# salesforce/LayoutDETR

Hardware: AMD Instinct MI355X
Metric: images/sec G+D fwd-bwd, 256x256 bg x9 elems (higher is better)
Workload: dtype f32

## Files before the change

### include/ldetr_hip.h

```cpp
#ifndef LDETR_HIP_H
#define LDETR_HIP_H

#include <stdint.h>

#ifdef __cplusplus
extern "C" {
#endif

const char* ldetr_last_error(void);
int ldetr_abi_version(void);

int ldetr_debug_trace_tiles(int64_t* buffer);

int ldetr_set_split_bf16(int tiles);

int ldetr_engine_launch_counts(int64_t* f32_pipe, int64_t* bf16_split_pipe);

int ldetr_set_workspace(void* ptr, int64_t bytes);

typedef struct ldetr_tensor4 {
    int N, C, H, W;
    int64_t sn, sc, sh, sw;
} ldetr_tensor4;

typedef struct ldetr_epilogue {
    float alpha;
    const float* col_scale;
    const float* col_bias;
    const float* samp_scale;
    int64_t samp_ld;
    const float* residual;
    int64_t ldr;
    int act;
    float act_alpha;
    float act_gain;
    const float* mask_src;
    int64_t ldm;
    int mask_mode;
    float out_scale;
    float p_drop;
    uint64_t seed;
    const uint64_t* seed_ptr;
    int accumulate;
    float* a_rowsum;
} ldetr_epilogue;

int ldetr_bias_act_f32(const float* x, const float* b, const float* xref, const float* yref, const float* dy, float* y,
                       int64_t sizeX, int sizeB, int64_t stepB, int grad, int act, float alpha, float gain, float clamp,
                       void* stream);

int ldetr_upfirdn2d_f32(const float* x, const float* f, float* y, int N, int C, int inH, int inW,
                        const int64_t* x_strides_nchw, int fh, int fw, int64_t f_stride_h, int64_t f_stride_w,
                        int upx, int upy, int downx, int downy, int padx0, int padx1, int pady0, int pady1, int flip,
                        float gain, int outH, int outW, const int64_t* y_strides_nchw,
                        const float* act_bias, int has_act, float act_alpha, float act_gain, void* stream);

int ldetr_gemm_f32(const float* A, int64_t lda, int ta, const float* B, int64_t ldb, int tb, float* C, int64_t ldc,
                   int M, int N, int K, int splitk, const ldetr_epilogue* ep, int pix_per_sample, void* stream);

typedef struct ldetr_gemm_desc {
    const float* A; int64_t lda; int ta;
    const float* B; int64_t ldb; int tb;
    float* C; int64_t ldc;
    int M, N, K, splitk;
    const ldetr_epilogue* ep;
    int pix_per_sample;
} ldetr_gemm_desc;
int ldetr_gemm_pair_f32(const ldetr_gemm_desc* g0, const ldetr_gemm_desc* g1, void* stream);
int ldetr_gemm_pair_is_single_launch(const ldetr_gemm_desc* g0, const ldetr_gemm_desc* g1);

int ldetr_conv2d_fwd_f32(const float* x, const ldetr_tensor4* xt, const float* w, int Cout, int KH, int KW, int stride,
                         int pad, float* y, int64_t ldy, int OH, int OW, const float* in_scale, int64_t in_scale_ld,
                         const ldetr_epilogue* ep, void* stream);
int ldetr_conv2d_bwd_data_f32(const float* dy, const ldetr_tensor4* dyt, const float* w, int Cin, int KH, int KW,
                              int stride, int pad, float* dx, int64_t lddx, int IH, int IW, const float* dy_scale,
                              int64_t dy_scale_ld, const ldetr_epilogue* ep, void* stream);
int ldetr_conv2d_bwd_weight_f32(const float* x, const ldetr_tensor4* xt, const float* dy, const ldetr_tensor4* dyt,
                                float* dw, int KH, int KW, int stride, int pad, int splitk, const float* x_scale,
                                int64_t x_scale_ld, const float* dy_scale, int64_t dy_scale_ld, int accumulate, void* stream);

int ldetr_conv_transpose2d_fwd_f32(const float* x, const ldetr_tensor4* xt, const float* w, int Cout, int KH, int KW,
                                   int stride, int pad, float* y, int64_t ldy, int OH, int OW, const float* in_scale,
                                   int64_t in_scale_ld, const ldetr_epilogue* ep, void* stream);
int ldetr_conv_transpose2d_bwd_data_f32(const float* dy, const ldetr_tensor4* dyt, const float* w, int Cin, int KH,
                                        int KW, int stride, int pad, float* dx, int64_t lddx, int IH, int IW,
                                        const float* dy_scale, int64_t dy_scale_ld, const ldetr_epilogue* ep,
                                        void* stream);
int ldetr_conv_transpose2d_bwd_weight_f32(const float* x, const ldetr_tensor4* xt, const float* dy,
                                          const ldetr_tensor4* dyt, float* dw, int KH, int KW, int stride, int pad,
                                          int splitk, const float* x_scale, int64_t x_scale_ld, const float* dy_scale,
                                          int64_t dy_scale_ld, int accumulate, void* stream);

int ldetr_attention_fwd_f32(const float* q, int64_t ldq, const float* k, int64_t ldk, const float* v, int64_t ldv,
                            const unsigned char* key_padding_mask, float* out, int64_t ldo, float* lse, int B, int H,
                            int Lq, int Lk, int head_dim, float scale, float p_drop, uint64_t seed, const uint64_t* seed_ptr,
                            int causal, void* stream);
int ldetr_attention_bwd_f32(const float* q, int64_t ldq, const float* k, int64_t ldk, const float* v, int64_t ldv,
                            const unsigned char* key_padding_mask, const float* out, int64_t ldo, const float* lse,
                            const float* dout, int64_t lddo, float* dq, int64_t lddq, float* dk, int64_t lddk,
                            float* dv, int64_t lddv, int B, int H, int Lq, int Lk, int head_dim, float scale,
                            float p_drop, uint64_t seed, const uint64_t* seed_ptr, int causal, void* stream);

int ldetr_torgb_bwd_finish_f32(const float* dws, const float* s, const float* w, int B, int C, float* dw, float* ds, void* stream);

int ldetr_loss_combine_fwd_f32(const float* const* x, const float* w, const int* n, const int* fn, const int* red, int K, int ld,
                               float* vals, float* sums, float* total, void* stream);
int ldetr_loss_combine_bwd_f32(const float* const* x, const float* w, const int* n, const int* fn, const int* red, int K, int ld,
                               const float* g, float* grads, void* stream);
int ldetr_masked_mse_fwd_f32(const float* a, const float* b, const uint8_t* valid, int64_t rows, int D, int bdiv, float* out2, void* stream);
int ldetr_masked_mse_bwd_f32(const float* a, const float* b, const uint8_t* valid, int64_t rows, int D, int bdiv, const float* out2,
                             const float* g, float* da, void* stream);

typedef struct ldetr_ln_args {
    const float* x; const float* r; const float* gamma; const float* beta;
    float* y; float* z; float* mean; float* rstd;
    const float* dy; float* dx; float* dr; float* dgamma; float* dbeta;
    int64_t rows; int D; float eps, p_drop; uint64_t seed; const uint64_t* seed_ptr;
    const float* pos; int64_t pos_rows; float* ypos; const float* dy2;
    int r_parts; int64_t r_part_stride; const float* r_bias;
    const float* dy_parts; int dy_nparts; int64_t dy_part_stride;
} ldetr_ln_args;
int ldetr_layernorm_fwd_group_f32(const ldetr_ln_args* a, int n, void* stream);
int ldetr_layernorm_bwd_group_f32(const ldetr_ln_args* a, int n, void* stream);
int ldetr_sum_parts_f32(const float* base, const float* parts, int n_parts, int64_t part_stride, float* out, int64_t n, void* stream);

typedef struct ldetr_ffn_args {
    const float* x; int64_t ldx;
    const float* w1; const float* b1;
    const float* w2;
    float* h;
    float* ypart;
    int M, F;
    float p_drop; uint64_t seed; const uint64_t* seed_ptr;
    const float* dy;
    float* dxpart;
    float* dh;
} ldetr_ffn_args;
int ldetr_ffn_fwd_group_f32(const ldetr_ffn_args* a, int n, void* stream);
int ldetr_ffn_bwd_group_f32(const ldetr_ffn_args* a, int n, void* stream);

typedef struct ldetr_mha_small_args {
    const float* x; int64_t ldx;
    const float* w_in; const float* b_in; const float* w_out;
    const unsigned char* kpm;
    float* qkv; float* o; float* lse; float* ypart;
    int B, L;
    float scale, p_drop; uint64_t seed; const uint64_t* seed_ptr;
    const float* dr;
    float* dqkv; float* dxpart;
} ldetr_mha_small_args;
int ldetr_mha_small_fwd_group_f32(const ldetr_mha_small_args* a, int n, void* stream);
int ldetr_mha_small_bwd_group_f32(const ldetr_mha_small_args* a, int n, void* stream);

typedef struct ldetr_mha_cross_args {
    const float* x; int64_t ldx;
    const float* w_q; const float* b_q;
    const float* k; int64_t ldk; const float* v; int64_t ldv;
    const float* w_out;
    const unsigned char* kpm;
    float* q; float* o; float* lse; float* ypart;
    int B, Lq, Lk;
    float scale, p_drop; uint64_t seed; const uint64_t* seed_ptr;
    const float* dr;
    float* dq; float* dk; int64_t lddk; float* dv; int64_t lddv; float* dxpart;
} ldetr_mha_cross_args;
int ldetr_mha_cross_fwd_f32(const ldetr_mha_cross_args* a, void* stream);
int ldetr_mha_cross_bwd_f32(const ldetr_mha_cross_args* a, void* stream);

typedef struct ldetr_wgrad_desc {
    const float* A; int64_t lda; const float* B; int64_t ldb;
    float* dW; int64_t ldw; float* db;
    int M, rows, cols;
} ldetr_wgrad_desc;
int ldetr_wgrad_multi_f32(const ldetr_wgrad_desc* d, int n, void* stream);

int ldetr_colsum_f32(const float* a, float* red, int B, int64_t P, int C, void* stream);
int ldetr_act_bwd_reduce_f32(const float* dy, const float* y, float* dv, const float* bias, const float* demod,
                             float* dbias, float* ddemod, int B, int64_t P, int C, int act, float alpha, float gain,
                             void* stream);
int ldetr_mul_reduce_f32(const float* a, const float* x, const float* scale, float* out, float* red, int B, int64_t P,
                         int C, void* stream);
int ldetr_torgb_fwd_f32(const float* x, const float* w, const float* styles, const float* bias, float* y,
                        int B, int64_t P, int C, void* stream);
int ldetr_torgb_bwd_f32(const float* x, const float* dy, const float* w, const float* styles, float* dx, float* dws,
                        float* dbias, int B, int64_t P, int C, void* stream);
int ldetr_sg2_handoff_f32(const float* dxs, const float* x, const float* dy_rgb, float* dv, const float* s_conv, const float* s_rgb,
                          const float* w_rgb, const float* bias, const float* demod, float* ds_conv, float* dws_rgb, float* dbias_rgb,
                          float* dbias, float* ddemod, int B, int64_t P, int C, float alpha, float gain, void* stream);

int ldetr_maxpool3x3s2_fwd_f32(const float* x, float* y, unsigned char* idx, int N, int H, int W, int C, void* stream);
int ldetr_maxpool3x3s2_bwd_f32(const float* dy, const unsigned char* idx, float* dx, int N, int H, int W, int C,
                               void* stream);

int ldetr_grad_sanitize_f32(float* g, int64_t n, float scale, float nan_value, float posinf, float neginf,
                            void* stream);
int ldetr_adam_step_f32(float* p, const float* g, float* m, float* v, int64_t n, int64_t step, float lr, float beta1,
                        float beta2, float eps, int fuse_sanitize, float gscale, float nan_value, float posinf,
                        float neginf, void* stream);
int ldetr_adam_ema_step_f32(float* p, const float* g, float* m, float* v, int64_t n, int64_t step, float lr, float beta1, float beta2,
                            float eps, int fuse_sanitize, float gscale, float nan_value, float posinf, float neginf,
                            float* p_ema, float ema_beta, void* stream);
int ldetr_ema_lerp_f32(float* p_ema, const float* p, int64_t n, float beta, void* stream);

int ldetr_softmax_xent_fwd_f32(const float* logits, int64_t ld, const int64_t* targets, float* row_lse, float* loss_sum, float* count,
                               int64_t rows, int V, int64_t ignore_index, float label_smoothing, void* stream);
int ldetr_softmax_xent_bwd_f32(const float* logits, int64_t ld, const int64_t* targets, const float* row_lse, const float* count,
                               const float* grad_out, float* dlogits, int64_t ldd, int64_t rows, int V, int64_t ignore_index,
                               float label_smoothing, void* stream);

int ldetr_embedding_fwd_f32(const float* weight, const float* pos, const int64_t* ids, float* out, int64_t n, int d, int V, int T,
                            void* stream);
int ldetr_embedding_bwd_f32(const float* dy, const int64_t* ids, float* dweight, int64_t n, int d, int V, int64_t padding_idx,
                            void* stream);

int ldetr_resample_coeffs(int in_size, int out_size, int32_t* bounds, int32_t* weights, int64_t weights_capacity, int* ksize_out);
int ldetr_resize_normalize_u8(const uint8_t* src, int64_t images, int H, int W, int out_h, int out_w, const int32_t* hbounds,
                              const int32_t* hweights, int hksize, const int32_t* vbounds, const int32_t* vweights, int vksize,
                              uint8_t* tmp, uint8_t* out_u8, float* out_chw, float mean0, float mean1, float mean2, float std0,
                              float std1, float std2, void* stream);

#define LDETR_PAGE_FILTER_BLUR 1
#define LDETR_PAGE_FILTER_EDGE 2
int ldetr_page_filter_u8(const uint8_t* src, uint8_t* dst, int64_t images, int H, int W, int kind, float radius, void* stream);

int ldetr_demod_fwd_f32(const float* weight, int64_t so, int64_t si, int64_t sh, int64_t sw, const float* styles, float* dcoefs,
                        float* w2, int B, int O, int I, int KH, int KW, float eps, void* stream);
int ldetr_demod_bwd_f32(const float* weight, int64_t so, int64_t si, int64_t sh, int64_t sw, const float* styles, const float* dcoefs,
                        const float* w2, const float* grad_dcoefs, float* dweight, int accumulate_dweight, float* dstyles, int B, int O,
                        int I, int KH, int KW, void* stream);

int ldetr_layout_losses_f32(const float* bbox, const float* bbox_ref, const uint8_t* valid, int B, int N, float* losses,
                            float* grads, void* stream);
int ldetr_layout_losses_bwd_f32(const float* grads, const float* grad_losses, int B, int N, float* dbbox, void* stream);

int ldetr_layout_finish_f32(const float* bbox_in, const int* num, const float* factors, const unsigned char* jitter, const unsigned char* mode,
                            float* bbox_out, float* overlap, float* alignment, int* order, int C, int K, int N, void* stream);

#define LDETR_FILTER_BILINEAR 0
#define LDETR_FILTER_LANCZOS 1
typedef struct ldetr_layout_raster_args {
    int struct_bytes;
    int B, N, S, nrow, n_colors, n_pages;
    const float* bbox;
    const uint8_t* valid;
    const int32_t* labels;
    const uint8_t* palette;
    const int32_t* page_wh;
    const uint8_t* pages;
    int64_t pages_bytes;
    const int64_t* page_table;
    const int32_t* page_index;
    const int32_t* coeffs;
    int64_t coeffs_len;
    const int64_t* cell_coeffs;
    int32_t* cells_dev;
    uint8_t* out;
} ldetr_layout_raster_args;
int ldetr_resample_coeffs_filter(int filter, int in_size, int out_size, int32_t* bounds, int32_t* weights, int64_t weights_capacity, int* ksize_out);
int ldetr_layout_raster_cell_size(int W, int H, int S, int* wn_out, int* hn_out);
int ldetr_layout_raster_u8(const ldetr_layout_raster_args* a, void* stream);

typedef struct ldetr_patch_resize_args {
    int struct_bytes;
    int n_jobs;
    const uint8_t* src0;
    int64_t src0_bytes;
    const uint8_t* src1;
    int64_t src1_bytes;
    uint8_t* dst;
    int64_t dst_bytes;
    const int64_t* jobs;
    const int32_t* tables;
    const int32_t* tables_host;
    int64_t tables_len;
    int32_t* jobs_dev;
} ldetr_patch_resize_args;
typedef struct ldetr_image_raster_args {
    int struct_bytes;
    int B, N, S, nrow;
    const float* bbox;
    const uint8_t* valid;
    const int32_t* rects;
    const int64_t* patch_off;
    const int64_t* page_off;
    const int32_t* page_wh;
    const uint8_t* pixels;
    int64_t pixels_bytes;
    const int32_t* coeffs;
    int64_t coeffs_len;
    const int64_t* cell_coeffs;
    int32_t* cells_dev;
    uint8_t* out;
} ldetr_image_raster_args;
int ldetr_patch_resize_u8(const ldetr_patch_resize_args* a, void* stream);
int ldetr_image_raster_u8(const ldetr_image_raster_args* a, void* stream);

#define LDETR_PNG_NOT_ELIGIBLE 3
#define LDETR_PNG_MALFORMED 4
typedef struct ldetr_png_decode_args {
    int struct_bytes;
    int n, H, W;
    int phases;
    int reserved;
    const uint8_t* files;
    int64_t files_bytes;
    const int64_t* file_off;
    const int64_t* file_off_dev;
    const int64_t* segments;
    const int64_t* segments_dev;
    int64_t n_segments;
    const int32_t* jobs;
    const int32_t* jobs_dev;
    int64_t n_jobs;
    uint8_t* scratch;
    int64_t scratch_bytes;
    uint8_t* dst;
} ldetr_png_decode_args;
int ldetr_png_scan(const uint8_t* file, int64_t file_bytes, int* width, int* height, int* channels, int64_t* segments, int64_t segments_capacity,
                   int64_t* segments_count, int32_t* row_starts, int64_t row_starts_capacity, int64_t* row_starts_count);
int ldetr_png_decode_u8(const ldetr_png_decode_args* a, void* stream);

typedef struct ldetr_png_encode_args {
    int struct_bytes;
    int H, W;
    int blocks;
    int filter;
    int reserved;
    const uint8_t* src;
    uint8_t* out;
    int64_t out_capacity;
    int64_t* total_bytes;
    uint8_t* workspace;
    int64_t workspace_bytes;
    int64_t* seg_table;
    int64_t seg_table_rows;
} ldetr_png_encode_args;
int ldetr_png_encode_bound(int H, int W, int64_t* out_bytes, int64_t* workspace_bytes);
int ldetr_png_encode_u8(const ldetr_png_encode_args* a, void* stream);

int ldetr_lsap_f64(const double* cost, int batch, int n, int maximize, int* row_ind, int* col_ind, void* stream);

int ldetr_layoutnet_features_f32(const float* bbox, const int64_t* label, const uint8_t* padding_mask, const int* label_map, int map_len,
                                 const float* weights, int64_t weights_len, int num_label, int B, int N, float* out, void* stream);

int ldetr_layoutnet_forward_f32(const float* bbox, const int64_t* label, const uint8_t* padding_mask, const float* enc_weights,
                                int64_t enc_len, const float* dec_weights, int64_t dec_len, int num_label, int B, int N,
                                float* logit_disc, float* logit_cls, float* bbox_pred, float* features, void* stream);

int ldetr_feature_stats_f64(const float* x, int64_t n, int F, double* raw_mean, double* raw_cov, void* stream);

int ldetr_box_giou_pairwise_f32(const float* boxes1, const float* boxes2, int B, int N, int M, int cxcywh, float* iou, float* uni,
                                float* giou, double* cost, double cost_sign, void* stream);

int ldetr_bmm_strided_f32(const float* A, const int64_t* sa, const float* B, const int64_t* sb, float* C, const int64_t* sc,
                          int nb1, int nb2, int M, int N, int K, float alpha, void* stream);

int ldetr_p3_split_f32(const float* src, int64_t ld, void* dst, int64_t rows, int C, void* stream);
int ldetr_p3_merge_f32(const void* src, float* dst, int64_t ld, int64_t rows, int C, void* stream);
int ldetr_p3_weight_bwd(const float* w_ohwi, const float* o_scale, void* dst, int O, int KH, int KW, int I, void* stream);

int ldetr_p3_weight_prep(const int64_t* table_dev, int nconv, int total_blocks, void* stream);

typedef struct ldetr_p3_epilogue {
    float alpha;
    const float* col_scale;
    const float* col_bias;
    const void* residual_p3;
    const float* residual_f32;
    const void* relu_mask_p3;
    int relu;
} ldetr_p3_epilogue;

int ldetr_p3_conv2d_fwd(const void* x, int N, int H, int W, int Cin, const void* w, int Cout, int KH, int KW, int stride, int pad,
// ... 23 lines not shown
```

### layoutdetr_amd/_lib.py

```python
import ctypes
import os
from ctypes import (POINTER, Structure, c_char_p, c_double, c_float, c_int, c_int64, c_ubyte, c_uint64, c_void_p)

_HERE = os.path.dirname(os.path.abspath(__file__))
ABI_VERSION = 25
LIB_PATH = os.environ.get('LDETR_LIB') or os.path.join(_HERE, 'lib', 'libldetr_hip.so')


class Tensor4(Structure):
    _fields_ = [('N', c_int), ('C', c_int), ('H', c_int), ('W', c_int),
                ('sn', c_int64), ('sc', c_int64), ('sh', c_int64), ('sw', c_int64)]


class GemmDesc(Structure):
    _fields_ = [('A', c_void_p), ('lda', c_int64), ('ta', c_int), ('B', c_void_p), ('ldb', c_int64), ('tb', c_int),
                ('C', c_void_p), ('ldc', c_int64), ('M', c_int), ('N', c_int), ('K', c_int), ('splitk', c_int),
                ('ep', c_void_p), ('pix_per_sample', c_int)]


class P3Epilogue(Structure):
    _fields_ = [('alpha', c_float), ('col_scale', c_void_p), ('col_bias', c_void_p), ('residual_p3', c_void_p),
                ('residual_f32', c_void_p), ('relu_mask_p3', c_void_p), ('relu', c_int)]


class Epilogue(Structure):
    _fields_ = [('alpha', c_float), ('col_scale', c_void_p), ('col_bias', c_void_p), ('samp_scale', c_void_p),
                ('samp_ld', c_int64), ('residual', c_void_p), ('ldr', c_int64), ('act', c_int),
                ('act_alpha', c_float), ('act_gain', c_float), ('mask_src', c_void_p), ('ldm', c_int64),
                ('mask_mode', c_int), ('out_scale', c_float), ('p_drop', c_float), ('seed', c_uint64),
                ('seed_ptr', c_void_p), ('accumulate', c_int), ('a_rowsum', c_void_p)]


class LnArgs(Structure):
    _fields_ = [('x', c_void_p), ('r', c_void_p), ('gamma', c_void_p), ('beta', c_void_p),
                ('y', c_void_p), ('z', c_void_p), ('mean', c_void_p), ('rstd', c_void_p),
                ('dy', c_void_p), ('dx', c_void_p), ('dr', c_void_p), ('dgamma', c_void_p), ('dbeta', c_void_p),
                ('rows', c_int64), ('D', c_int), ('eps', c_float), ('p_drop', c_float), ('seed', c_uint64), ('seed_ptr', c_void_p),
                ('pos', c_void_p), ('pos_rows', c_int64), ('ypos', c_void_p), ('dy2', c_void_p),
                ('r_parts', c_int), ('r_part_stride', c_int64), ('r_bias', c_void_p),
                ('dy_parts', c_void_p), ('dy_nparts', c_int), ('dy_part_stride', c_int64)]


class FfnArgs(Structure):
    _fields_ = [('x', c_void_p), ('ldx', c_int64), ('w1', c_void_p), ('b1', c_void_p), ('w2', c_void_p), ('h', c_void_p), ('ypart', c_void_p),
                ('M', c_int), ('F', c_int), ('p_drop', c_float), ('seed', c_uint64), ('seed_ptr', c_void_p),
                ('dy', c_void_p), ('dxpart', c_void_p), ('dh', c_void_p)]


class MhaSmallArgs(Structure):
    _fields_ = [('x', c_void_p), ('ldx', c_int64), ('w_in', c_void_p), ('b_in', c_void_p), ('w_out', c_void_p), ('kpm', c_void_p),
                ('qkv', c_void_p), ('o', c_void_p), ('lse', c_void_p), ('ypart', c_void_p), ('B', c_int), ('L', c_int),
                ('scale', c_float), ('p_drop', c_float), ('seed', c_uint64), ('seed_ptr', c_void_p),
                ('dr', c_void_p), ('dqkv', c_void_p), ('dxpart', c_void_p)]


class MhaCrossArgs(Structure):
    _fields_ = [('x', c_void_p), ('ldx', c_int64), ('w_q', c_void_p), ('b_q', c_void_p), ('k', c_void_p), ('ldk', c_int64), ('v', c_void_p), ('ldv', c_int64),
                ('w_out', c_void_p), ('kpm', c_void_p), ('q', c_void_p), ('o', c_void_p), ('lse', c_void_p), ('ypart', c_void_p),
                ('B', c_int), ('Lq', c_int), ('Lk', c_int), ('scale', c_float), ('p_drop', c_float), ('seed', c_uint64), ('seed_ptr', c_void_p),
                ('dr', c_void_p), ('dq', c_void_p), ('dk', c_void_p), ('lddk', c_int64), ('dv', c_void_p), ('lddv', c_int64), ('dxpart', c_void_p)]


class WgradDesc(Structure):
    _fields_ = [('A', c_void_p), ('lda', c_int64), ('B', c_void_p), ('ldb', c_int64), ('dW', c_void_p), ('ldw', c_int64), ('db', c_void_p),
                ('M', c_int), ('rows', c_int), ('cols', c_int)]


class LayoutRasterArgs(Structure):
    _fields_ = [('struct_bytes', c_int), ('B', c_int), ('N', c_int), ('S', c_int), ('nrow', c_int), ('n_colors', c_int), ('n_pages', c_int),
                ('bbox', c_void_p), ('valid', c_void_p), ('labels', c_void_p), ('palette', c_void_p), ('page_wh', c_void_p),
                ('pages', c_void_p), ('pages_bytes', c_int64), ('page_table', c_void_p), ('page_index', c_void_p),
                ('coeffs', c_void_p), ('coeffs_len', c_int64), ('cell_coeffs', c_void_p), ('cells_dev', c_void_p), ('out', c_void_p)]


class PatchResizeArgs(Structure):
    _fields_ = [('struct_bytes', c_int), ('n_jobs', c_int), ('src0', c_void_p), ('src0_bytes', c_int64), ('src1', c_void_p), ('src1_bytes', c_int64),
                ('dst', c_void_p), ('dst_bytes', c_int64), ('jobs', c_void_p), ('tables', c_void_p), ('tables_host', c_void_p), ('tables_len', c_int64),
                ('jobs_dev', c_void_p)]


class ImageRasterArgs(Structure):
    _fields_ = [('struct_bytes', c_int), ('B', c_int), ('N', c_int), ('S', c_int), ('nrow', c_int),
                ('bbox', c_void_p), ('valid', c_void_p), ('rects', c_void_p), ('patch_off', c_void_p), ('page_off', c_void_p), ('page_wh', c_void_p),
                ('pixels', c_void_p), ('pixels_bytes', c_int64), ('coeffs', c_void_p), ('coeffs_len', c_int64), ('cell_coeffs', c_void_p),
                ('cells_dev', c_void_p), ('out', c_void_p)]


class PngDecodeArgs(Structure):
    _fields_ = [('struct_bytes', c_int), ('n', c_int), ('H', c_int), ('W', c_int), ('phases', c_int), ('reserved', c_int),
                ('files', c_void_p), ('files_bytes', c_int64), ('file_off', c_void_p), ('file_off_dev', c_void_p),
                ('segments', c_void_p), ('segments_dev', c_void_p), ('n_segments', c_int64),
                ('jobs', c_void_p), ('jobs_dev', c_void_p), ('n_jobs', c_int64),
                ('scratch', c_void_p), ('scratch_bytes', c_int64), ('dst', c_void_p)]


class PngEncodeArgs(Structure):
    _fields_ = [('struct_bytes', c_int), ('H', c_int), ('W', c_int), ('blocks', c_int), ('filter', c_int), ('reserved', c_int),
                ('src', c_void_p), ('out', c_void_p), ('out_capacity', c_int64), ('total_bytes', c_void_p),
                ('workspace', c_void_p), ('workspace_bytes', c_int64), ('seg_table', c_void_p), ('seg_table_rows', c_int64)]


_P = c_void_p
_I = c_int
_L = c_int64
_F = c_float
_T4 = POINTER(Tensor4)
_EP = POINTER(Epilogue)

SIGNATURES = {
    'ldetr_set_workspace': [_P, _L],
    'ldetr_bias_act_f32': [_P, _P, _P, _P, _P, _P, _L, _I, _L, _I, _I, _F, _F, _F, _P],
    'ldetr_upfirdn2d_f32': [_P, _P, _P, _I, _I, _I, _I, POINTER(c_int64), _I, _I, _L, _L, _I, _I, _I, _I, _I, _I, _I, _I,
                            _I, _F, _I, _I, POINTER(c_int64), _P, _I, _F, _F, _P],
    'ldetr_gemm_f32': [_P, _L, _I, _P, _L, _I, _P, _L, _I, _I, _I, _I, _EP, _I, _P],
    'ldetr_conv2d_fwd_f32': [_P, _T4, _P, _I, _I, _I, _I, _I, _P, _L, _I, _I, _P, _L, _EP, _P],
    'ldetr_conv2d_bwd_data_f32': [_P, _T4, _P, _I, _I, _I, _I, _I, _P, _L, _I, _I, _P, _L, _EP, _P],
    'ldetr_conv2d_bwd_weight_f32': [_P, _T4, _P, _T4, _P, _I, _I, _I, _I, _I, _P, _L, _P, _L, _I, _P],
    'ldetr_conv_transpose2d_fwd_f32': [_P, _T4, _P, _I, _I, _I, _I, _I, _P, _L, _I, _I, _P, _L, _EP, _P],
    'ldetr_conv_transpose2d_bwd_data_f32': [_P, _T4, _P, _I, _I, _I, _I, _I, _P, _L, _I, _I, _P, _L, _EP, _P],
    'ldetr_conv_transpose2d_bwd_weight_f32': [_P, _T4, _P, _T4, _P, _I, _I, _I, _I, _I, _P, _L, _P, _L, _I, _P],
    'ldetr_attention_fwd_f32': [_P, _L, _P, _L, _P, _L, _P, _P, _L, _P, _I, _I, _I, _I, _I, _F, _F, c_uint64, _P, _I, _P],
    'ldetr_attention_bwd_f32': [_P, _L, _P, _L, _P, _L, _P, _P, _L, _P, _P, _L, _P, _L, _P, _L, _P, _L,
                                _I, _I, _I, _I, _I, _F, _F, c_uint64, _P, _I, _P],
    'ldetr_colsum_f32': [_P, _P, _I, _L, _I, _P],
    'ldetr_act_bwd_reduce_f32': [_P, _P, _P, _P, _P, _P, _P, _I, _L, _I, _I, _F, _F, _P],
    'ldetr_mul_reduce_f32': [_P, _P, _P, _P, _P, _I, _L, _I, _P],
    'ldetr_torgb_fwd_f32': [_P, _P, _P, _P, _P, _I, _L, _I, _P],
    'ldetr_torgb_bwd_f32': [_P, _P, _P, _P, _P, _P, _P, _I, _L, _I, _P],
    'ldetr_maxpool3x3s2_fwd_f32': [_P, _P, _P, _I, _I, _I, _I, _P],
    'ldetr_maxpool3x3s2_bwd_f32': [_P, _P, _P, _I, _I, _I, _I, _P],
    'ldetr_grad_sanitize_f32': [_P, _L, _F, _F, _F, _F, _P],
    'ldetr_adam_step_f32': [_P, _P, _P, _P, _L, _L, _F, _F, _F, _F, _I, _F, _F, _F, _F, _P],
    'ldetr_adam_ema_step_f32': [_P, _P, _P, _P, _L, _L, _F, _F, _F, _F, _I, _F, _F, _F, _F, _P, _F, _P],
    'ldetr_ema_lerp_f32': [_P, _P, _L, _F, _P],
    'ldetr_lsap_f64': [_P, _I, _I, _I, _P, _P, _P],
    'ldetr_layoutnet_features_f32': [_P, _P, _P, POINTER(c_int), _I, _P, _L, _I, _I, _I, _P, _P],
    'ldetr_layoutnet_forward_f32': [_P, _P, _P, _P, _L, _P, _L, _I, _I, _I, _P, _P, _P, _P, _P],
    'ldetr_feature_stats_f64': [_P, _L, _I, _P, _P, _P],
    'ldetr_box_giou_pairwise_f32': [_P, _P, _I, _I, _I, _I, _P, _P, _P, _P, c_double, _P],
    'ldetr_bmm_strided_f32': [_P, _P, _P, _P, _P, _P, _I, _I, _I, _I, _I, _F, _P],
    'ldetr_softmax_xent_fwd_f32': [_P, _L, _P, _P, _P, _P, _L, _I, _L, _F, _P],
    'ldetr_softmax_xent_bwd_f32': [_P, _L, _P, _P, _P, _P, _P, _L, _L, _I, _L, _F, _P],
    'ldetr_embedding_fwd_f32': [_P, _P, _P, _P, _L, _I, _I, _I, _P],
    'ldetr_embedding_bwd_f32': [_P, _P, _P, _L, _I, _I, _L, _P],
    'ldetr_debug_trace_tiles': [_P],
    'ldetr_set_split_bf16': [c_int],
    'ldetr_engine_launch_counts': [POINTER(c_int64), POINTER(c_int64)],
    'ldetr_layernorm_fwd_group_f32': [_P, _I, _P],
    'ldetr_layernorm_bwd_group_f32': [_P, _I, _P],
    'ldetr_sum_parts_f32': [_P, _P, _I, _L, _P, _L, _P],
    'ldetr_ffn_fwd_group_f32': [_P, _I, _P],
    'ldetr_ffn_bwd_group_f32': [_P, _I, _P],
    'ldetr_mha_small_fwd_group_f32': [_P, _I, _P],
    'ldetr_mha_small_bwd_group_f32': [_P, _I, _P],
    'ldetr_mha_cross_fwd_f32': [_P, _P],
    'ldetr_mha_cross_bwd_f32': [_P, _P],
    'ldetr_wgrad_multi_f32': [_P, _I, _P],
    'ldetr_loss_combine_fwd_f32': [_P, _P, _P, _P, _P, _I, _I, _P, _P, _P, _P],
    'ldetr_loss_combine_bwd_f32': [_P, _P, _P, _P, _P, _I, _I, _P, _P, _P],
    'ldetr_masked_mse_fwd_f32': [_P, _P, _P, _L, _I, _I, _P, _P],
    'ldetr_masked_mse_bwd_f32': [_P, _P, _P, _L, _I, _I, _P, _P, _P, _P],
    'ldetr_torgb_bwd_finish_f32': [_P, _P, _P, _I, _I, _P, _P, _P],
    'ldetr_sg2_handoff_f32': [_P, _P, _P, _P, _P, _P, _P, _P, _P, _P, _P, _P, _P, _P, _I, _L, _I, _F, _F, _P],
    'ldetr_gemm_pair_f32': [_P, _P, _P],
    'ldetr_gemm_pair_is_single_launch': [_P, _P],
    'ldetr_demod_fwd_f32': [_P, _L, _L, _L, _L, _P, _P, _P, _I, _I, _I, _I, _I, _F, _P],
    'ldetr_demod_bwd_f32': [_P, _L, _L, _L, _L, _P, _P, _P, _P, _P, _I, _P, _I, _I, _I, _I, _I, _P],
    'ldetr_layout_losses_f32': [_P, _P, _P, _I, _I, _P, _P, _P],
    'ldetr_layout_losses_bwd_f32': [_P, _P, _I, _I, _P, _P],
    'ldetr_layout_finish_f32': [_P, _P, _P, _P, _P, _P, _P, _P, _P, _I, _I, _I, _P],
    'ldetr_resample_coeffs': [_I, _I, _P, _P, _L, _P],
    'ldetr_resample_coeffs_filter': [_I, _I, _I, _P, _P, _L, _P],
    'ldetr_layout_raster_cell_size': [_I, _I, _I, _P, _P],
    'ldetr_layout_raster_u8': [_P, _P],
    'ldetr_patch_resize_u8': [_P, _P],
    'ldetr_image_raster_u8': [_P, _P],
    'ldetr_p3_split_f32': [_P, _L, _P, _L, _I, _P],
    'ldetr_p3_merge_f32': [_P, _P, _L, _L, _I, _P],
    'ldetr_p3_weight_bwd': [_P, _P, _P, _I, _I, _I, _I, _P],
    'ldetr_p3_conv2d_bwd_data': [_P, _I, _I, _I, _I, _P, _I, _I, _I, _I, _I, _I, _I, _P, _P, _P, _P],
    'ldetr_p3_conv2d_fwd': [_P, _I, _I, _I, _I, _P, _I, _I, _I, _I, _I, _P, _P, _P, _P],
    'ldetr_p3_conv2d_bwd_weight': [_P, _I, _I, _I, _I, _P, _I, _I, _I, _I, _I, _P, _P, _P],
    'ldetr_p3_weight_prep': [_P, _I, _I, _P],
    'ldetr_p3_conv2d_fwd_dual': [_P, _P, _I, _I, _I, _I, _P, _P, _I, _I, _I, _I, _I, _P, _P, _P, _P, _P, _P, _P],
    'ldetr_p3_conv2d_bwd_pair': [_P, _I, _I, _I, _I, _P, _P, _I, _I, _I, _I, _I, _I, _I, _P, _P, _P, _P, _P, _P, _P],
    'ldetr_p3_last_launch': [_P],
    'ldetr_engine_last_launch': [_P],
    'ldetr_struct_sizes': [_P],
    'ldetr_resize_normalize_u8': [_P, _L, _I, _I, _I, _I, _P, _P, _I, _P, _P, _I, _P, _P, _P, _F, _F, _F, _F, _F, _F, _P],
    'ldetr_page_filter_u8': [_P, _P, _L, _I, _I, _I, _F, _P],
    'ldetr_png_scan': [_P, _L, _P, _P, _P, _P, _L, _P, _P, _L, _P],
    'ldetr_png_decode_u8': [_P, _P],
    'ldetr_png_encode_bound': [_I, _I, _P, _P],
    'ldetr_png_encode_u8': [_P, _P],
}

_lib = None


def load():
    global _lib
    if _lib is not None:
        return _lib
    if not os.path.exists(LIB_PATH):
        raise RuntimeError(
            f'{LIB_PATH} not found: build the gfx950 kernels first (python -m layoutdetr_amd.build or '
            f'__graft_entry__.build()).  layoutdetr_amd has no CPU/PyTorch fallback path.')
    import torch
    lib = ctypes.CDLL(LIB_PATH)
    lib.ldetr_last_error.restype = c_char_p
    lib.ldetr_last_error.argtypes = []
    lib.ldetr_abi_version.restype = c_int
    lib.ldetr_abi_version.argtypes = []
    for name, argtypes in SIGNATURES.items():
        fn = getattr(lib, name)
        fn.restype = c_int
        fn.argtypes = argtypes
    if lib.ldetr_abi_version() != ABI_VERSION:
        raise RuntimeError('libldetr_hip.so ABI version mismatch; rebuild it')
    sizes = (ctypes.c_int32 * 6)()
    lib.ldetr_struct_sizes(sizes)
    mirror = [ctypes.sizeof(t) for t in (LnArgs, FfnArgs, MhaSmallArgs, MhaCrossArgs, WgradDesc, P3Epilogue)]
    if list(sizes) != mirror:
        raise RuntimeError(f'libldetr_hip.so argument blocks {list(sizes)} do not match the ctypes mirror {mirror}; rebuild')
    _lib = lib
    return lib


def check(rc, what=''):
    if rc != 0:
        msg = load().ldetr_last_error().decode('utf-8', 'replace')
        raise RuntimeError(f'{what}: {msg}' if what else msg)
```

### layoutdetr_amd/build.py

```python
import hashlib
import os
import shutil
import subprocess
import sys
from concurrent.futures import ThreadPoolExecutor

HERE = os.path.dirname(os.path.abspath(__file__))
CSRC = os.path.join(HERE, 'csrc')
LIBDIR = os.path.join(HERE, 'lib')
OBJDIR = os.path.join(LIBDIR, 'obj')
LIBNAME = 'libldetr_hip.so'
ARCH = 'gfx950'

SOURCES = ['ldetr_core.cpp', 'bias_act.hip', 'upfirdn2d.hip', 'gemm_conv.hip', 'attention.hip', 'layernorm.hip',
           'misc_ops.hip', 'optim.hip', 'lsap.hip', 'xent.hip', 'resample.hip', 'layout_loss.hip', 'demod.hip', 'wgrad_smallc.hip', 'stem_conv.hip', 'box_ops.hip', 'ffn_fused.hip', 'conv_c32.hip', 'mha_small.hip', 'p3_engine.hip', 'bmm_strided.hip', 'layoutnet.hip', 'layoutnet_train.hip', 'layout_finish.hip', 'layout_raster.hip', 'page_filter.hip', 'patch_resize.hip', 'png_decode.hip', 'png_encode.hip']
HEADERS = ['ldetr_common.hpp', 'layoutnet_layers.hpp', os.path.join('..', '..', 'include', 'ldetr_hip.h')]

FLAGS = ([] if os.environ.get('LDETR_TILE_TRACE') else ['-DLDETR_TILE_TRACE=0']) + (['-DP3_TRACE'] if os.environ.get('LDETR_P3_TRACE') else []) + ['-O3', '-std=c++17', '-fPIC', f'--offload-arch={ARCH}', '-munsafe-fp-atomics', '-fno-gpu-rdc',
         '-Wno-unused-result', '-Rpass-analysis=kernel-resource-usage']
NO_SCRATCH = ('wgrad_c32_3x3_kernel', 'gemm_f32_kernel', 'gemm_small_kernel', 'attn_fwd_kernel', 'attn_fwd_wide_kernel', 'attn_bwd_kernel', 'ffn_fwd_kernel', 'ffn_bwd_kernel', 'conv3x3_c32_kernel', 'mha_small_fwd_kernel', 'mha_cross_fwd_kernel', 'mha_small_bwd_kernel', 'mha_cross_bwd_kernel', 'wgrad_multi_kernel', 'ln_fwd_kernel', 'ln_bwd_kernel', 'p3_nt_kernel', 'p3_tn_kernel', 'p3_c3_kernel', 'p3_bwd_pair', 'layoutnet_features_kernel', 'layoutnet_forward_kernel', 'feature_stats_f64_kernel', 'layout_finish_kernel', 'layout_raster_kernel', 'page_blur_kernel', 'page_edge_kernel', 'patch_resize_kernel', 'sg2_handoff_kernel', 'png_gather_kernel', 'png_unfilter_kernel', 'png_enc_filter_kernel', 'png_enc_deflate_kernel', 'png_enc_assemble_kernel')


def _hipcc():
    for cand in (os.environ.get('HIPCC'), shutil.which('hipcc'), '/opt/rocm/bin/hipcc'):
        if cand and os.path.exists(cand):
            return cand
    raise RuntimeError('hipcc not found: the gfx950 kernel library cannot be built')


def _digest(paths):
    h = hashlib.sha256()
    for p in paths:
        with open(p, 'rb') as f:
            h.update(f.read())
    h.update(' '.join(FLAGS).encode())
    return h.hexdigest()


def _kernel_resources(remarks):
    out, cur = {}, None
    for line in remarks.splitlines():
        if 'remark:' not in line:
            continue
        body = line.split('remark:', 1)[1].split('[-Rpass-analysis', 1)[0].strip()
        if body.startswith('Function Name:'):
            cur = body.split(':', 1)[1].strip()
            out[cur] = {}
        elif cur is not None and ':' in body:
            k, v = body.rsplit(':', 1)
            out[cur][k.strip()] = v.strip()
    return out


def source_digest():
    return _digest(sorted(os.path.join(CSRC, f) for f in os.listdir(CSRC) if f.endswith(('.hip', '.cpp', '.hpp')) and not f.startswith('.'))
                   + [os.path.normpath(os.path.join(CSRC, HEADERS[-1]))])


def lib_path():
    return os.path.join(LIBDIR, LIBNAME)


def build(force=False, verbose=True):
    os.makedirs(OBJDIR, exist_ok=True)
    hipcc = _hipcc()
    hdrs = [os.path.normpath(os.path.join(CSRC, h)) for h in HEADERS]
    objs, jobs = [], []
    for src in SOURCES:
        sp = os.path.join(CSRC, src)
        obj = os.path.join(OBJDIR, src + '.o')
        stamp = obj + '.sha'
        dig = _digest([sp] + hdrs)
        objs.append(obj)
        if not force and os.path.exists(obj) and os.path.exists(stamp) and open(stamp).read() == dig:
            continue
        jobs.append((sp, obj, stamp, dig))

    def compile_one(job):
        sp, obj, stamp, dig = job
        cmd = [hipcc] + FLAGS + ['-x', 'hip', '-c', sp, '-o', obj]
        if verbose:
            print('[ldetr build]', os.path.basename(sp), flush=True)
        r = subprocess.run(cmd, capture_output=True, text=True)
        if r.returncode != 0:
            raise RuntimeError(f'hipcc failed for {sp}:\n{r.stdout}\n{r.stderr}')
        res = _kernel_resources(r.stderr)
        with open(obj + '.resources.txt', 'w') as f:
            for name, d in res.items():
                f.write(f"{name} vgprs={d.get('VGPRs', '?')} agprs={d.get('AGPRs', '?')} scratch={d.get('ScratchSize [bytes/lane]', '?')} "
                        f"occupancy={d.get('Occupancy [waves/SIMD]', '?')} lds={d.get('LDS Size [bytes/block]', '?')}\n")
        bad = [n for n, d in res.items() if any(k in n for k in NO_SCRATCH) and d.get('ScratchSize [bytes/lane]', '0') != '0']
        if bad:
            raise RuntimeError(f'{os.path.basename(sp)}: scratch memory in register-budgeted kernels: ' + ', '.join(bad[:4]))
        with open(stamp, 'w') as f:
            f.write(dig)

    if jobs:
        with ThreadPoolExecutor(max_workers=min(8, len(jobs))) as ex:
            list(ex.map(compile_one, jobs))
    out = lib_path()
    if jobs or not os.path.exists(out):
        cmd = [hipcc, '-shared', '-fPIC', f'--offload-arch={ARCH}', '-fno-gpu-rdc', '-o', out] + objs
        r = subprocess.run(cmd, capture_output=True, text=True)
        if r.returncode != 0:
            raise RuntimeError(f'link failed:\n{r.stdout}\n{r.stderr}')
        if verbose:
            print('[ldetr build] linked', out, flush=True)
    return out


if __name__ == '__main__':
    build(force='--force' in sys.argv)
```

### layoutdetr_amd/csrc/gemm_conv.hip

```cpp
#include <cstdlib>
#include <type_traits>
#include <atomic>
#include "ldetr_common.hpp"
#include "../../include/ldetr_hip.h"

namespace ldetr {
static thread_local int64_t t_launches_f32 = 0, t_launches_split = 0;
void count_engine_launch(bool bf16_split_pipe) { (bf16_split_pipe ? t_launches_split : t_launches_f32)++; }

enum {
    OP_KC_DENSE = 0,
    OP_KC_CONV = 1,
    OP_KC_CONVT = 2,
    OP_KC_WTAP = 3,
    OP_RC_DENSE = 4,
    OP_RC_PIX = 5,
    OP_RC_WT = 6,
    OP_RC_CONVK = 7,
};

struct Operand {
    const float* p;
    long ld;
    int vec;
// ... 742 lines not shown
                for (int j = 0; j < TN; j++) b[nx][j] = Bs[buf][(kk + 1) * 2 + kl][wn * WN + j * 32 + cl];
            }
            __builtin_amdgcn_sched_barrier(0);
#pragma unroll
            for (int i = 0; i < TM; i++)
#pragma unroll
                for (int j = 0; j < TN; j++)
                    acc[i][j] = __builtin_amdgcn_mfma_f32_32x32x2f32(a[c][i], b[c][j], acc[i][j], 0, 0, 0);
            __builtin_amdgcn_sched_barrier(0);
        }
    };
    auto compute_split = [&]() {
#pragma unroll
        for (int ks = 0; ks < BKT / 16; ks++) {
            bf16x8_t a[TM][3], b[TN][3];
#pragma unroll
            for (int i = 0; i < TM; i++)
#pragma unroll
                for (int q = 0; q < 3; q++) a[i][q] = *reinterpret_cast<const bf16x8_t*>(adrA(q, 2 * ks + kl, wm * WM + i * 32 + cl, 0));
#pragma unroll
            for (int j = 0; j < TN; j++)
#pragma unroll
                for (int q = 0; q < 3; q++) b[j][q] = *reinterpret_cast<const bf16x8_t*>(adrB(q, 2 * ks + kl, wn * WN + j * 32 + cl, 0));
#pragma unroll
            for (int i = 0; i < TM; i++)
#pragma unroll
                for (int j = 0; j < TN; j++) {
                    acc[i][j] = __builtin_amdgcn_mfma_f32_32x32x16_bf16(a[i][1], b[j][1], acc[i][j], 0, 0, 0);
                    acc[i][j] = __builtin_amdgcn_mfma_f32_32x32x16_bf16(a[i][0], b[j][2], acc[i][j], 0, 0, 0);
                    acc[i][j] = __builtin_amdgcn_mfma_f32_32x32x16_bf16(a[i][2], b[j][0], acc[i][j], 0, 0, 0);
                    acc[i][j] = __builtin_amdgcn_mfma_f32_32x32x16_bf16(a[i][0], b[j][1], acc[i][j], 0, 0, 0);
                    acc[i][j] = __builtin_amdgcn_mfma_f32_32x32x16_bf16(a[i][1], b[j][0], acc[i][j], 0, 0, 0);
                    acc[i][j] = __builtin_amdgcn_mfma_f32_32x32x16_bf16(a[i][0], b[j][0], acc[i][j], 0, 0, 0);
                }
        }
    };
    if (nk > 0) {
        gload(z.kbeg, ra0, rb0, sa0);
        lstore(std::bool_constant<SPLIT>{}, 0, ra0, rb0, sa0);
    }
    long long tr1 = 0, tr2 = 0;
    if constexpr (SPLIT) {
        __syncthreads();
        for (int kt = 0; kt < nk; kt++) {
            if (kt + 1 < nk) gload(z.kbeg + (kt + 1) * BKT, ra0, rb0, sa0);
            compute_split();
            __syncthreads();
            if (kt + 1 < nk) { lstore(std::bool_constant<SPLIT>{}, 0, ra0, rb0, sa0); __syncthreads(); }
        }
        float chk = 0.f;
#pragma unroll
        for (int i = 0; i < TM; i++)
#pragma unroll
            for (int j = 0; j < TN; j++)
#pragma unroll
                for (int r = 0; r < 16; r++) chk = __builtin_fmaf(acc[i][j][r], 0.f, chk);
        if (__builtin_expect(__syncthreads_or(chk != chk), 0)) {
            int t2 = tid;
            asm volatile("" : "+v"(t2));
            float (*A1)[LDA] = reinterpret_cast<float (*)[LDA]>(ldetr_smem);
            float (*B1)[LDB] = reinterpret_cast<float (*)[LDB]>(ldetr_smem + BKT * LDA);
            static_assert((size_t)BKT * (LDA + LDB) * sizeof(float) <= (size_t)3 * (BKT / 8) * (PLA + PLB), "the f32 image of one k-tile must fit inside the bf16 image");
#pragma unroll
            for (int i = 0; i < TM; i++)
#pragma unroll
                for (int j = 0; j < TN; j++)
#pragma unroll
                    for (int r = 0; r < 16; r++) acc[i][j][r] = 0.f;
            reset_kstate();
            const int kl2 = (t2 & 63) >> 5, cl2 = t2 & 31, w2 = t2 >> 6, wm2 = w2 / WGN, wn2 = w2 % WGN;
            for (int kt = 0; kt < nk; kt++) {
                gload(z.kbeg + kt * BKT, ra0, rb0, sa0);
                if constexpr (A_DEFER) {
                    if (a_defer) {
#pragma unroll
                        for (int i = 0; i < NUA; i++) { ra0[i].x *= sa0[i].x; ra0[i].y *= sa0[i].y; ra0[i].z *= sa0[i].z; ra0[i].w *= sa0[i].w; }
                    }
                }
#pragma unroll
                for (int i = 0; i < NUA; i++) {
                    int r, k; unitA(t2, i, r, k);
                    if constexpr (A_KC) { A1[k + 0][r] = ra0[i].x; A1[k + 1][r] = ra0[i].y; A1[k + 2][r] = ra0[i].z; A1[k + 3][r] = ra0[i].w; }
                    else { A1[k][r + 0] = ra0[i].x; A1[k][r + 1] = ra0[i].y; A1[k][r + 2] = ra0[i].z; A1[k][r + 3] = ra0[i].w; }
                }
#pragma unroll
                for (int i = 0; i < NUB; i++) {
                    int r, k; unitB(t2, i, r, k);
                    if constexpr (B_KC) { B1[k + 0][r] = rb0[i].x; B1[k + 1][r] = rb0[i].y; B1[k + 2][r] = rb0[i].z; B1[k + 3][r] = rb0[i].w; }
                    else { B1[k][r + 0] = rb0[i].x; B1[k][r + 1] = rb0[i].y; B1[k][r + 2] = rb0[i].z; B1[k][r + 3] = rb0[i].w; }
                }
                __syncthreads();
#pragma unroll 1
                for (int kk = 0; kk < BKT / 2; kk++) {
#pragma unroll
                    for (int i = 0; i < TM; i++) {
                        const float a = A1[kk * 2 + kl2][wm2 * WM + i * 32 + cl2];
#pragma unroll
                        for (int j = 0; j < TN; j++)
                            acc[i][j] = __builtin_amdgcn_mfma_f32_32x32x2f32(a, B1[kk * 2 + kl2][wn2 * WN + j * 32 + cl2], acc[i][j], 0, 0, 0);
                    }
                }
                __syncthreads();
            }
        }
    } else
    {
        __syncthreads();
        if (LDETR_TILE_TRACE && p.trace) tr1 = wall_clock64();
        if (!LDETR_TILE_TRACE) __builtin_amdgcn_sched_barrier(0);
        for (int kt = 0; kt < nk; kt++) {
            const int buf = kt & 1;
            if (kt + 1 < nk) gload(z.kbeg + (kt + 1) * BKT, ra0, rb0, sa0);
            compute(buf);
            if (kt + 1 < nk) lstore(std::false_type{}, buf ^ 1, ra0, rb0, sa0);
            __syncthreads();
        }
    }

    if (LDETR_TILE_TRACE && p.trace) tr2 = wall_clock64();
    if (!LDETR_TILE_TRACE) __builtin_amdgcn_sched_barrier(0);
    auto trace_out = [&]() {
        if (LDETR_TILE_TRACE && p.trace && threadIdx.x == 0) {
            long long* t = p.trace + 5 * (((long)blockIdx.z * gridDim.y + blockIdx.y) * gridDim.x + blockIdx.x);
            t[0] = tr0; t[1] = tr1; t[2] = tr2; t[3] = wall_clock64();
            t[4] = ((long long)__builtin_amdgcn_s_getreg(20 | (31 << 11)) << 32) | (unsigned)__builtin_amdgcn_s_getreg(4 | (31 << 11));
        }
    };
    bool direct = p.splitk <= 1;
    if (p.splitk > 1 && p.ws) {
        const int zb = p.zmode == 1 ? p.pstep * p.pstep : (p.zmode == 2 ? p.ntaps : 1);
        const int ks = blockIdx.z / zb;
        const long tile = ((long)(blockIdx.z - ks * zb) * gridDim.y + blockIdx.y) * gridDim.x + blockIdx.x;
        float* slot0 = p.ws + tile * p.splitk * (long)(BM * BN);
        float* mine = slot0 + (long)ks * (BM * BN);
#pragma unroll
        for (int i = 0; i < TM; i++)
#pragma unroll
            for (int j = 0; j < TN; j++)
#pragma unroll
                for (int r = 0; r < 16; r++)
                    __hip_atomic_store(mine + ((i * TN + j) * 16 + r) * NT + tid, acc[i][j][r], __ATOMIC_RELAXED, __HIP_MEMORY_SCOPE_AGENT);
        asm volatile("s_waitcnt vmcnt(0)" ::: "memory");
        __shared__ int s_last;
        __syncthreads();
        if (tid == 0) {
            int old = atomicAdd(p.ws_count + tile, 1);
            s_last = (old == p.splitk - 1);
            if (s_last) __hip_atomic_store(p.ws_count + tile, 0, __ATOMIC_RELAXED, __HIP_MEMORY_SCOPE_AGENT);
        }
        __syncthreads();
        if (!s_last) { trace_out(); return; }
#pragma unroll
        for (int i = 0; i < TM; i++)
#pragma unroll
            for (int j = 0; j < TN; j++)
#pragma unroll
                for (int r = 0; r < 16; r++) acc[i][j][r] = 0.f;
        for (int sl = 0; sl < p.splitk; sl++) {
            const float* src = slot0 + (long)sl * (BM * BN);
#pragma unroll
            for (int i = 0; i < TM; i++)
#pragma unroll
                for (int j = 0; j < TN; j++)
#pragma unroll
                    for (int r = 0; r < 16; r++)
                        acc[i][j][r] += __hip_atomic_load(src + ((i * TN + j) * 16 + r) * NT + tid, __ATOMIC_RELAXED, __HIP_MEMORY_SCOPE_AGENT);
        }
        direct = true;
    }

    const GemmEpilogue& ep = p.ep;
    const float inv_keep = ep.p_drop > 0.f ? 1.f / (1.f - ep.p_drop) : 1.f;
    if (direct && p.ep_vec) {
        constexpr int CP = BN + 4;
        constexpr int LDSF = 2 * BKT * (LDA + LDB);
        constexpr int PASSES = (BM * CP + LDSF - 1) / LDSF, RP = BM / PASSES;
        static_assert(BM % PASSES == 0 && RP * CP <= LDSF && (RP % 32) == 0, "epilogue staging does not fit");
        static_assert(!SPLIT || RP * CP * 4 <= 3 * (BKT / 8) * (PLA + PLB), "epilogue staging does not fit the split path's LDS image");
        float* Cs = ldetr_smem;
#pragma unroll
        for (int ps = 0; ps < PASSES; ps++) {
            if (ps > 0) __syncthreads();
#pragma unroll
            for (int i = 0; i < TM; i++) {
                const int rb = wm * WM + i * 32 - ps * RP;
                if (rb < 0 || rb >= RP) continue;
#pragma unroll
                for (int j = 0; j < TN; j++)
#pragma unroll
                    for (int r = 0; r < 16; r++)
                        Cs[(rb + (r & 3) + 8 * (r >> 2) + 4 * kl) * CP + wn * WN + j * 32 + cl] = acc[i][j][r];
            }
            __syncthreads();
            for (int u = tid; u < RP * (BN / 4); u += NT) {
                const int rl = u / (BN / 4), c4 = (u - rl * (BN / 4)) * 4;
                const int m = m0 + ps * RP + rl, n = n0 + c4;
                if (m >= z.M || n >= p.N) continue;
                long orow = m;
                if (p.zmode == 1 && p.pstep > 1) {
                    int per = z.DH2 * z.DW2;
                    int nn = m / per; int rem = m - nn * per;
                    int y2 = rem / z.DW2; int x2 = rem - y2 * z.DW2;
                    orow = ((long)nn * p.A.DH + (y2 * p.pstep + z.py)) * p.A.DW + (x2 * p.pstep + z.px);
                }
                const int samp = (ep.samp_scale && p.pix_per_sample > 0) ? (int)((unsigned)orow / (unsigned)p.pix_per_sample) : 0;
                const float4 a4 = *reinterpret_cast<const float4*>(Cs + rl * CP + c4);
                float4 cs4 = make_float4(1.f, 1.f, 1.f, 1.f), cb4 = make_float4(0.f, 0.f, 0.f, 0.f), rs4 = make_float4(0.f, 0.f, 0.f, 0.f);
                if (ep.col_scale) cs4 = *reinterpret_cast<const float4*>(ep.col_scale + n);
                if (ep.col_bias) cb4 = *reinterpret_cast<const float4*>(ep.col_bias + n);
                if (ep.residual) rs4 = *reinterpret_cast<const float4*>(ep.residual + orow * ep.ldr + n);
                float4 mk4 = make_float4(0.f, 0.f, 0.f, 0.f);
                if (ep.mask_mode) mk4 = *reinterpret_cast<const float4*>(ep.mask_src + orow * ep.ldm + n);
                float* dst = p.C + z.c_off + orow * p.ldc + n;
                float4 o;
                o.x = apply_epilogue(ep, a4.x, orow, n + 0, samp, p.ldc, inv_keep, cs4.x, cb4.x, rs4.x, mk4.x);
                o.y = apply_epilogue(ep, a4.y, orow, n + 1, samp, p.ldc, inv_keep, cs4.y, cb4.y, rs4.y, mk4.y);
                o.z = apply_epilogue(ep, a4.z, orow, n + 2, samp, p.ldc, inv_keep, cs4.z, cb4.z, rs4.z, mk4.z);
                o.w = apply_epilogue(ep, a4.w, orow, n + 3, samp, p.ldc, inv_keep, cs4.w, cb4.w, rs4.w, mk4.w);
                if (ep.accumulate) { const float4 c = *reinterpret_cast<const float4*>(dst); o.x += c.x; o.y += c.y; o.z += c.z; o.w += c.w; }
                *reinterpret_cast<float4*>(dst) = o;
            }
        }
        trace_out(); return;
    }
    float cs[TN], cb[TN], sfc[TN];
#pragma unroll
    for (int j = 0; j < TN; j++) {
        int n = n0 + wn * WN + j * 32 + cl;
        cs[j] = (ep.col_scale && n < p.N) ? ep.col_scale[n] : 1.f;
        cb[j] = (ep.col_bias && n < p.N) ? ep.col_bias[n] : 0.f;
        sfc[j] = (p.scol && n < p.N) ? p.scol[(long)z.samp * p.scol_ld + n] : 1.f;
    }
#pragma unroll
    for (int i = 0; i < TM; i++) {
#pragma unroll
        for (int r = 0; r < 16; r++) {
            int m = m0 + wm * WM + i * 32 + (r & 3) + 8 * (r >> 2) + 4 * kl;
            if (m >= z.M) continue;
            long orow = m;
            if (p.zmode == 1 && p.pstep > 1) {
                int per = z.DH2 * z.DW2;
                int n = m / per; int rem = m - n * per;
                int y2 = rem / z.DW2; int x2 = rem - y2 * z.DW2;
                orow = ((long)n * p.A.DH + (y2 * p.pstep + z.py)) * p.A.DW + (x2 * p.pstep + z.px);
            }
            int samp = (ep.samp_scale && p.pix_per_sample > 0) ? (int)((unsigned)orow / (unsigned)p.pix_per_sample) : 0;
            const float sfr = p.srow ? p.srow[(long)z.samp * p.srow_ld + m] : 1.f;
#pragma unroll
            for (int j = 0; j < TN; j++) {
                int n = n0 + wn * WN + j * 32 + cl;
                if (n >= p.N) continue;
                float* dst = p.C + z.c_off + orow * p.ldc + n;
                const float a = acc[i][j][r] * sfr * sfc[j];
                if (!direct) {
                    atomicAdd(dst, a * (ep.row_scale ? ep.alpha * ep.row_scale[orow] : ep.alpha));
                } else {
                    float v = apply_epilogue(ep, a, orow, n, samp, p.ldc, inv_keep, cs[j], cb[j], ep.residual ? ep.residual[orow * ep.ldr + n] : 0.f,
                                           ep.mask_mode ? ep.mask_src[orow * ep.ldm + n] : 0.f);
                    if (ep.accumulate) *dst += v; else *dst = v;
                }
            }
        }
    }
    trace_out();
}

template <int T>
__device__ __forceinline__ void small_load(const Operand& o, int row, int R, int k0, int kl, int kend, float (&f)[16]) {
    const int kb = k0 + 16 * kl;
    if (T == 0) {
        const float* src = o.p + (long)row * o.ld + kb;
        if (row < R && o.vec) {
#pragma unroll
            for (int j = 0; j < 4; j++) {
                float4 v = make_float4(0.f, 0.f, 0.f, 0.f);
                if (kb + 4 * j < kend) v = *reinterpret_cast<const float4*>(src + 4 * j);
                f[4 * j] = v.x; f[4 * j + 1] = v.y; f[4 * j + 2] = v.z; f[4 * j + 3] = v.w;
            }
        } else {
#pragma unroll
            for (int t = 0; t < 16; t++) f[t] = (row < R && kb + t < kend) ? src[t] : 0.f;
        }
    } else {
        const float* src = o.p + (long)kb * o.ld + row;
#pragma unroll
        for (int t = 0; t < 16; t++) f[t] = (row < R && kb + t < kend) ? src[(long)t * o.ld] : 0.f;
    }
}

template <int T>
__device__ __forceinline__ void small_load_fast(const __amdgpu_buffer_rsrc_t& rs, int voff, int k0, int ld, float (&f)[16]) {
    if (T == 0) {
#pragma unroll
        for (int j = 0; j < 4; j++) {
            const auto v = __builtin_amdgcn_raw_buffer_load_b128(rs, voff + 16 * j, k0 * 4, 0);
            f[4 * j] = __int_as_float(v[0]); f[4 * j + 1] = __int_as_float(v[1]); f[4 * j + 2] = __int_as_float(v[2]); f[4 * j + 3] = __int_as_float(v[3]);
        }
    } else {
#pragma unroll
        for (int t = 0; t < 16; t++) f[t] = __int_as_float(__builtin_amdgcn_raw_buffer_load_b32(rs, voff, (k0 + t) * ld * 4, 0));
    }
}

template <int TA, int TB, int NW, bool FAST = false>
__device__ __forceinline__ void gemm_small_body(const GemmParams& p, const int bx, const int by, const int bz, const int sk, const int gx) {
    using f32x16 = __attribute__((__vector_size__(16 * sizeof(float)))) float;
    __shared__ float red[NW][32][33];
    const int tid = threadIdx.x, lane = tid & 63, wave = tid >> 6;
    const int cl = lane & 31, kl = lane >> 5;
    const int m0 = by * 32, n0 = bx * 32;
    const int chunks_all = (p.K + 31) / 32;
    const int cper = (chunks_all + sk - 1) / sk;
    const int kblk0 = bz * cper * 32, kblk1 = min(p.K, kblk0 + cper * 32);
    const int chunks = kblk1 > kblk0 ? (kblk1 - kblk0 + 31) / 32 : 0, per = (chunks + NW - 1) / NW;
    const int kbeg = kblk0 + wave * per * 32, kend = min(kblk1, kbeg + per * 32);
    __amdgpu_buffer_rsrc_t rsA = __builtin_amdgcn_make_buffer_rsrc(const_cast<float*>(p.A.p), 0, FAST ? 0x7fffffff : 0, 0x00020000);
    __amdgpu_buffer_rsrc_t rsB = __builtin_amdgcn_make_buffer_rsrc(const_cast<float*>(p.B.p), 0, FAST ? 0x7fffffff : 0, 0x00020000);
    const int voffA = (m0 + cl < p.M) ? (TA == 0 ? ((m0 + cl) * (int)p.A.ld + 16 * kl) * 4 : (16 * kl * (int)p.A.ld + m0 + cl) * 4) : (int)0x80000000;
    const int voffB = (n0 + cl < p.N) ? (TB == 0 ? ((n0 + cl) * (int)p.B.ld + 16 * kl) * 4 : (16 * kl * (int)p.B.ld + n0 + cl) * 4) : (int)0x80000000;
    auto loadA = [&](int k0, float (&f)[16]) {
        if constexpr (FAST) small_load_fast<TA>(rsA, voffA, k0, (int)p.A.ld, f); else small_load<TA>(p.A, m0 + cl, p.M, k0, kl, kend, f);
        if constexpr (TA == 0) {
            if (p.A.scale) {
                const int kb = k0 + 16 * kl;
#pragma unroll
                for (int j = 0; j < 4; j++) {
                    if (kb + 4 * j < kend) {
                        const float4 s4 = *reinterpret_cast<const float4*>(p.A.scale + kb + 4 * j);
                        f[4 * j] *= s4.x; f[4 * j + 1] *= s4.y; f[4 * j + 2] *= s4.z; f[4 * j + 3] *= s4.w;
                    }
                }
            }
        }
    };
    auto loadB = [&](int k0, float (&f)[16]) {
        if constexpr (FAST) small_load_fast<TB>(rsB, voffB, k0, (int)p.B.ld, f); else small_load<TB>(p.B, n0 + cl, p.N, k0, kl, kend, f);
    };
    f32x16 acc;
#pragma unroll
    for (int r = 0; r < 16; r++) acc[r] = 0.f;
    float a0[16], b0[16], a1[16], b1[16];
    const bool want_rs = TA == 1 && p.ep.a_rowsum != nullptr && bx == 0;
    float rs = 0.f;
    if (kbeg < kend) {
        loadA(kbeg, a0);
        loadB(kbeg, b0);
    }
    for (int k = kbeg; k < kend; k += 64) {
        if (k + 32 < kend) {
            loadA(k + 32, a1);
            loadB(k + 32, b1);
        }
#pragma unroll
        for (int t = 0; t < 16; t++) acc = __builtin_amdgcn_mfma_f32_32x32x2f32(a0[t], b0[t], acc, 0, 0, 0);
        if (want_rs) {
#pragma unroll
            for (int t = 0; t < 16; t++) rs += a0[t];
        }
        if (k + 32 >= kend) break;
        if (k + 64 < kend) {
            loadA(k + 64, a0);
            loadB(k + 64, b0);
        }
#pragma unroll
        for (int t = 0; t < 16; t++) acc = __builtin_amdgcn_mfma_f32_32x32x2f32(a1[t], b1[t], acc, 0, 0, 0);
        if (want_rs) {
#pragma unroll
            for (int t = 0; t < 16; t++) rs += a1[t];
        }
    }
    __shared__ float rsum[NW][32];
    if (want_rs) {
        rs += __shfl_xor(rs, 32);
        if (kl == 0) rsum[wave][cl] = rs;
    }
#pragma unroll
    for (int r = 0; r < 16; r++) red[wave][(r & 3) + 8 * (r >> 2) + 4 * kl][cl] = acc[r];
    __syncthreads();
    if (want_rs && tid < 32 && m0 + tid < p.M) {
        float tot = 0.f;
#pragma unroll
        for (int w = 0; w < NW; w++) tot += rsum[w][tid];
        if (sk > 1) atomicAdd(p.ep.a_rowsum + m0 + tid, tot);
        else p.ep.a_rowsum[m0 + tid] += tot;
    }
    const GemmEpilogue& ep = p.ep;
    const float inv_keep = ep.p_drop > 0.f ? 1.f / (1.f - ep.p_drop) : 1.f;
    float* slot0 = nullptr;
    if (sk > 1) {
        const long tile = (long)by * gx + bx;
        slot0 = p.ws + tile * sk * 1024;
        float* mine = slot0 + (long)bz * 1024;
        for (int q = tid; q < 256; q += NW * 64) {
            const int row = q >> 3, c4 = (q & 7) * 4;
#pragma unroll
            for (int e = 0; e < 4; e++) {
                float sum = 0.f;
#pragma unroll
                for (int w = 0; w < NW; w++) sum += red[w][row][c4 + e];
                __hip_atomic_store(mine + q * 4 + e, sum, __ATOMIC_RELAXED, __HIP_MEMORY_SCOPE_AGENT);
            }
        }
        asm volatile("s_waitcnt vmcnt(0)" ::: "memory");
        __shared__ int s_last_small;
        __syncthreads();
        if (tid == 0) {
            const int old = atomicAdd(p.ws_count + tile, 1);
            s_last_small = (old == sk - 1);
            if (s_last_small) __hip_atomic_store(p.ws_count + tile, 0, __ATOMIC_RELAXED, __HIP_MEMORY_SCOPE_AGENT);
        }
        __syncthreads();
        if (!s_last_small) return;
    }
    for (int q = tid; q < 256; q += NW * 64) {
        const int row = q >> 3, c4 = (q & 7) * 4;
        const int m = m0 + row;
        if (m >= p.M) continue;
        float v[4];
        if (sk > 1) {
#pragma unroll
            for (int e = 0; e < 4; e++) v[e] = 0.f;
            float part[8][4];
#pragma unroll
            for (int z = 0; z < 8; z++)
#pragma unroll
                for (int e = 0; e < 4; e++)
                    part[z][e] = z < sk ? __hip_atomic_load(slot0 + (long)z * 1024 + q * 4 + e, __ATOMIC_RELAXED, __HIP_MEMORY_SCOPE_AGENT) : 0.f;
#pragma unroll
            for (int z = 0; z < 8; z++)
#pragma unroll
                for (int e = 0; e < 4; e++) v[e] += part[z][e];
        } else {
#pragma unroll
            for (int e = 0; e < 4; e++) {
                float sum = 0.f;
#pragma unroll
                for (int w = 0; w < NW; w++) sum += red[w][row][c4 + e];
                v[e] = sum;
            }
        }
        const int samp = (ep.samp_scale && p.pix_per_sample > 0) ? m / p.pix_per_sample : 0;
        float* dst = p.C + (long)m * p.ldc + n0 + c4;
#pragma unroll
        for (int e = 0; e < 4; e++)
            if (n0 + c4 + e < p.N) v[e] = apply_epilogue(ep, v[e], m, n0 + c4 + e, samp, p.ldc, inv_keep, ep.col_scale ? ep.col_scale[n0 + c4 + e] : 1.f, ep.col_bias ? ep.col_bias[n0 + c4 + e] : 0.f,
                                                             ep.residual ? ep.residual[(long)m * ep.ldr + n0 + c4 + e] : 0.f,
                                                             ep.mask_mode ? ep.mask_src[(long)m * ep.ldm + n0 + c4 + e] : 0.f);
        if (n0 + c4 + 3 < p.N && (p.ldc & 3) == 0 && ((((uintptr_t)p.C) & 15) == 0)) {
            float4 o = make_float4(v[0], v[1], v[2], v[3]);
            if (ep.accumulate) { float4 c = *reinterpret_cast<float4*>(dst); o.x += c.x; o.y += c.y; o.z += c.z; o.w += c.w; }
            *reinterpret_cast<float4*>(dst) = o;
        } else {
#pragma unroll
            for (int e = 0; e < 4; e++)
                if (n0 + c4 + e < p.N) { if (ep.accumulate) dst[e] += v[e]; else dst[e] = v[e]; }
        }
    }
}

template <int TA, int TB, int NW, bool FAST = false>
__global__ __launch_bounds__(NW * 64) void gemm_small_kernel(GemmParams p) {
    gemm_small_body<TA, TB, NW, FAST>(p, blockIdx.x, blockIdx.y, blockIdx.z, gridDim.z, gridDim.x);
}

template <int TA0, int TB0, int TA1, int TB1, int NW, bool FAST = false>
__global__ __launch_bounds__(NW * 64) void gemm_small_pair_kernel(GemmParams p0, GemmParams p1, int gx0, int nt0, int sk0, int gx1, int nt1, int sk1) {
    const int b = blockIdx.x;
    if (b < nt0 * sk0) { const int t = b % nt0; gemm_small_body<TA0, TB0, NW, FAST>(p0, t % gx0, t / gx0, b / nt0, sk0, gx0); }
    else { const int c = b - nt0 * sk0, t = c % nt1; gemm_small_body<TA1, TB1, NW, FAST>(p1, t % gx1, t / gx1, c / nt1, sk1, gx1); }
}

static inline bool al16(const void* p) { return (((uintptr_t)p) & 15) == 0; }


constexpr long WS_COUNTERS = 262144;
struct Workspace { void* ptr; size_t bytes; size_t counter_cursor; size_t partial_cursor; };
static Workspace g_workspace[64];
static Workspace& workspace_for_current_device() {
    static Workspace none = {nullptr, 0, 0, 0};
    int dev = 0;
    if (hipGetDevice(&dev) != hipSuccess || dev < 0 || dev >= 64) return none;
    return g_workspace[dev];
}

static bool ring_alloc(long tiles, size_t bytes, int** counters, float** partials) {
    Workspace& w = workspace_for_current_device();
    const size_t need = (bytes + 255) & ~(size_t)255;
    const size_t pbytes = w.bytes > WS_COUNTERS * sizeof(int) ? w.bytes - WS_COUNTERS * sizeof(int) : 0;
    if (!w.ptr || need > pbytes || tiles > WS_COUNTERS) return false;
    if (w.counter_cursor + tiles > (size_t)WS_COUNTERS) w.counter_cursor = 0;
    if (w.partial_cursor + need > pbytes) w.partial_cursor = 0;
    *counters = reinterpret_cast<int*>(w.ptr) + w.counter_cursor;
    *partials = reinterpret_cast<float*>(reinterpret_cast<char*>(w.ptr) + WS_COUNTERS * sizeof(int) + w.partial_cursor);
    w.counter_cursor += tiles; w.partial_cursor += need;
    return true;
}

bool splitk_ws_alloc(long tiles, size_t partial_bytes, float** ws, int** counters) { return ring_alloc(tiles, partial_bytes, counters, ws); }

float* scratch_alloc(size_t bytes) {
    int* counters; float* r;
    return ring_alloc(0, bytes, &counters, &r) ? r : nullptr;
}

static int plan_small_split(GemmParams& p, long blocks) {
    int sk = 1;
    if (blocks <= 128 && p.K >= 1024) {
        sk = p.K / 256; if (sk > 8) sk = 8;
        while (sk > 1 && blocks * sk > 640) sk--;
        if (sk > 1 && !ring_alloc(blocks, (size_t)blocks * sk * 1024 * sizeof(float), &p.ws_count, &p.ws)) sk = 1;
    }
    return sk;
}

static bool small_fast_ok(const GemmParams& p, int ta, int tb) {
    static const int on = (int)knob("SMALL_FAST", 1);
    const long a_bytes = (ta ? (long)p.K * p.A.ld : (long)p.M * p.A.ld) * 4, b_bytes = (tb ? (long)p.K * p.B.ld : (long)p.N * p.B.ld) * 4;
    return on && (p.K % 32) == 0 && a_bytes < 0x7fffffffL && b_bytes < 0x7fffffffL && (ta || (p.A.ld % 4) == 0) && (tb || (p.B.ld % 4) == 0) &&
           ((((uintptr_t)p.A.p) | ((uintptr_t)p.B.p)) & 15) == 0;
}

static bool small_wants8(long blocks, int sk, int K) { return blocks * sk <= 256 && (K + sk - 1) / sk >= 512; }

template <int NW, bool FAST, int TA, int TB>
static auto small_kernel() { return gemm_small_kernel<TA, TB, NW, FAST>; }
template <int NW, bool FAST, int TA0, int TB0, int TA1, int TB1>
static auto small_kernel() { return gemm_small_pair_kernel<TA0, TB0, TA1, TB1, NW, FAST>; }

template <int... MODES, typename... Args>
static void launch_small_kernel(bool fast, bool w8, dim3 grid, hipStream_t st, const Args&... args) {
    if (fast) {
        if (w8) hipLaunchKernelGGL((small_kernel<8, true, MODES...>()), grid, 512, 0, st, args...);
        else hipLaunchKernelGGL((small_kernel<4, true, MODES...>()), grid, 256, 0, st, args...);
    } else {
        if (w8) hipLaunchKernelGGL((small_kernel<8, false, MODES...>()), grid, 512, 0, st, args...);
        else hipLaunchKernelGGL((small_kernel<4, false, MODES...>()), grid, 256, 0, st, args...);
    }
    t_launches_f32++;
}

template <int TA, int TB>
static int launch_small(GemmParams& p, hipStream_t st) {
    dim3 grid(cdiv(p.N, 32), cdiv(p.M, 32), 1);
    const long blocks = (long)grid.x * grid.y;
    const int sk = plan_small_split(p, blocks);
    grid.z = sk;
    const bool fast = small_fast_ok(p, TA, TB);
    const bool w8 = small_wants8(blocks, sk, p.K);
    launch_small_kernel<TA, TB>(fast, w8, grid, st, p);
    note_engine_launch(2, 32, 32, 0, w8 ? 8 : 4, fast ? 1 : 0, 0, sk, blocks * sk, TA * 2 + TB);
    return check_launch("gemm_small");
}

template <int TA0>
static int launch_small_pair(GemmParams& p0, GemmParams& p1, hipStream_t st) {
    const int gx0 = cdiv(p0.N, 32), nt0 = gx0 * cdiv(p0.M, 32), gx1 = cdiv(p1.N, 32), nt1 = gx1 * cdiv(p1.M, 32);
    const int sk0 = plan_small_split(p0, nt0), sk1 = plan_small_split(p1, nt1);
    const bool w8 = small_wants8(nt0, sk0, p0.K) && small_wants8(nt1, sk1, p1.K);
    const bool fast = small_fast_ok(p0, TA0, 1) && small_fast_ok(p1, 1, 1);
    const dim3 grid((unsigned)(nt0 * sk0 + nt1 * sk1));
    launch_small_kernel<TA0, 1, 1, 1>(fast, w8, grid, st, p0, p1, gx0, nt0, sk0, gx1, nt1, sk1);
    note_engine_launch(3, 32, 32, 0, w8 ? 8 : 4, fast ? 1 : 0, 0, sk0 * 256 + sk1, (long)grid.x, (TA0 * 2 + 1) * 4 + 3);
    return check_launch("gemm_small_pair");
}

struct EpiParams { GemmEpilogue ep; float* C; long ldc; long rows; int N; int pix_per_sample; };

__global__ __launch_bounds__(256) void gemm_epilogue_kernel(EpiParams q) {
    const float inv_keep = q.ep.p_drop > 0.f ? 1.f / (1.f - q.ep.p_drop) : 1.f;
    const long total = q.rows * q.N;
    for (long i = (long)blockIdx.x * blockDim.x + threadIdx.x; i < total; i += (long)gridDim.x * blockDim.x) {
        long row = i / q.N; int n = (int)(i - row * q.N);
        int samp = (q.ep.samp_scale && q.pix_per_sample > 0) ? (int)(row / q.pix_per_sample) : 0;
        float* dst = q.C + row * q.ldc + n;
        *dst = apply_epilogue(q.ep, *dst, row, n, samp, q.ldc, inv_keep, q.ep.col_scale ? q.ep.col_scale[n] : 1.f, q.ep.col_bias ? q.ep.col_bias[n] : 0.f,
                              q.ep.residual ? q.ep.residual[row * q.ep.ldr + n] : 0.f,
                              q.ep.mask_mode ? q.ep.mask_src[row * q.ep.ldm + n] : 0.f);
    }
}

static bool epilogue_is_linear(const GemmEpilogue& ep) {
    return !ep.col_scale && !ep.samp_scale && !ep.col_bias && !ep.residual && !ep.act && !ep.mask_mode && ep.p_drop == 0.f &&
           ep.out_scale == 1.f;
}


#ifndef T128_BK
#define T128_BK 32
#endif
#ifndef T128_WAVES
#define T128_WAVES 8
#endif
#ifndef LDETR_EPILOGUE_VEC
#define LDETR_EPILOGUE_VEC 1
#endif
#ifndef T12864_SPLIT_MIN_TILES
#define T12864_SPLIT_MIN_TILES 64
#endif
#ifndef T12864_WAVES
#define T12864_WAVES 8
#define T12864_BK 32
#endif

static const long SMALL_GEMM_TILES = 256;
constexpr long SMALL_GEMM_MNK = 1l << 30;
static bool small_class(long M, long N, long K) { return (long)cdiv(M, 64) * cdiv(N, 64) < SMALL_GEMM_TILES && M * N * K <= SMALL_GEMM_MNK; }
#ifndef WGRAD_MIN_K
#define WGRAD_MIN_K 512
#endif

__global__ void __launch_bounds__(256) zero_fill_kernel(float* __restrict__ dst, long pitch, long width, long rows) {
    const long total = rows * width;
    for (long i = (long)blockIdx.x * 256 + threadIdx.x; i < total; i += (long)gridDim.x * 256) {
        const long r = i / width;
        dst[r * pitch + (i - r * width)] = 0.f;
    }
}
static int zero_fill(float* dst, long pitch, long width, long rows, hipStream_t st) {
    if (rows <= 0 || width <= 0) return LDETR_OK;
    if (pitch == width) { width *= rows; pitch = width; rows = 1; }
    long total = rows * width;
    int g = (int)((total + 255) / 256); if (g > 2048) g = 2048;
    hipLaunchKernelGGL(zero_fill_kernel, g, 256, 0, st, dst, pitch, width, rows);
    return check_launch("zero_fill");
}

static long long* g_trace_buffer = nullptr;
static std::atomic<int> g_split_bf16_override{-1};

static int split_bf16_tiles() {
    static const int env = (int)knob("SPLIT_BF16", 15);
    const int ovr = g_split_bf16_override.load(std::memory_order_relaxed);
    return ovr >= 0 ? ovr : env;
}
bool engine_split_enabled() { return split_bf16_tiles() != 0; }

template <int AMODE>
constexpr bool fast_cap_a = (AMODE == OP_KC_CONV || AMODE == OP_KC_CONVT || AMODE == OP_KC_DENSE || AMODE == OP_RC_DENSE || AMODE == OP_RC_PIX);
template <int BMODE>
constexpr bool fast_cap_b = (BMODE == OP_KC_DENSE || BMODE == OP_RC_WT || BMODE == OP_RC_DENSE || BMODE == OP_RC_PIX || BMODE == OP_KC_WTAP);
template <int AMODE, int BMODE>
constexpr bool fast_cap = fast_cap_a<AMODE> || fast_cap_b<BMODE>;

template <int AMODE, int BMODE>
static bool fast_operands_ok(const GemmParams& p, int Mmax) {
    static const int fast_loads = (int)knob("FAST_LOADS", 63);
    constexpr int BKT = 32;
    constexpr bool a_cap = fast_cap_a<AMODE>;
    if (!fast_cap<AMODE, BMODE>) return false;
    const long lim = 0x7fffffffL;
    auto taps_ok = [&](int C, int KH, int KW) {
        return C > 0 && (C % BKT) == 0 && C >= (p.narrow ? BKT : 2 * BKT) && (long)KH * KW <= 32 && p.samp_pix == 0;
    };
    if (AMODE == OP_KC_CONV) {
        const long padoff = (long)p.A.pad * p.A.sh + (long)p.A.pad * p.A.sw;
        if (!((fast_loads & 1) && p.A.vec && p.zmode == 0 && taps_ok(p.A.C, p.A.KH, p.A.KW) && ((long)p.nsamp * p.A.sn + padoff) * 4 < lim)) return false;
    }
    if (AMODE == OP_KC_CONVT) {
        const long shift = (long)(p.A.KH - 1) * p.A.sh + (long)(p.A.KW - 1) * p.A.sw;
        const int tstep = p.zmode == 1 ? p.pstep : 1;
        if (!((fast_loads & 4) && p.A.vec && taps_ok(p.A.C, p.A.KH, p.A.KW) && tstep == p.A.stride &&
              ((long)p.nsamp * p.A.sn + 2 * shift + p.A.sh + p.A.sw) * 4 < lim)) return false;
    }
    if (AMODE == OP_KC_DENSE) {
        if (!((fast_loads & 8) && p.A.vec && (p.K % BKT) == 0 && (long)Mmax * p.A.ld * 4 < lim && p.samp_pix == 0 && p.zmode == 0)) return false;
    }
    if (BMODE == OP_KC_DENSE) {
        if (!((fast_loads & 2) && p.B.vec && (p.K % BKT) == 0 && (long)p.N * p.B.ld * 4 < lim && p.samp_pix == 0 && (p.zmode == 0 || a_cap))) return false;
    }
    if (AMODE == OP_RC_DENSE) {
        if (!((fast_loads & 16) && p.A.vec && (long)p.K * p.A.ld * 4 < lim)) return false;
    }
    if (BMODE == OP_RC_DENSE) {
        if (!((fast_loads & 16) && p.B.vec && (long)p.K * p.B.ld * 4 < lim)) return false;
    }
    if (BMODE == OP_KC_WTAP) {
        if (!((fast_loads & 4) && p.B.vec && taps_ok(p.B.C, p.B.KH, p.B.KW) && p.B.C == p.A.C && (long)p.N * p.B.ld * 4 < lim)) return false;
    }
    if (AMODE == OP_RC_PIX) {
        const int DH = p.A.DH, DW = p.A.DW, pad = p.A.tapped ? p.A.pad : 0;
        const bool rows_ok = DH > 0 && DW > 0 && ((DW % BKT) == 0 || ((BKT % DW) == 0 && ((long)DH * DW) % BKT == 0));
        if (!((fast_loads & 32) && p.A.vec && rows_ok && (p.K % BKT) == 0 && (BMODE != OP_RC_PIX || (p.B.DH == DH && p.B.DW == DW)) &&
              ((long)p.nsamp * p.A.sn + (long)pad * (p.A.sh + p.A.sw) + (long)BKT * (p.A.sh + p.A.sw)) * 4 < lim)) return false;
    }
    if (BMODE == OP_RC_PIX) {
        const int DH = p.B.DH, DW = p.B.DW, pad = p.B.tapped ? p.B.pad : 0;
        const bool rows_ok = DH > 0 && DW > 0 && ((DW % BKT) == 0 || ((BKT % DW) == 0 && ((long)DH * DW) % BKT == 0));
        if (!((fast_loads & 32) && p.B.vec && rows_ok && (p.K % BKT) == 0 &&
              ((long)p.nsamp * p.B.sn + (long)pad * (p.B.sh + p.B.sw) + (long)BKT * (p.B.sh + p.B.sw)) * 4 < lim)) return false;
    }
    if (BMODE == OP_RC_WT) {
        const int C = (AMODE <= OP_KC_WTAP) ? p.A.C : p.B.C;
        if (!((fast_loads & 4) && p.B.vec && taps_ok(p.B.C, p.B.KH, p.B.KW) && p.B.C == C &&
              ((long)p.B.C * p.B.ld + (long)p.B.KH * p.B.KW * p.B.Cr) * 4 < lim)) return false;
    }
    return true;
}

template <int BM, int BN, int BKT, int AMODE, int BMODE, int NWV, bool FAST, bool SPLIT = false>
static int launch_tile_impl(GemmParams& p, dim3 grid, hipStream_t st) {
    p.trace = g_trace_buffer;
    constexpr bool a_kc = AMODE <= OP_KC_WTAP, b_kc = BMODE <= OP_KC_WTAP;
    constexpr size_t lds = SPLIT ? (size_t)3 * (BKT / 8) * ((BM * 16 + (a_kc ? LDETR_KC_PAD : 0)) + (BN * 16 + (b_kc ? LDETR_KC_PAD : 0)))
                                 : (size_t)2 * BKT * ((BM + 2) + (BN + 2)) * sizeof(float);
    auto kern = gemm_f32_kernel<BM, BN, BKT, AMODE, BMODE, NWV, FAST, SPLIT>;
    if (lds > 64 * 1024) {
        static std::atomic<bool> raised[64];
        int dev = 0;
        if (hipGetDevice(&dev) != hipSuccess || dev < 0 || dev >= 64) dev = -1;
        if (dev < 0 || !raised[dev].load(std::memory_order_acquire)) {
            if (hipFuncSetAttribute(reinterpret_cast<const void*>(kern), hipFuncAttributeMaxDynamicSharedMemorySize, (int)lds) != hipSuccess) {
                set_error("gemm: cannot raise the dynamic LDS limit to %zu bytes", lds);
                return LDETR_ERR_LAUNCH;
            }
            if (dev >= 0) raised[dev].store(true, std::memory_order_release);
        }
    }
    hipLaunchKernelGGL(kern, grid, NWV * 64, lds, st, p);
    (SPLIT ? t_launches_split : t_launches_f32)++;
    note_engine_launch(1, BM, BN, BKT, NWV, FAST ? 1 : 0, SPLIT ? 1 : 0, p.splitk > 1 ? p.splitk : 1, (long)grid.x * grid.y * grid.z, AMODE * 16 + BMODE);
    return check_launch("gemm_f32");
}

template <int BM, int BN, int BKT, int AMODE, int BMODE, int NWV = 4>
static int launch_tile(GemmParams& p, dim3 grid, int Mmax, hipStream_t st) {
    if constexpr (fast_cap<AMODE, BMODE>) {
        if (fast_operands_ok<AMODE, BMODE>(p, Mmax)) return launch_tile_impl<BM, BN, BKT, AMODE, BMODE, NWV, true>(p, grid, st);
    }
    return launch_tile_impl<BM, BN, BKT, AMODE, BMODE, NWV, false>(p, grid, st);
}

template <int AMODE, int BMODE>
static int launch_gemm(GemmParams& p, int Mmax, long out_rows, int zbase, bool auto_split, bool caller_zeroed, hipStream_t st) {
    const int sk0 = p.splitk > 1 ? p.splitk : 1;
    long t128 = (long)cdiv(Mmax, 128) * cdiv(p.N, 128) * zbase * sk0;
    bool use128 = (t128 >= 384 && Mmax >= 128 && p.N >= 128);
    long t64 = (long)cdiv(Mmax, 64) * cdiv(p.N, 64) * zbase;
    long t12864 = (long)cdiv(Mmax, 128) * cdiv(p.N, 64) * zbase * sk0;
    bool use12864 = !use128 && t12864 >= 512 && Mmax >= 128;
    if (!use128 && !use12864 && auto_split && p.splitk <= 1 && zbase == 1 && Mmax >= 128 && t12864 >= T12864_SPLIT_MIN_TILES &&
        !(p.ep.accumulate && !epilogue_is_linear(p.ep))) {
        const int sk = (int)((512 + t12864 - 1) / t12864);
        if (sk >= 2 && sk <= 8 && p.K / sk >= 512) { use12864 = true; p.splitk = sk; }
    }
    if (!use128 && !use12864 && auto_split && p.splitk <= 1 && t64 < 768 && !(p.ep.accumulate && !epilogue_is_linear(p.ep))) {
        int want = (int)(((t64 < 160 ? 384 : 1024) + t64 - 1) / t64);
        int maxs = p.K / (t64 < 160 ? 128 : 256);
        int sk = want < maxs ? want : maxs;
        if (sk >= 2) p.splitk = sk;
    }
    {
        static const int ft = (int)knob("FORCE_TILE", 0);
        static const int fs = (int)knob("FORCE_SK", 0);
        if (ft) {
            use128 = ft == 3 && Mmax >= 128 && p.N >= 128; use12864 = ft == 2 && Mmax >= 128;
            if (fs) { int s2 = fs; while (s2 > 1 && p.K / s2 < 64) s2--; p.splitk = (p.ep.accumulate && !epilogue_is_linear(p.ep)) ? 1 : s2; }
        }
    }
    constexpr bool narrow_cap = (AMODE == OP_KC_CONV || AMODE == OP_KC_CONVT) && (BMODE == OP_KC_DENSE || BMODE == OP_RC_WT || BMODE == OP_KC_WTAP);
    bool use_narrow = false;
    if constexpr (narrow_cap) {
        if (p.N <= 32 && p.N % 4 == 0 && p.splitk <= 1 && (long)cdiv(Mmax, 256) * zbase >= 512) {
            use_narrow = true; use128 = use12864 = false; p.narrow = 1;
        }
    }
    GemmEpilogue full = p.ep;
    const bool split = p.splitk > 1;
    bool fixup = false;
    if (split && !(caller_zeroed && epilogue_is_linear(p.ep)) && !(p.ep.accumulate && epilogue_is_linear(p.ep))) {
        const int bm = (use128 || use12864) ? 128 : 64, bn = use128 ? 128 : 64;
        const long tiles = (long)cdiv(p.N, bn) * cdiv(Mmax, bm) * zbase;
        fixup = ring_alloc(tiles, (size_t)tiles * p.splitk * bm * bn * sizeof(float), &p.ws_count, &p.ws);
    }
    if (split && !fixup) {
        if (!p.ep.accumulate && !caller_zeroed) {
            if (int zrc = zero_fill(p.C, p.ldc, p.N, out_rows, st)) return zrc;
        }
    }
    {
        const GemmEpilogue& e = p.ep;
        auto ok4 = [](const void* q, long ld) { return !q || (al16(q) && (ld % 4) == 0); };
        p.ep_vec = (p.N % 4 == 0) && al16(p.C) && (p.ldc % 4 == 0) && (p.c_tap_stride % 4 == 0) && ok4(e.col_scale, 0) && ok4(e.col_bias, 0) &&
                   ok4(e.residual, e.ldr) && ok4(e.samp_scale, e.samp_ld) && ok4(e.mask_mode ? e.mask_src : nullptr, e.ldm) && !p.srow && !p.scol && !e.row_scale && LDETR_EPILOGUE_VEC;
    }
    dim3 grid(cdiv(p.N, use128 ? 128 : 64), cdiv(Mmax, (use128 || use12864) ? 128 : 64), zbase * (split ? p.splitk : 1));
    constexpr int split_min_kk = 128;
    const int split_tiles = split_bf16_tiles();
    bool sp = false;
    if constexpr (fast_cap<AMODE, BMODE>) sp = split_tiles && (p.K / (split ? p.splitk : 1)) >= split_min_kk && fast_operands_ok<AMODE, BMODE>(p, Mmax);
    if constexpr (narrow_cap) {
        if (use_narrow) {
            if constexpr (fast_cap<AMODE, BMODE>) { if (sp && (split_tiles & 4)) return launch_tile_impl<256, 32, 32, AMODE, BMODE, 4, true, true>(p, dim3(1, cdiv(Mmax, 256), zbase), st); }
            return launch_tile<256, 32, 32, AMODE, BMODE, 4>(p, dim3(1, cdiv(Mmax, 256), zbase), Mmax, st);
        }
    }
    int rc = LDETR_OK;
    if constexpr (fast_cap<AMODE, BMODE>) {
        if (sp && use128 && (split_tiles & 1)) rc = launch_tile_impl<128, 128, 32, AMODE, BMODE, 4, true, true>(p, grid, st);
        else if (sp && use12864 && (split_tiles & 2)) rc = launch_tile_impl<128, 64, 32, AMODE, BMODE, 4, true, true>(p, grid, st);
        else if (sp && !use128 && !use12864 && (split_tiles & 8)) rc = launch_tile_impl<64, 64, 32, AMODE, BMODE, 4, true, true>(p, grid, st);
        else sp = false;
    }
    if (!sp) {
        if (use128) rc = launch_tile<128, 128, T128_BK, AMODE, BMODE, T128_WAVES>(p, grid, Mmax, st);
        else if (use12864) rc = launch_tile<128, 64, T12864_BK, AMODE, BMODE, T12864_WAVES>(p, grid, Mmax, st);
        else rc = launch_tile<64, 64, 32, AMODE, BMODE>(p, grid, Mmax, st);
    }
    if (rc) return rc;
    if (split && !fixup && !epilogue_is_linear(full)) {
        EpiParams q;
        q.ep = full; q.ep.alpha = 1.f; q.ep.row_scale = nullptr; q.ep.accumulate = 0;
        q.C = p.C; q.ldc = p.ldc; q.rows = out_rows; q.N = p.N; q.pix_per_sample = p.pix_per_sample;
        long total = out_rows * p.N;
        int g = (int)((total + 255) / 256); if (g > 4096) g = 4096; if (g < 1) g = 1;
        hipLaunchKernelGGL(gemm_epilogue_kernel, g, 256, 0, st, q);
        rc = check_launch("gemm_epilogue");
    }
    return rc;
}

static int wgrad_auto_split(int M, int N, int K, int zbase) {
    const int WMINK = ((double)M * N * K * zbase < 6e8) ? 128 : WGRAD_MIN_K;
    auto pick = [&](long tiles, long target, int min_k) {
        long s = (target + tiles - 1) / tiles, maxs = K / min_k;
        if (s > maxs) s = maxs;
        return (int)(s < 1 ? 1 : s);
    };
    if (M >= 128 && N >= 128) {
        long t = (long)cdiv(M, 128) * cdiv(N, 128) * zbase; int s = pick(t, 512, WMINK);
        if (t * s >= 384) return s;
    }
    if (M >= 128) {
        long t = (long)cdiv(M, 128) * cdiv(N, 64) * zbase; int s = pick(t, 768, WMINK);
        if (t * s >= 512) return s;
    }
    long t = (long)cdiv(M, 64) * cdiv(N, 64) * zbase;
    return pick(t, 768, WMINK);
}

static void set_sample_slices(GemmParams& p, int nsamp, int pix_per_samp, int want, const float* srow, long srow_ld,
                              const float* scol, long scol_ld) {
    int q = (want + nsamp / 2) / nsamp;
    if (q < 1) q = 1;
    while (q > 1 && pix_per_samp / q < 64) q--;
    p.samp_pix = pix_per_samp; p.samp_q = q;
    p.srow = srow; p.srow_ld = srow_ld; p.scol = scol; p.scol_ld = scol_ld;
    p.splitk = nsamp * q;
    if (p.splitk > 1) p.ep.accumulate = 0;
}

static void fill_epilogue(GemmEpilogue& ep, const ldetr_epilogue* e) {
    memset(&ep, 0, sizeof(ep));
    ep.out_scale = 1.f; ep.act_gain = 1.f; ep.alpha = 1.f;
    if (!e) return;
    ep.alpha = e->alpha;
    ep.col_scale = e->col_scale; ep.col_bias = e->col_bias;
    ep.samp_scale = e->samp_scale; ep.samp_ld = e->samp_ld;
    ep.residual = e->residual; ep.ldr = e->ldr;
    ep.act = e->act; ep.act_alpha = e->act_alpha; ep.act_gain = e->act_gain;
    ep.mask_src = e->mask_src; ep.ldm = e->ldm; ep.mask_mode = e->mask_mode;
    ep.out_scale = e->out_scale; ep.p_drop = e->p_drop; ep.seed = e->seed; ep.seed_ptr = (const unsigned long long*)e->seed_ptr; ep.accumulate = e->accumulate;
    ep.a_rowsum = e->a_rowsum;
}

static void init_operand(Operand& o) { memset(&o, 0, sizeof(o)); o.KW = 1; o.KH = 1; o.stride = 1; o.C = 1; o.Cr = 1; }

static GemmParams new_params() {
    GemmParams p; memset(&p, 0, sizeof(p));
    init_operand(p.A); init_operand(p.B);
    return p;
}

static void set_conv_src(Operand& o, const float* x, const ldetr_tensor4* t) {
    o.p = x; o.SH = t->H; o.SW = t->W; o.sn = t->sn; o.sh = t->sh; o.sw = t->sw; o.sc = t->sc;
}

static void set_conv_operand(Operand& o, const float* x, const ldetr_tensor4* t, const float* scale, long scale_ld, int DH, int DW,
                             int stride, int pad, int KH, int KW) {
    set_conv_src(o, x, t);
    o.DH = DH; o.DW = DW; o.stride = stride; o.pad = pad; o.KH = KH; o.KW = KW;
    o.scale = scale; o.scale_ld = scale_ld;
    o.vec = al16(x) && (t->sn % 4 == 0) && (t->sh % 4 == 0) && (t->sw % 4 == 0) && (!scale || (al16(scale) && scale_ld % 4 == 0));
}

static bool packed_nhwc(const ldetr_tensor4* t) { return t->sw == t->C && t->sh == (long)t->W * t->C && t->sn == (long)t->H * t->W * t->C; }

}

using namespace ldetr;

extern "C" int ldetr_debug_trace_tiles(int64_t* buffer) {
    g_trace_buffer = reinterpret_cast<long long*>(buffer);
    return LDETR_OK;
}

extern "C" int ldetr_engine_launch_counts(int64_t* f32_pipe, int64_t* bf16_split_pipe) {
    if (f32_pipe) *f32_pipe = t_launches_f32;
    if (bf16_split_pipe) *bf16_split_pipe = t_launches_split;
    return LDETR_OK;
}

extern "C" int ldetr_set_split_bf16(int tiles) {
    const int prev = g_split_bf16_override.exchange(tiles);
    return prev;
}

extern "C" int ldetr_set_workspace(void* ptr, int64_t bytes) {
    int dev = 0;
    LDETR_CHECK(hipGetDevice(&dev) == hipSuccess && dev >= 0 && dev < 64, "set_workspace: no current device");
    LDETR_CHECK(bytes >= 0, "set_workspace: negative size");
    LDETR_CHECK(!ptr || (((uintptr_t)ptr) & 15) == 0, "set_workspace: pointer must be 16-byte aligned");
    LDETR_CHECK(!ptr || bytes > (int64_t)(WS_COUNTERS * sizeof(int)), "set_workspace: too small");
    g_workspace[dev].ptr = ptr; g_workspace[dev].bytes = ptr ? (size_t)bytes : 0;
    g_workspace[dev].counter_cursor = 0; g_workspace[dev].partial_cursor = 0;
    return LDETR_OK;
}

static GemmParams fill_dense(const ldetr_gemm_desc& g) {
    GemmParams p = new_params();
    p.A.p = g.A; p.A.ld = g.lda; p.B.p = g.B; p.B.ld = g.ldb;
    p.A.vec = al16(g.A) && (g.lda % 4 == 0) && (g.ta ? (g.M % 4 == 0) : (g.K % 4 == 0));
    p.B.vec = al16(g.B) && (g.ldb % 4 == 0) && (g.tb ? (g.N % 4 == 0) : (g.K % 4 == 0));
    p.M = g.M; p.N = g.N; p.K = g.K; p.C = g.C; p.ldc = g.ldc;
    p.zmode = 0; p.splitk = 1; p.pstep = 1; p.nsamp = 1; p.pix_per_sample = g.pix_per_sample;
    fill_epilogue(p.ep, g.ep);
    return p;
}

static int gemm_dense(const ldetr_gemm_desc& g, void* stream) {
    const int M = g.M, N = g.N, K = g.K, ta = g.ta, tb = g.tb;
    LDETR_CHECK(g.A && g.B && g.C, "gemm: null pointer");
    LDETR_CHECK(M >= 0 && N >= 0 && K >= 0, "gemm: negative dimension");
    if (M == 0 || N == 0) return LDETR_OK;
    GemmParams p = fill_dense(g);
    p.splitk = g.splitk < 1 ? 1 : g.splitk;
    LDETR_CHECK(!(p.splitk > 1 && p.ep.accumulate && !epilogue_is_linear(p.ep)), "gemm: split-K + accumulate needs a linear epilogue");
    hipStream_t st = (hipStream_t)stream;
    const bool auto_split = (g.splitk == 0);
    const bool small = auto_split && small_class(M, N, K);
    if (p.ep.a_rowsum) {
        LDETR_CHECK(ta == 1 && g.lda == M, "gemm: a_rowsum needs ta == 1 and a packed A (lda == M)");
        if (!(small && tb)) {
            int rc = ldetr_colsum_f32(g.A, p.ep.a_rowsum, 1, K, M, stream);
            if (rc) return rc;
            p.ep.a_rowsum = nullptr;
        }
    }
    if (small) {
        if (!ta && !tb) return launch_small<0, 0>(p, st);
        if (!ta && tb) return launch_small<0, 1>(p, st);
        if (ta && tb) return launch_small<1, 1>(p, st);
    }
    if (!ta && !tb) return launch_gemm<OP_KC_DENSE, OP_KC_DENSE>(p, M, M, 1, auto_split, false, st);
    if (!ta && tb) return launch_gemm<OP_KC_DENSE, OP_RC_DENSE>(p, M, M, 1, auto_split, false, st);
    if (ta && tb) return launch_gemm<OP_RC_DENSE, OP_RC_DENSE>(p, M, M, 1, auto_split, false, st);
    set_error("gemm: (ta=1, tb=0) is not instantiated");
    return LDETR_ERR_UNSUPPORTED;
}

extern "C" int ldetr_gemm_f32(const float* A, int64_t lda, int ta, const float* B, int64_t ldb, int tb,
                              float* C, int64_t ldc, int M, int N, int K, int splitk,
                              const ldetr_epilogue* ep, int pix_per_sample, void* stream) {
    const ldetr_gemm_desc g = {A, lda, ta, B, ldb, tb, C, ldc, M, N, K, splitk, ep, pix_per_sample};
    return gemm_dense(g, stream);
}

static bool small_class(const ldetr_gemm_desc& g) {
    return g.splitk == 0 && g.M > 0 && g.N > 0 && g.K > 0 && small_class(g.M, g.N, g.K);
}

static bool pair_single_launch(const ldetr_gemm_desc* g0, const ldetr_gemm_desc* g1) {
    static const int pair_on = (int)knob("GEMM_PAIR", 1);
    const bool nn_tn = g0->ta == 0 && g0->tb == 1 && g1->ta == 1 && g1->tb == 1, tn_tn = g0->ta == 1 && g0->tb == 1 && g1->ta == 1 && g1->tb == 1;
    return pair_on && (nn_tn || tn_tn) && g0->A && g0->B && g0->C && g1->A && g1->B && g1->C && small_class(*g0) && small_class(*g1) &&
           (!g1->ep || !g1->ep->a_rowsum || g1->lda == g1->M) && (!(g0->ep && g0->ep->a_rowsum) || (tn_tn && g0->lda == g0->M));
}

extern "C" int ldetr_gemm_pair_is_single_launch(const ldetr_gemm_desc* g0, const ldetr_gemm_desc* g1) {
    return (g0 && g1 && pair_single_launch(g0, g1)) ? 1 : 0;
}

extern "C" int ldetr_gemm_pair_f32(const ldetr_gemm_desc* g0, const ldetr_gemm_desc* g1, void* stream) {
    LDETR_CHECK(g0 && g1, "gemm_pair: null descriptor");
    if (pair_single_launch(g0, g1)) {
        GemmParams p0 = fill_dense(*g0), p1 = fill_dense(*g1);
        return g0->ta == 1 ? launch_small_pair<1>(p0, p1, (hipStream_t)stream) : launch_small_pair<0>(p0, p1, (hipStream_t)stream);
    }
    int rc = gemm_dense(*g0, stream);
    if (rc) return rc;
    return gemm_dense(*g1, stream);
}

extern "C" int ldetr_conv2d_fwd_f32(const float* x, const ldetr_tensor4* xt, const float* w, int Cout, int KH, int KW,
                                    int stride, int pad, float* y, int64_t ldy, int OH, int OW,
                                    const float* in_scale, int64_t in_scale_ld,
                                    const ldetr_epilogue* ep, void* stream) {
    LDETR_CHECK(x && w && y && xt, "conv2d_fwd: null pointer");
    int eOH = (xt->H + 2 * pad - KH) / stride + 1, eOW = (xt->W + 2 * pad - KW) / stride + 1;
    LDETR_CHECK(eOH == OH && eOW == OW, "conv2d_fwd: output size mismatch (expected %dx%d)", eOH, eOW);
    {
        const int took = try_launch_stem_conv(x, xt, w, Cout, KH, KW, stride, pad, y, ldy, OH, OW, in_scale, ep, (hipStream_t)stream);
        if (took >= 0) return took;
    }
    {
        const int took = try_launch_conv_c32(x, xt, w, Cout, KH, KW, stride, pad, y, ldy, OH, OW, in_scale, in_scale_ld, ep, 0, (hipStream_t)stream);
        if (took > 0) t_launches_f32++;
        if (took != 0) return took > 0 ? LDETR_OK : LDETR_ERR_LAUNCH;
    }
    GemmParams p = new_params();
    set_conv_operand(p.A, x, xt, in_scale, in_scale_ld, OH, OW, stride, pad, KH, KW);
    p.A.C = xt->C;
    p.A.vec = p.A.vec && (xt->sc == 1) && (xt->C % 4 == 0);
    long K = (long)KH * KW * xt->C;
    p.B.p = w; p.B.ld = K; p.B.vec = al16(w) && (K % 4 == 0);
    p.M = xt->N * OH * OW; p.N = Cout; p.K = (int)K; p.C = y; p.ldc = ldy;
    p.zmode = 0; p.splitk = 1; p.pstep = 1; p.nsamp = xt->N; p.pix_per_sample = OH * OW;
    fill_epilogue(p.ep, ep);
    hipStream_t st = (hipStream_t)stream;
    if (KH == 1 && KW == 1 && stride == 1 && pad == 0 && p.A.vec && !in_scale && packed_nhwc(xt)) {
        p.A.ld = xt->C;
        if (!p.ep.samp_scale && small_class(p.M, p.N, p.K)) return launch_small<0, 0>(p, st);
        return launch_gemm<OP_KC_DENSE, OP_KC_DENSE>(p, p.M, p.M, 1, true, false, st);
    }
    return launch_gemm<OP_KC_CONV, OP_KC_DENSE>(p, p.M, p.M, 1, true, false, st);
}

extern "C" int ldetr_conv2d_bwd_data_f32(const float* dy, const ldetr_tensor4* dyt, const float* w, int Cin, int KH, int KW,
                                         int stride, int pad, float* dx, int64_t lddx, int IH, int IW,
                                         const float* dy_scale, int64_t dy_scale_ld,
                                         const ldetr_epilogue* ep, void* stream) {
    LDETR_CHECK(dy && w && dx && dyt, "conv2d_bwd_data: null pointer");
    LDETR_CHECK(dyt->sc == 1 && dyt->C % 4 == 0 && Cin % 4 == 0, "conv2d_bwd_data: channels must be NHWC-contiguous multiples of 4");
    {
        const int took = try_launch_conv_c32(dy, dyt, w, Cin, KH, KW, stride, pad, dx, lddx, IH, IW, dy_scale, dy_scale_ld, ep, 1, (hipStream_t)stream);
        if (took > 0) t_launches_f32++;
        if (took != 0) return took > 0 ? LDETR_OK : LDETR_ERR_LAUNCH;
    }
    GemmParams p = new_params();
    set_conv_operand(p.A, dy, dyt, dy_scale, dy_scale_ld, IH, IW, stride, pad, KH, KW);
    p.A.C = dyt->C;
    LDETR_CHECK(p.A.vec, "conv2d_bwd_data: dy must be 16-byte aligned NHWC");
    p.B.p = w; p.B.ld = (long)KH * KW * Cin; p.B.C = dyt->C; p.B.Cr = Cin; p.B.KH = KH; p.B.KW = KW;
    p.B.vec = al16(w);
    p.N = Cin; p.C = dx; p.ldc = lddx;
    p.zmode = 1; p.splitk = 1; p.pstep = stride; p.nsamp = dyt->N; p.pix_per_sample = IH * IW;
    p.M = dyt->N * IH * IW; p.K = KH * KW * dyt->C;
    fill_epilogue(p.ep, ep);
    if (KH == 1 && KW == 1 && stride == 1 && pad == 0 && packed_nhwc(dyt) && (!dy_scale || dy_scale_ld == 0) && dyt->C % 4 == 0 &&
        !p.ep.samp_scale && small_class(p.M, p.N, p.K)) {
        GemmParams g = p;
        g.zmode = 0; g.pstep = 1; g.A.ld = dyt->C; g.B.ld = Cin; g.B.vec = al16(w) && (Cin % 4 == 0);
        return launch_small<0, 1>(g, (hipStream_t)stream);
    }
    int Mmax = dyt->N * cdiv(IH, stride) * cdiv(IW, stride);
    return launch_gemm<OP_KC_CONVT, OP_RC_WT>(p, Mmax, (long)p.M, stride * stride, true, false, (hipStream_t)stream);
}

static int wgrad_begin(GemmParams& p, int splitk, int nsamp, float* dw, long wsz, int accumulate, hipStream_t st) {
    p = new_params();
    fill_epilogue(p.ep, nullptr);
    p.splitk = splitk; p.pstep = 1; p.nsamp = nsamp; p.pix_per_sample = 0;
    if (!accumulate) { if (int zrc = zero_fill(dw, wsz, wsz, 1, st)) return zrc; }
    if (splitk == 1 && accumulate) p.ep.accumulate = 1;
    return LDETR_OK;
}

static void wgrad_factor_sample_scales(GemmParams& p, int nsamp, int pix_per_samp, int accumulate, const float*& dy_scale, long dy_scale_ld,
                                       const float*& x_scale, long x_scale_ld) {
    if (!((dy_scale || x_scale) && (!dy_scale || dy_scale_ld != 0) && (!x_scale || x_scale_ld != 0) && pix_per_samp >= 64)) return;
    set_sample_slices(p, nsamp, pix_per_samp, p.splitk, dy_scale, dy_scale_ld, x_scale, x_scale_ld);
    if (p.splitk == 1 && accumulate) p.ep.accumulate = 1;
    dy_scale = nullptr; x_scale = nullptr;
}

extern "C" int ldetr_conv2d_bwd_weight_f32(const float* x, const ldetr_tensor4* xt, const float* dy, const ldetr_tensor4* dyt,
                                           float* dw, int KH, int KW, int stride, int pad, int splitk,
                                           const float* x_scale, int64_t x_scale_ld,
                                           const float* dy_scale, int64_t dy_scale_ld, int accumulate, void* stream) {
    LDETR_CHECK(x && dy && dw && xt && dyt, "conv2d_bwd_weight: null pointer");
    LDETR_CHECK(dyt->sc == 1, "conv2d_bwd_weight: dy must be NHWC");
    int Cin = xt->C, Cout = dyt->C, OH = dyt->H, OW = dyt->W;
    hipStream_t st = (hipStream_t)stream;
    int Kpix = dyt->N * OH * OW;
    const bool gather = (xt->sc != 1 || Cin % 4 != 0);
    if (splitk < 1)
        splitk = gather ? wgrad_auto_split(Cout, KH * KW * Cin, Kpix, 1) : wgrad_auto_split(Cout, Cin, Kpix, KH * KW);
    GemmParams p;
    if (int rc = wgrad_begin(p, splitk, xt->N, dw, (long)Cout * KH * KW * Cin, accumulate, st)) return rc;
    if (!gather) {
        const int took = try_launch_wgrad_smallc(x, xt, dy, dyt, dw, KH, KW, stride, pad, x_scale, x_scale_ld, dy_scale, dy_scale_ld, st);
        if (took > 0) t_launches_f32++;
        if (took != 0) return took > 0 ? LDETR_OK : LDETR_ERR_LAUNCH;
    }
    p.M = Cout; p.K = Kpix; p.C = dw; p.ldc = (long)KH * KW * Cin;
    if (gather) {
        LDETR_CHECK(packed_nhwc(dyt), "conv2d_bwd_weight: dy must be packed NHWC");
        LDETR_CHECK(!x_scale && !dy_scale, "conv2d_bwd_weight: scales unsupported on the scalar-gather path");
        p.A.p = dy; p.A.ld = Cout; p.A.vec = al16(dy) && (Cout % 4 == 0);
        set_conv_src(p.B, x, xt);
        p.B.DH = OH; p.B.DW = OW; p.B.C = Cin; p.B.stride = stride; p.B.pad = pad; p.B.KH = KH; p.B.KW = KW;
        p.N = KH * KW * Cin; p.zmode = 0;
        return launch_gemm<OP_RC_DENSE, OP_RC_CONVK>(p, p.M, p.M, 1, false, true, st);
    }
    if (dy_scale && dy_scale_ld == 0) { p.ep.row_scale = dy_scale; dy_scale = nullptr; }
    p.N = Cin; p.zmode = 2; p.ntaps = KH * KW; p.c_tap_stride = Cin;
    wgrad_factor_sample_scales(p, dyt->N, OH * OW, accumulate, dy_scale, dy_scale_ld, x_scale, x_scale_ld);
    if (!dy_scale && packed_nhwc(dyt)) {
        p.A.p = dy; p.A.ld = Cout; p.A.vec = al16(dy) && (Cout % 4 == 0);
        if (!x_scale && KH == 1 && KW == 1 && stride == 1 && pad == 0 && packed_nhwc(xt)) {
            p.B.p = x; p.B.ld = Cin; p.B.vec = al16(x);
            if (small_class(p.M, p.N, p.K) && Kpix <= 8192) {
                p.zmode = 0; p.ntaps = 1; p.c_tap_stride = 0; p.splitk = 1; p.ep.accumulate = 1;
                return launch_small<1, 1>(p, st);
            }
            return launch_gemm<OP_RC_DENSE, OP_RC_DENSE>(p, p.M, p.M, 1, false, true, st);
        }
        set_conv_operand(p.B, x, xt, x_scale, x_scale_ld, OH, OW, stride, pad, KH, KW);
        p.B.tapped = 1;
        return launch_gemm<OP_RC_DENSE, OP_RC_PIX>(p, p.M, p.M, p.ntaps, false, true, st);
    }
    set_conv_operand(p.A, dy, dyt, dy_scale, dy_scale_ld, OH, OW, 1, 0, 1, 1);
    p.A.vec = p.A.vec && (Cout % 4 == 0);
    set_conv_operand(p.B, x, xt, x_scale, x_scale_ld, OH, OW, stride, pad, KH, KW);
    p.B.tapped = 1;
    return launch_gemm<OP_RC_PIX, OP_RC_PIX>(p, p.M, p.M, p.ntaps, false, true, st);
}

extern "C" int ldetr_conv_transpose2d_fwd_f32(const float* x, const ldetr_tensor4* xt, const float* w, int Cout, int KH, int KW,
                                              int stride, int pad, float* y, int64_t ldy, int OH, int OW,
                                              const float* in_scale, int64_t in_scale_ld,
                                              const ldetr_epilogue* ep, void* stream) {
    LDETR_CHECK(x && w && y && xt, "conv_transpose2d_fwd: null pointer");
    LDETR_CHECK(xt->sc == 1 && xt->C % 4 == 0, "conv_transpose2d_fwd: x must be NHWC with C % 4 == 0");
    int eOH = (xt->H - 1) * stride - 2 * pad + KH, eOW = (xt->W - 1) * stride - 2 * pad + KW;
    LDETR_CHECK(eOH == OH && eOW == OW, "conv_transpose2d_fwd: output size mismatch (expected %dx%d)", eOH, eOW);
    GemmParams p = new_params();
    set_conv_operand(p.A, x, xt, in_scale, in_scale_ld, OH, OW, stride, pad, KH, KW);
    p.A.C = xt->C;
    LDETR_CHECK(p.A.vec, "conv_transpose2d_fwd: x must be 16-byte aligned NHWC");
    p.B.p = w; p.B.ld = (long)KH * KW * xt->C; p.B.C = xt->C; p.B.KH = KH; p.B.KW = KW; p.B.vec = al16(w);
    LDETR_CHECK(p.B.vec, "conv_transpose2d_fwd: w must be 16-byte aligned");
    p.N = Cout; p.C = y; p.ldc = ldy;
    p.zmode = 1; p.splitk = 1; p.pstep = stride; p.nsamp = xt->N; p.pix_per_sample = OH * OW;
    p.M = xt->N * OH * OW; p.K = KH * KW * xt->C;
    fill_epilogue(p.ep, ep);
    int Mmax = xt->N * cdiv(OH, stride) * cdiv(OW, stride);
    return launch_gemm<OP_KC_CONVT, OP_KC_WTAP>(p, Mmax, (long)p.M, stride * stride, false, false, (hipStream_t)stream);
}

extern "C" int ldetr_conv_transpose2d_bwd_data_f32(const float* dy, const ldetr_tensor4* dyt, const float* w, int Cin, int KH, int KW,
                                                   int stride, int pad, float* dx, int64_t lddx, int IH, int IW,
                                                   const float* dy_scale, int64_t dy_scale_ld,
                                                   const ldetr_epilogue* ep, void* stream) {
    LDETR_CHECK(dy && w && dx && dyt, "conv_transpose2d_bwd_data: null pointer");
    LDETR_CHECK(dyt->sc == 1 && dyt->C % 4 == 0 && Cin % 4 == 0, "conv_transpose2d_bwd_data: channels must be NHWC multiples of 4");
    GemmParams p = new_params();
    set_conv_operand(p.A, dy, dyt, dy_scale, dy_scale_ld, IH, IW, stride, pad, KH, KW);
    p.A.C = dyt->C;
    LDETR_CHECK(p.A.vec, "conv_transpose2d_bwd_data: dy must be 16-byte aligned NHWC");
    p.B.p = w; p.B.ld = (long)KH * KW * Cin; p.B.C = dyt->C; p.B.Cr = Cin; p.B.KH = KH; p.B.KW = KW; p.B.vec = al16(w);
    p.M = dyt->N * IH * IW; p.N = Cin; p.K = KH * KW * dyt->C; p.C = dx; p.ldc = lddx;
    p.zmode = 0; p.splitk = 1; p.pstep = 1; p.nsamp = dyt->N; p.pix_per_sample = IH * IW;
    fill_epilogue(p.ep, ep);
    return launch_gemm<OP_KC_CONV, OP_RC_WT>(p, p.M, p.M, 1, true, false, (hipStream_t)stream);
}

extern "C" int ldetr_conv_transpose2d_bwd_weight_f32(const float* x, const ldetr_tensor4* xt, const float* dy, const ldetr_tensor4* dyt,
                                                     float* dw, int KH, int KW, int stride, int pad, int splitk,
                                                     const float* x_scale, int64_t x_scale_ld,
                                                     const float* dy_scale, int64_t dy_scale_ld, int accumulate, void* stream) {
    LDETR_CHECK(x && dy && dw && xt && dyt, "conv_transpose2d_bwd_weight: null pointer");
    LDETR_CHECK(dyt->sc == 1 && xt->sc == 1 && xt->C % 4 == 0 && dyt->C % 4 == 0, "conv_transpose2d_bwd_weight: NHWC, C % 4 == 0 required");
    int Cin = xt->C, Cout = dyt->C;
    hipStream_t st = (hipStream_t)stream;
    if (splitk < 1) splitk = wgrad_auto_split(Cout, Cin, xt->N * xt->H * xt->W, KH * KW);
    GemmParams p;
    if (int rc = wgrad_begin(p, splitk, xt->N, dw, (long)Cout * KH * KW * Cin, accumulate, st)) return rc;
    wgrad_factor_sample_scales(p, xt->N, xt->H * xt->W, accumulate, dy_scale, dy_scale_ld, x_scale, x_scale_ld);
    set_conv_operand(p.A, dy, dyt, dy_scale, dy_scale_ld, xt->H, xt->W, stride, pad, KH, KW);
    p.A.tapped = 1;
    p.M = Cout; p.N = Cin; p.K = xt->N * xt->H * xt->W; p.C = dw; p.ldc = (long)KH * KW * Cin;
    p.zmode = 2; p.ntaps = KH * KW; p.c_tap_stride = Cin;
    set_conv_operand(p.B, x, xt, x_scale, x_scale_ld, xt->H, xt->W, 1, 0, 1, 1);
    if (!x_scale && packed_nhwc(xt)) {
        p.B.p = x; p.B.ld = Cin; p.B.vec = al16(x);
        return launch_gemm<OP_RC_PIX, OP_RC_DENSE>(p, p.M, p.M, p.ntaps, false, true, st);
    }
    return launch_gemm<OP_RC_PIX, OP_RC_PIX>(p, p.M, p.M, p.ntaps, false, true, st);
}
```

### layoutdetr_amd/hip/attention.py

```python
import math

import torch

from . import core
from .linear import linear


class _AttnFn(torch.autograd.Function):

    @staticmethod
    def forward(ctx, q, k, v, kpm, B, H, Lq, Lk, p_drop, kv_grad_dst=None):
        core.require_gpu(q, k, v, kpm)
        ctx.kv_grad_dst = kv_grad_dst
        dh = q.shape[1] // H
        assert q.stride(1) == 1 and k.stride(1) == 1 and v.stride(1) == 1
        d = H * dh
        out = torch.empty((B * Lq, d), device=q.device, dtype=torch.float32)
        lse = torch.empty((B * H * Lq,), device=q.device, dtype=torch.float32)
        seed = core.next_seed() if p_drop > 0 else 0
        scale = 1.0 / math.sqrt(dh)
        core.check(core.lib().ldetr_attention_fwd_f32(
            core.ptr(q), q.stride(0), core.ptr(k), k.stride(0), core.ptr(v), v.stride(0), core.ptr(kpm),
            core.ptr(out), d, core.ptr(lse), B, H, Lq, Lk, dh, scale, p_drop, seed, core.seed_ptr() if p_drop > 0 else None,
            0, core.stream()), 'attention_fwd')
        ctx.save_for_backward(q, k, v, kpm, out, lse)
        ctx.cfg = (B, H, Lq, Lk, dh, scale, p_drop, seed)
        return out

    @staticmethod
    def backward(ctx, dout):
        q, k, v, kpm, out, lse = ctx.saved_tensors
        B, H, Lq, Lk, dh, scale, p_drop, seed = ctx.cfg
        d = H * dh
        dout = core.f32c(dout)
        dq = torch.empty((B * Lq, d), device=q.device, dtype=torch.float32)
        if ctx.kv_grad_dst is not None:
            dk, dv = ctx.kv_grad_dst()
        else:
            dk = torch.empty((B * Lk, d), device=q.device, dtype=torch.float32)
            dv = torch.empty((B * Lk, d), device=q.device, dtype=torch.float32)
        core.check(core.lib().ldetr_attention_bwd_f32(
            core.ptr(q), q.stride(0), core.ptr(k), k.stride(0), core.ptr(v), v.stride(0), core.ptr(kpm),
            core.ptr(out), d, core.ptr(lse), core.ptr(dout), d, core.ptr(dq), d, core.ptr(dk), dk.stride(0), core.ptr(dv), dv.stride(0),
            B, H, Lq, Lk, dh, scale, p_drop, seed, core.seed_ptr() if p_drop > 0 else None, 0, core.stream()), 'attention_bwd')
        return dq, dk, dv, None, None, None, None, None, None, None


class _AttnPackedFn(torch.autograd.Function):

    @staticmethod
    def forward(ctx, qkv, v_sep, kpm, B, H, L, p_drop, causal=False):
        core.require_gpu(qkv, v_sep, kpm)
        assert qkv.stride(1) == 1
        d = qkv.shape[1] // (3 if v_sep is None else 2)
        dh = d // H
        q, k = qkv[:, :d], qkv[:, d:2 * d]
        v = qkv[:, 2 * d:] if v_sep is None else v_sep
        assert v.stride(1) == 1
        out = torch.empty((B * L, d), device=qkv.device, dtype=torch.float32)
        lse = torch.empty((B * H * L,), device=qkv.device, dtype=torch.float32)
        seed = core.next_seed() if p_drop > 0 else 0
        scale = 1.0 / math.sqrt(dh)
        core.check(core.lib().ldetr_attention_fwd_f32(
            core.ptr(q), q.stride(0), core.ptr(k), k.stride(0), core.ptr(v), v.stride(0), core.ptr(kpm),
            core.ptr(out), d, core.ptr(lse), B, H, L, L, dh, scale, p_drop, seed, core.seed_ptr() if p_drop > 0 else None,
            1 if causal else 0, core.stream()), 'attention_fwd')
        ctx.save_for_backward(qkv, v_sep, kpm, out, lse)
        ctx.cfg = (B, H, L, dh, scale, p_drop, seed, 1 if causal else 0)
        return out

    @staticmethod
    def backward(ctx, dout):
        qkv, v_sep, kpm, out, lse = ctx.saved_tensors
        B, H, L, dh, scale, p_drop, seed, causal = ctx.cfg
        d = H * dh
        q, k = qkv[:, :d], qkv[:, d:2 * d]
        v = qkv[:, 2 * d:] if v_sep is None else v_sep
        dout = core.f32c(dout)
        dqkv = torch.empty_like(qkv)
        dq, dk = dqkv[:, :d], dqkv[:, d:2 * d]
        dv = dqkv[:, 2 * d:] if v_sep is None else torch.empty((B * L, d), device=qkv.device, dtype=torch.float32)
        core.check(core.lib().ldetr_attention_bwd_f32(
            core.ptr(q), q.stride(0), core.ptr(k), k.stride(0), core.ptr(v), v.stride(0), core.ptr(kpm),
            core.ptr(out), d, core.ptr(lse), core.ptr(dout), d, core.ptr(dq), dq.stride(0), core.ptr(dk), dk.stride(0),
            core.ptr(dv), dv.stride(0), B, H, L, L, dh, scale, p_drop, seed, core.seed_ptr() if p_drop > 0 else None,
            causal, core.stream()), 'attention_bwd')
        return dqkv, (None if v_sep is None else dv), None, None, None, None, None, None


def kpm_u8(key_padding_mask):
    m = key_padding_mask
    if m is None:
        return None
    if m.dtype == torch.bool:
        return (m if m.is_contiguous() else m.contiguous()).view(torch.uint8)
    return m.to(torch.uint8).contiguous()


def attention(q, k, v, key_padding_mask, B, H, Lq, Lk, p_drop=0.0, kv_grad_dst=None):
    return _AttnFn.apply(q, k, v, kpm_u8(key_padding_mask), B, H, Lq, Lk, p_drop, kv_grad_dst)


class _GroupedKVFn(torch.autograd.Function):

    @staticmethod
    def forward(ctx, mem_pos, mem, holder, *params):
        core.require_gpu(mem_pos, mem)
        ctx.set_materialize_grads(False)
        Ws, bs = params[0::2], params[1::2]
        n, d = len(Ws), mem.shape[1]
        M = mem.shape[0]
        mp, mm = core.f32c(mem_pos), core.f32c(mem)
        with torch.no_grad():
            Wk = torch.cat([w.detach()[d:2 * d] for w in Ws] + [w.detach()[2 * d:] for w in Ws])
            bk = torch.cat([b.detach()[d:2 * d] for b in bs] + [b.detach()[2 * d:] for b in bs])
        nd = n * d
        KV = torch.empty((M, 2 * nd), device=mem.device, dtype=torch.float32)
        core.gemm(mp, Wk[:nd], 0, 0, M, nd, d, out=KV[:, :nd], ep=core.epilogue(col_bias=bk[:nd]))
        core.gemm(mm, Wk[nd:], 0, 0, M, nd, d, out=KV[:, nd:], ep=core.epilogue(col_bias=bk[nd:]))
        ctx.save_for_backward(mp, mm, Wk)
        ctx.params = (Ws, bs)
        ctx.cfg = (n, d, M)
        ctx.holder = holder
        holder.dK = holder.dV = None
        return tuple(KV[:, i * d:(i + 1) * d] for i in range(2 * n))

    @staticmethod
    def backward(ctx, *grads):
        mp, mm, Wk = ctx.saved_tensors
        n, d, M = ctx.cfg
        Ws, bs = ctx.params
        nd = n * d
        dK, dV = ctx.holder.dK, ctx.holder.dV
        fresh = dK is None
        if fresh:
            dK = core.zeros((M, nd), mp.device); dV = core.zeros((M, nd), mp.device)
        for i, g in enumerate(grads):
            dst = (dK if i < n else dV)[:, (i % n) * d:(i % n + 1) * d]
            if g is None:
                if not fresh:
                    dst.zero_()
            elif g.data_ptr() != dst.data_ptr() or g.stride() != dst.stride():
                dst.copy_(g)
        ctx.holder.dK = ctx.holder.dV = None
        dmp = core.gemm(dK, Wk[:nd], 0, 1, M, d, nd) if ctx.needs_input_grad[0] else None
        dmm = core.gemm(dV, Wk[nd:], 0, 1, M, d, nd) if ctx.needs_input_grad[1] else None
        need_w = any(ctx.needs_input_grad[3 + 2 * i] for i in range(n)) and not core.WEIGHT_GRADIENTS_DISABLED[0]
        out = [None] * (2 * n)
        if need_w:
            T = torch.empty((2, nd, d), device=mp.device, dtype=torch.float32)
            tb = core.zeros((2, nd), mp.device)
            core.gemm(dK, mp, 1, 1, nd, d, M, out=T[0], ep=core.epilogue(a_rowsum=tb[0]))
            core.gemm(dV, mm, 1, 1, nd, d, M, out=T[1], ep=core.epilogue(a_rowsum=tb[1]))
            gws, gbs = [core.flat_grad(w) for w in Ws], [core.flat_grad(b) for b in bs]
            strided = all(g is not None for g in gws + gbs) and n > 1
            if strided:
                sw = gws[1].storage_offset() - gws[0].storage_offset(); sb = gbs[1].storage_offset() - gbs[0].storage_offset()
                strided = (all(g.is_contiguous() and g.untyped_storage().data_ptr() == gws[0].untyped_storage().data_ptr() for g in gws + gbs)
                           and all(gws[i].storage_offset() - gws[0].storage_offset() == i * sw and gbs[i].storage_offset() - gbs[0].storage_offset() == i * sb for i in range(n)))
            if strided:
                gw = torch.as_strided(gws[0], (n, 2, d, d), (sw, d * d, d, 1), gws[0].storage_offset() + d * d)
                gw += T.view(2, n, d, d).permute(1, 0, 2, 3)
                gb = torch.as_strided(gbs[0], (n, 2, d), (sb, d, 1), gbs[0].storage_offset() + d)
                gb += tb.view(2, n, d).permute(1, 0, 2)
            else:
                for i in range(n):
                    if gws[i] is not None:
                        gws[i][d:2 * d] += T[0, i * d:(i + 1) * d]; gws[i][2 * d:] += T[1, i * d:(i + 1) * d]
                    else:
                        g = torch.zeros_like(Ws[i]); g[d:2 * d] = T[0, i * d:(i + 1) * d]; g[2 * d:] = T[1, i * d:(i + 1) * d]
                        out[2 * i] = g
                    if gbs[i] is not None:
                        gbs[i][d:2 * d] += tb[0, i * d:(i + 1) * d]; gbs[i][2 * d:] += tb[1, i * d:(i + 1) * d]
                    else:
                        g = torch.zeros_like(bs[i]); g[d:2 * d] = tb[0, i * d:(i + 1) * d]; g[2 * d:] = tb[1, i * d:(i + 1) * d]
                        out[2 * i + 1] = g
        return (dmp, dmm, None) + tuple(out)


class _KVHolder(object):
    dK = dV = None


def grouped_kv(mem_pos, mem, mhas):
    n, d, M = len(mhas), mem.shape[1], mem.shape[0]
    holder = _KVHolder()
    outs = _GroupedKVFn.apply(mem_pos, mem, holder, *[t for m in mhas for t in (m.in_proj_weight, m.in_proj_bias)])

    def dst(i):
        def views():
            if holder.dK is None:
                holder.dK = core.zeros((M, n * d), mem.device)
                holder.dV = core.zeros((M, n * d), mem.device)
            return holder.dK[:, i * d:(i + 1) * d], holder.dV[:, i * d:(i + 1) * d]
        return views
    return [(outs[i], outs[n + i], dst(i)) for i in range(n)]


def mha_forward(query, key, value, in_proj_weight, in_proj_bias, out_w, out_b, nhead, B, Lq, Lk,
                key_padding_mask=None, p_drop=0.0, same_qk=False, same_qkv=False, qk_pos=None, passthru=False, qk_in=None, kv_alias=False):
    d = query.shape[1]
    W, bvec = in_proj_weight, in_proj_bias
    alias = query
    if same_qkv:
        r = linear(query, W, bvec, passthru=passthru)
        qkv, alias = r if passthru else (r, query)
        o = _AttnPackedFn.apply(qkv, None, kpm_u8(key_padding_mask), B, nhead, Lq, p_drop)
    elif same_qk and qk_in is not None:
        qk = linear(qk_in, W, bvec, rows=(0, 2 * d))
        r = linear(query, W, bvec, rows=(2 * d, 3 * d), passthru=passthru)
        v, alias = r if passthru else (r, query)
        o = _AttnPackedFn.apply(qk, v, kpm_u8(key_padding_mask), B, nhead, Lq, p_drop)
    elif same_qk:
        r = linear(query, W, bvec, rows=(0, 2 * d), add_input=qk_pos, passthru=passthru)
        qk, alias = r if passthru else (r, query)
        vin = alias if value is query else value
        r = linear(vin, W, bvec, rows=(2 * d, 3 * d), passthru=passthru and value is query)
        v, alias = r if (passthru and value is query) else (r, alias)
        o = _AttnPackedFn.apply(qk, v, kpm_u8(key_padding_mask), B, nhead, Lq, p_drop)
    else:
        r = linear(query, W, bvec, rows=(0, d), passthru=passthru)
        q, alias = r if passthru else (r, query)
        if kv_alias:
            k, key = linear(key, W, bvec, rows=(d, 2 * d), passthru=True)
            v, value = linear(value, W, bvec, rows=(2 * d, 3 * d), passthru=True)
        else:
            k = linear(key, W, bvec, rows=(d, 2 * d))
            v = linear(value, W, bvec, rows=(2 * d, 3 * d))
        o = attention(q, k, v, key_padding_mask, B, nhead, Lq, Lk, p_drop)
    out = linear(o, out_w, out_b)
    if kv_alias:
        return out, alias, key, value
    return (out, alias) if passthru else out


def mha_cross_kv(query, K, V, grad_dst, in_proj_weight, in_proj_bias, out_w, out_b, nhead, B, Lq, Lk, key_padding_mask=None, p_drop=0.0):
    d = query.shape[1]
    q, alias = linear(query, in_proj_weight, in_proj_bias, rows=(0, d), passthru=True)
    o = attention(q, K, V, key_padding_mask, B, nhead, Lq, Lk, p_drop, kv_grad_dst=grad_dst)
    return linear(o, out_w, out_b), alias
```

### layoutdetr_amd/hip/core.py

```python
import ctypes
import os

import torch

from .. import _lib
from .._lib import Epilogue, Tensor4

ACT_NONE, ACT_RELU, ACT_LRELU = 0, 1, 2

_seed_counter = [0x5EED]

WEIGHT_GRADIENTS_DISABLED = [False]


class _EngineProfile(object):

    def __init__(self):
        self.enabled = False
        self.records = []

    def reset(self):
        self.records = []

    def summary(self):
        fl = sum(r[1] for r in self.records)
        ms = sum(r[2].elapsed_time(r[3]) for r in self.records)
        return fl, ms * 1e-3, len(self.records)


PROF = _EngineProfile()


_LEGACY_ENV = ('LDETR_PAIR_D', 'LDETR_DUAL_TRUNK', 'LDETR_FUSED_LAYOUT_LOSSES', 'LDETR_FFN_FUSED', 'LDETR_FFN_FUSED_LARGE', 'LDETR_GROUP_KV', 'LDETR_NO_WORKSPACE',
               'LDETR_TOKEN_STACKS', 'LDETR_SPLIT_BF16', 'LDETR_GEMM_PAIR', 'LDETR_P3_PAIR')
_legacy_warned = [False]


def _warn_legacy_env():
    if _legacy_warned[0]:
        return
    _legacy_warned[0] = True
    old = [k for k in _LEGACY_ENV if k in os.environ]
    if old:
        import warnings
        warnings.warn(f'{", ".join(old)}: these switch variables are IGNORED; the switches that remain are keys of LDETR_DEBUG="KEY=value,..."; see DESIGN.md, '
                      '"Diagnostic switches"')


def knob(key, default):
    _warn_legacy_env()
    for kv in os.environ.get('LDETR_DEBUG', '').split(','):
        k, _, v = kv.partition('=')
        if k.strip() == key and v.strip():
            try:
                return int(v)
            except ValueError:
                return int(float(v))
    return default


def engine_call(tag, flops, thunk, operands=(), nbytes=None):
    if not PROF.enabled:
        return thunk()
    s = torch.cuda.Event(enable_timing=True)
    e = torch.cuda.Event(enable_timing=True)
    c0 = engine_launch_counts()
    s.record()
    r = thunk()
    e.record()
    c1 = engine_launch_counts()
    if nbytes is None:
        nbytes = 4.0 * sum(t.numel() for t in operands if t is not None)
    PROF.records.append((tag, float(flops), s, e, nbytes, (c1[0] - c0[0], c1[1] - c0[1]), launched_kernel(tag)))
    return r


_P3_KINDS = {1: 'p3_nt_kernel', 2: 'p3_c3_kernel', 3: 'p3_tn_kernel', 4: 'p3_bwd_pair_nt_kernel', 5: 'p3_bwd_pair_c3_kernel'}
_ENGINE_KINDS = {1: 'gemm_f32_kernel', 2: 'gemm_small_kernel', 3: 'gemm_small_pair_kernel', 4: 'conv3x3_c32_kernel', 5: 'wgrad_c32_3x3_kernel', 6: 'stem_conv7x7_kernel'}


def launched_kernel(tag):
    info = (ctypes.c_int32 * 10)()
    if tag.startswith('ldetr_p3'):
        check(lib().ldetr_p3_last_launch(info), 'p3_last_launch')
        kind, bm, bn, nw, sk = info[0], info[1], info[2], info[3], info[4]
        name = _P3_KINDS.get(kind, 'p3_?')
        if kind in (2, 5):
            return name
        return f'{name}<{bm},{bn},{nw}w>' + (f' splitK={sk}' if sk > 1 else '')
    if tag == 'ldetr_token_stack':
        return 'token-stack kernels (mha_small / mha_cross / ffn / wgrad_multi)'
    check(lib().ldetr_engine_last_launch(info), 'engine_last_launch')
    kind, bm, bn, bk, nw, fast, split, sk = [info[i] for i in range(8)]
    name = _ENGINE_KINDS.get(kind, 'engine_?')
    if kind == 1:
        return f'{name}<{bm},{bn},{bk},{nw}w' + (',FAST' if fast else '') + (',SPLIT' if split else '') + '>' + (f' splitK={sk}' if sk > 1 else '')
    if kind in (2, 3):
        return f'{name}<{nw}w' + (',FAST' if fast else '') + '>'
    if kind == 4:
        return 'conv3x3_c32_split_kernel' if split else name
    return name


def engine_launch_counts():
    a, b = ctypes.c_int64(0), ctypes.c_int64(0)
    lib().ldetr_engine_launch_counts(ctypes.byref(a), ctypes.byref(b))
    return a.value, b.value



_workspace = {}
WORKSPACE_BYTES = int(os.environ.get('LDETR_WORKSPACE_MIB', '256')) << 20


def disable_splitk_workspace():
    l = _lib.load()
    dev = torch.cuda.current_device()
    _workspace[dev] = None
    check(l.ldetr_set_workspace(None, 0), 'set_workspace')


def enable_splitk_workspace():
    _workspace.pop(torch.cuda.current_device(), None)
    lib()


def lib():
    l = _lib.load()
    if torch.cuda.is_available():
        dev = torch.cuda.current_device()
        if dev not in _workspace:
            ws = torch.zeros(WORKSPACE_BYTES // 4, dtype=torch.float32, device=torch.device('cuda', dev))
            _workspace[dev] = ws
            check_rc = l.ldetr_set_workspace(ctypes.c_void_p(ws.data_ptr()), ws.numel() * 4)
            if check_rc != 0:
                raise RuntimeError('ldetr_set_workspace failed: ' + l.ldetr_last_error().decode())
    return l


def check(rc, what=''):
    _lib.check(rc, what)


def require_gpu(*tensors):
    for t in tensors:
        if t is not None and t.device.type != 'cuda':
            raise RuntimeError('layoutdetr_amd ops require tensors in GPU memory (no CPU fallback); got device '
                               f'{t.device}')


def stream():
    return ctypes.c_void_p(torch.cuda.current_stream().cuda_stream)


def ptr(t):
    if t is None:
        return None
    return ctypes.c_void_p(t.data_ptr())


def f32c(t):
    if t is None:
        return None
    if t.dtype != torch.float32:
        t = t.float()
    return t.contiguous()


def next_seed():
    _seed_counter[0] += 1
    base = int(torch.initial_seed()) & 0xFFFFFFFF
    return ((base << 32) ^ (_seed_counter[0] * 0x9E3779B1)) & 0xFFFFFFFFFFFFFFFF


_iter_seed = {}


def iter_seed(device=None):
    device = torch.device('cuda', torch.cuda.current_device()) if device is None else torch.device(device)
    key = (device.type, device.index)
    if key not in _iter_seed:
        _iter_seed[key] = torch.zeros(1, dtype=torch.int64, device=device)
    return _iter_seed[key]


def reseed(device=None):
    iter_seed(device).random_()


def seed_ptr():
    return ctypes.c_void_p(iter_seed().data_ptr())


def tensor4_nhwc(x):
    N, H, W, C = x.shape
    sn, sh, sw, sc = x.stride()
    return Tensor4(N, C, H, W, sn, sc, sh, sw)


def tensor4_nchw(x):
    N, C, H, W = x.shape
    sn, sc, sh, sw = x.stride()
    return Tensor4(N, C, H, W, sn, sc, sh, sw)


def epilogue(alpha=1.0, col_scale=None, col_bias=None, samp_scale=None, residual=None, act=ACT_NONE, act_alpha=0.0,
             act_gain=1.0, mask_src=None, mask_mode=0, out_scale=1.0, p_drop=0.0, seed=0, accumulate=False, a_rowsum=None):
    ep = Epilogue()
    ep.alpha = alpha
    ep.col_scale = col_scale.data_ptr() if col_scale is not None else None
    ep.col_bias = col_bias.data_ptr() if col_bias is not None else None
    if samp_scale is not None:
        ep.samp_scale = samp_scale.data_ptr()
        ep.samp_ld = samp_scale.stride(0)
    if residual is not None:
        ep.residual = residual.data_ptr()
        ep.ldr = residual.shape[-1]
    ep.act = act
    ep.act_alpha = act_alpha
    ep.act_gain = act_gain
    if mask_src is not None:
        ep.mask_src = mask_src.data_ptr()
        ep.ldm = mask_src.shape[-1]
    ep.mask_mode = mask_mode
    ep.out_scale = out_scale
    ep.p_drop = p_drop
    ep.seed = seed
    ep.seed_ptr = iter_seed().data_ptr() if p_drop > 0 else None
    ep.accumulate = 1 if accumulate else 0
    ep.a_rowsum = a_rowsum.data_ptr() if a_rowsum is not None else None
    return ep


def gemm(A, B, ta, tb, M, N, K, out=None, ep=None, splitk=0, pix_per_sample=0, lda=None, ldb=None):
    require_gpu(A, B)
    if out is None:
        out = torch.empty((M, N), device=A.device, dtype=torch.float32)
    lda = A.stride(0) if lda is None else lda
    ldb = B.stride(0) if ldb is None else ldb
    engine_call('gemm', 2.0 * M * N * K, lambda: check(lib().ldetr_gemm_f32(
        ptr(A), lda, int(ta), ptr(B), ldb, int(tb), ptr(out), out.stride(0), M, N, K, splitk,
        ctypes.byref(ep) if ep is not None else None, pix_per_sample, stream()), 'gemm'), nbytes=4.0 * (M * K + N * K + M * N))
    return out


def _pair_descs(g0, g1):
    descs = []
    flops = 0.0
    for g in (g0, g1):
        require_gpu(g['A'], g['B'], g['out'])
        d = _lib.GemmDesc()
        d.A = g['A'].data_ptr(); d.lda = g['A'].stride(0); d.ta = int(g['ta'])
        d.B = g['B'].data_ptr(); d.ldb = g['B'].stride(0); d.tb = int(g['tb'])
        d.C = g['out'].data_ptr(); d.ldc = g['out'].stride(0)
        d.M, d.N, d.K, d.splitk = int(g['M']), int(g['N']), int(g['K']), 0
        d.ep = ctypes.addressof(g['ep']) if g.get('ep') is not None else None
        d.pix_per_sample = 0
        descs.append(d)
        flops += 2.0 * d.M * d.N * d.K
    return descs, flops


def gemm_pair_is_single_launch(g0, g1):
    descs, _ = _pair_descs(g0, g1)
    return lib().ldetr_gemm_pair_is_single_launch(ctypes.byref(descs[0]), ctypes.byref(descs[1])) == 1


def gemm_pair(g0, g1):
    descs, flops = _pair_descs(g0, g1)
    engine_call('gemm', flops, lambda: check(lib().ldetr_gemm_pair_f32(ctypes.byref(descs[0]), ctypes.byref(descs[1]), stream()), 'gemm_pair'),
                nbytes=4.0 * sum(d.M * d.K + d.N * d.K + d.M * d.N for d in descs))


def colsum(a2d, B=1):
    require_gpu(a2d)
    R, C = a2d.shape
    if C % 4 != 0:
        return a2d.reshape(B, R // B, C).sum(1)
    red = torch.zeros((B, C), device=a2d.device, dtype=torch.float32)
    check(lib().ldetr_colsum_f32(ptr(a2d), ptr(red), B, R // B, C, stream()), 'colsum')
    return red


def flat_grad(p):
    if isinstance(p, torch.nn.Parameter) and getattr(p, '_ldetr_flat', False) and p.grad is not None and not torch.is_grad_enabled():
        return p.grad
    return None


class _ZeroArena(object):

    def __init__(self):
        self.buf = {}
        self.cursor = 0
        self.high = {}
        self.open = None

    def begin(self, device):
        dev = device.index if device.index is not None else torch.cuda.current_device()
        self.open = None
        if dev not in self.buf:
            if torch.cuda.is_current_stream_capturing():
                return
            cap = 1 << 22
            self.buf[dev] = (torch.zeros(cap, device=torch.device('cuda', dev), dtype=torch.float32), cap)
            self.high[dev] = 0
        buf, cap = self.buf[dev]
        n = min(cap, max(self.high[dev] * 2, 1 << 16))
        buf[:n].zero_()
        self.limit, self.cursor, self.open = n, 0, dev

    def take(self, shape, device):
        dev = device.index if device.index is not None else torch.cuda.current_device()
        if self.open != dev:
            return None
        n = 1
        for d in shape:
            n *= int(d)
        pad = (n + 3) // 4 * 4
        if self.cursor + pad > self.limit:
            self.high[dev] = max(self.high[dev], self.cursor + pad)
            return None
        out = self.buf[dev][0][self.cursor:self.cursor + n].view(shape)
        self.cursor += pad
        self.high[dev] = max(self.high[dev], self.cursor)
        return out

    def end(self):
        if self.open is not None and self.cursor and knob('ARENA_GUARD', 0) and not torch.cuda.is_current_stream_capturing():
            self.buf[self.open][0][:self.cursor].fill_(float('nan'))
        self.open = None


ZERO_ARENA = _ZeroArena()
_ZERO_ARENA_ON = True


def zero_arena_begin(device):
    if _ZERO_ARENA_ON:
        ZERO_ARENA.begin(torch.device(device))


def zero_arena_end():
    ZERO_ARENA.end()


def zeros(shape, device):
    device = torch.device(device)
    t = ZERO_ARENA.take(tuple(shape), device) if device.type == 'cuda' else None
    return t if t is not None else torch.zeros(shape, device=device, dtype=torch.float32)


def pick_splitk(tiles, K, target=512, min_k=256):
    s = 1
    while tiles * s < target and K // (s * 2) >= min_k and s < 256:
        s *= 2
    return s
```

### layoutdetr_amd/hip/linear.py

```python
import ctypes
import os

import torch

from . import core
from .core import ACT_LRELU, ACT_NONE, ACT_RELU


def act_backward(dy2, y2, act, act_alpha, act_gain, want_dbias, bias=None, demod=None, want_ddemod=False, B=1, dbias_out=None):
    R, C = dy2.shape
    if C % 4 != 0:
        if act == ACT_NONE:
            dv = dy2 * act_gain if act_gain != 1.0 else dy2
        else:
            neg = 0.0 if act == ACT_RELU else act_alpha
            dv = dy2 * torch.where(y2 > 0, act_gain, act_gain * neg)
        if want_dbias and dbias_out is not None:
            dbias_out += dv.sum(0)
            return dv, None, None
        return dv, (dv.sum(0) if want_dbias else None), None
    dv = torch.empty_like(dy2)
    if want_dbias and dbias_out is not None:
        dbias = dbias_out
    else:
        dbias = torch.zeros(C, device=dy2.device, dtype=torch.float32) if want_dbias else None
    ddemod = core.zeros((B, C), dy2.device) if want_ddemod else None
    core.check(core.lib().ldetr_act_bwd_reduce_f32(
        core.ptr(dy2), core.ptr(y2), core.ptr(dv), core.ptr(bias), core.ptr(demod), core.ptr(dbias), core.ptr(ddemod),
        B, R // B, C, act, act_alpha, act_gain, core.stream()), 'act_bwd_reduce')
    return dv, (None if dbias_out is not None else dbias), ddemod


class _LinearFn(torch.autograd.Function):
    @staticmethod
    def forward(ctx, x, weight, bias, act, act_alpha, act_gain, p_drop, wscale, rows, add_input, passthru):
        core.require_gpu(x, weight, bias)
        ctx.set_materialize_grads(False)
        r0, r1 = rows if rows is not None else (0, weight.shape[0])
        N, K = r1 - r0, weight.shape[1]
        x2 = x.reshape(-1, K)
        if not (x2.dtype == torch.float32 and x2.stride(1) == 1 and x2.stride(0) >= K and x2.stride(0) % 4 == 0 and x2.data_ptr() % 16 == 0):
            x2 = core.f32c(x2)
        if add_input is not None:
            if add_input.requires_grad:
                raise RuntimeError('linear: add_input is a constant (the sine position embedding); a learned embedding must be added by the caller')
            x2 = x2 + add_input.reshape(-1, K)
        w = core.f32c(weight.detach()[r0:r1])
        b = core.f32c(bias.detach()[r0:r1]) if bias is not None else None
        M = x2.shape[0]
        seed = core.next_seed() if p_drop > 0 else 0
        ep = core.epilogue(alpha=wscale, col_bias=b, act=act, act_alpha=act_alpha, act_gain=act_gain, p_drop=p_drop,
                           seed=seed)
        y = core.gemm(x2, w, 0, 0, M, N, K, ep=ep)
        ctx.save_for_backward(x2, w, y if act != ACT_NONE else None)
        ctx.cfg = (act, act_alpha, act_gain, p_drop, wscale, bias is not None, x.shape)
        ctx.params = (weight, bias, r0, r1)
        if p_drop > 0 and act != ACT_RELU:
            raise RuntimeError('linear: fused dropout is only defined after relu (FFN hidden layer)')
        if passthru:
            return y.reshape(*x.shape[:-1], N), x
        return y.reshape(*x.shape[:-1], N)

    @staticmethod
    def backward(ctx, dy, dx_pass=None):
        x2, w, y = ctx.saved_tensors
        act, act_alpha, act_gain, p_drop, wscale, has_bias, xshape = ctx.cfg
        N, K = w.shape
        M = x2.shape[0]
        if dy is None:
            return (dx_pass,) + (None,) * 10
        dy2 = core.f32c(dy.reshape(-1, N))
        need_x, need_w, need_b = ctx.needs_input_grad[0], ctx.needs_input_grad[1], has_bias and ctx.needs_input_grad[2]
        wparam, bparam, r0, r1 = ctx.params
        gw = core.flat_grad(wparam) if need_w else None
        gb = core.flat_grad(bparam) if need_b else None
        if gw is not None:
            gw = gw[r0:r1]
        if gb is not None:
            gb = gb[r0:r1] if (N % 4 == 0 and r0 % 4 == 0) else None
        pairable = need_x and need_w and gw is not None and gw.is_contiguous()
        dx = dw = db = None
        if act != ACT_NONE:
            gain = act_gain / (1.0 - p_drop) if p_drop > 0 else act_gain
            dpre, db, _ = act_backward(dy2, y, act, act_alpha, gain, need_b, dbias_out=gb)
        else:
            dpre = dy2
            db = None
            fold_db = need_b and gb is not None and need_w and gw is not None and gw.is_contiguous() and dpre.is_contiguous()
            if need_b and not fold_db:
                if gb is not None:
                    core.check(core.lib().ldetr_colsum_f32(core.ptr(dpre), core.ptr(gb), 1, M, N, core.stream()), 'colsum')
                else:
                    db = core.colsum(dpre).reshape(-1)
        if need_x and need_w and pairable:
            res = core.f32c(dx_pass.reshape(-1, K)) if dx_pass is not None else None
            dx2 = torch.empty((M, K), device=dpre.device, dtype=torch.float32)
            rsum = gb if (act == ACT_NONE and fold_db) else None
            core.gemm_pair(dict(A=dpre, B=w, ta=0, tb=1, M=M, N=K, K=N, out=dx2, ep=core.epilogue(alpha=wscale, residual=res)),
                           dict(A=dpre, B=x2, ta=1, tb=1, M=N, N=K, K=M, out=gw, ep=core.epilogue(alpha=wscale, accumulate=True, a_rowsum=rsum)))
            dx = dx2.reshape(xshape)
            need_x = need_w = False
        if need_x:
            res = core.f32c(dx_pass.reshape(-1, K)) if dx_pass is not None else None
            dx = core.gemm(dpre, w, 0, 1, M, K, N, ep=core.epilogue(alpha=wscale, residual=res)).reshape(xshape)
        if need_w:
            if gw is not None and gw.is_contiguous():
                rsum = gb if (act == ACT_NONE and fold_db) else None
                core.gemm(dpre, x2, 1, 1, N, K, M, out=gw, ep=core.epilogue(alpha=wscale, accumulate=True, a_rowsum=rsum))
            else:
                dw = core.gemm(dpre, x2, 1, 1, N, K, M, ep=core.epilogue(alpha=wscale))
        full = wparam.shape[0]
        if dw is not None and (r1 - r0) != full:
            dwf = torch.zeros((full, K), device=dw.device, dtype=torch.float32); dwf[r0:r1] = dw; dw = dwf
        if db is not None and (r1 - r0) != full:
            dbf = torch.zeros(full, device=db.device, dtype=torch.float32); dbf[r0:r1] = db; db = dbf
        return dx, dw, db, None, None, None, None, None, None, None, None


def linear(x, weight, bias=None, act=ACT_NONE, act_alpha=0.0, act_gain=1.0, p_drop=0.0, wscale=1.0, rows=None, add_input=None,
           passthru=False):
    return _LinearFn.apply(x, weight, bias, act, act_alpha, act_gain, p_drop, wscale, rows, add_input, passthru)
```

### layoutdetr_amd/training/networks_detr.py

```python
import numpy as np
import torch
import torch.nn as nn
import torch.nn.functional as F

from ..detr_util.misc import NestedTensor, nested_tensor_from_tensor_list
from ..hip import composite
from ..hip import conv as hconv
from ..hip import core
from ..hip.linear import linear
from .detr_backbone import Backbone, Joiner
from .detr_position_encoding import PositionEmbeddingSine
from .detr_transformer import Transformer, TransformerEncoder, TransformerEncoderLayer, TransformerWithToken
from .networks_stylegan2 import Decoder
from .util import TransformerWithToken_layoutganpp, encode_seq_first, encode_seq_first_pair


def merge_lists(lists):
    ret = []
    for l in lists:
        ret += l
    return ret


def split_list(list_a, chunk_size):
    return [list_a[i:i + chunk_size] for i in range(0, len(list_a), chunk_size)]


def normalize_2nd_moment(x, eps=1e-8):
    return x * (x.square().mean(dim=1, keepdim=True) + eps).rsqrt()


REFERENCE_DEFAULTS = False


def _resolve_text_mode(text_mode, tokenizer):
    if text_mode is not None:
        return text_mode
    if not REFERENCE_DEFAULTS:
        return 'features'
    if tokenizer is None:
        raise RuntimeError("Generator / Discriminator built through the reference's module names (layoutdetr_amd.dropin) take strings as bbox_text "
                           "and therefore need the BERT vocabulary: set LDETR_BERT_VOCAB=<path to bert-base-uncased vocab.txt> (or pass "
                           "tokenizer_vocab=...), or pass text_mode='features' and feed TextFeatures")
    return 'encoder+lm'


def build_backbone():
    backbone = Backbone(name='resnet50', train_backbone=True, return_interm_layers=None, dilation=False)
    position_embedding = PositionEmbeddingSine(num_pos_feats=128, normalize=True)
    model = Joiner(backbone, position_embedding)
    model.num_channels = backbone.num_channels
    return model


class TextFeatures(object):

    def __init__(self, text_feat, text_len, input_ids=None, attention_mask=None):
        self.text_feat = text_feat
        self.text_len = text_len
        self.input_ids = input_ids
        self.attention_mask = attention_mask

    def __len__(self):
        return self.text_feat.shape[0]

    def __getitem__(self, idx):
        return TextFeatures(self.text_feat[idx], self.text_len[idx],
                            None if self.input_ids is None else self.input_ids[idx],
                            None if self.attention_mask is None else self.attention_mask[idx])


class TextTokens(object):

    def __init__(self, input_ids, attention_mask, text_len, bos_token_id=30522, pad_token_id=0):
        self.input_ids, self.attention_mask, self.text_len = input_ids, attention_mask, text_len
        self.bos_token_id, self.pad_token_id = bos_token_id, pad_token_id

    def __len__(self):
        return self.input_ids.shape[0]

    def __getitem__(self, idx):
        return TextTokens(self.input_ids[idx], self.attention_mask[idx], self.text_len[idx], self.bos_token_id, self.pad_token_id)


def _build_text_encoder(text_mode, med_config, num_layers, num_heads):
    if text_mode == 'features':
        return _NoTextEncoder()
    if text_mode not in ('encoder', 'encoder+lm'):
        raise ValueError("text_mode must be 'features' (TextFeatures in), 'encoder' or 'encoder+lm' (TextTokens in)")
    import os
    from . import med
    cfg = med.BertConfig.from_json_file(med_config) if (med_config and os.path.exists(med_config)) else med.BertConfig()
    cfg.num_hidden_layers, cfg.num_attention_heads = num_layers, num_heads
    return med.BertModel(cfg, add_pooling_layer=False)


def _build_text_decoder(text_mode, med_config, num_layers, num_heads, encoder_width, vocab_size=30524):
    if text_mode != 'encoder+lm':
        return None
    import os
    from . import med
    cfg = med.BertConfig.from_json_file(med_config) if (med_config and os.path.exists(med_config)) else med.BertConfig()
    cfg.num_hidden_layers, cfg.num_attention_heads, cfg.encoder_width, cfg.vocab_size = num_layers, num_heads, encoder_width, vocab_size
    return med.BertLMHeadModel(cfg)


def _lm_loss(module, bbox_text, padding_mask, B, N, static):
    if module.text_decoder is None or not isinstance(bbox_text, TextTokens):
        return None
    dev = padding_mask.device
    T = bbox_text.input_ids.shape[-1]
    ids = bbox_text.input_ids.reshape(B * N, T).to(dev).clone()
    am = bbox_text.attention_mask.reshape(B * N, T).to(dev)
    ids[:, 0] = bbox_text.bos_token_id
    targets = ids.masked_fill(ids == bbox_text.pad_token_id, -100)
    pm = padding_mask.reshape(B * N)
    if static:
        targets = targets.masked_fill(pm[:, None], -100)
    else:
        keep = ~pm
        ids, am, targets = ids[keep], am[keep], targets[keep]
    return module.text_decoder(ids, attention_mask=am, labels=targets, return_dict=True, mode='text').loss


class _NoTextEncoder(nn.Module):

    def forward(self, *a, **k):
        raise NotImplementedError("text_mode='features': pass TextFeatures instead of strings (BERT text path is SURVEY §8f-1)")


class _EmbeddingFn(torch.autograd.Function):

    @staticmethod
    def forward(ctx, ids, weight):
        core.require_gpu(ids, weight)
        V, d = weight.shape
        i64 = ids.to(torch.int64).contiguous()
        out = torch.empty(tuple(ids.shape) + (d,), device=weight.device, dtype=torch.float32)
        core.check(core.lib().ldetr_embedding_fwd_f32(core.ptr(weight.detach().contiguous()), None, core.ptr(i64), core.ptr(out), i64.numel(), d, V, 1, core.stream()), 'embedding_fwd')
        ctx.save_for_backward(i64)
        ctx.param = weight
        return out

    @staticmethod
    def backward(ctx, dy):
        i64, = ctx.saved_tensors
        w = ctx.param
        V, d = w.shape
        acc = core.flat_grad(w)
        tgt = acc if (acc is not None and acc.is_contiguous()) else torch.zeros((V, d), device=dy.device, dtype=torch.float32)
        core.check(core.lib().ldetr_embedding_bwd_f32(core.ptr(core.f32c(dy)), core.ptr(i64), core.ptr(tgt), i64.numel(), d, V, -1, core.stream()), 'embedding_bwd')
        return None, (None if tgt is acc else tgt)


class Embedding(nn.Embedding):

    def forward(self, ids):
        if ids.is_cuda and self.weight.dtype == torch.float32 and self.weight.shape[1] % 4 == 0 and self.padding_idx is None:
            return _EmbeddingFn.apply(ids, self.weight)
        return super().forward(ids)


class Linear(nn.Linear):

    def forward(self, x, relu=False):
        if composite.active():
            return composite.linear(x, self.weight, self.bias, relu=relu)
        return linear(x, self.weight, self.bias, act=core.ACT_RELU if relu else core.ACT_NONE)


class Conv1x1(nn.Conv2d):

    def forward(self, x_nchw_view):
        x = x_nchw_view.permute(0, 2, 3, 1)
        y = hconv.conv2d_nhwc(x, self.weight, None, self.bias, None, 1, 0, relu=False)
        return y.permute(0, 3, 1, 2)


class MLP(nn.Module):

    def __init__(self, input_dim, hidden_dim, output_dim, num_layers):
        super().__init__()
        self.num_layers = num_layers
        h = [hidden_dim] * (num_layers - 1)
        self.layers = nn.ModuleList(Linear(n, k) for n, k in zip([input_dim] + h, h + [output_dim]))

    def forward(self, x, final_relu=False):
        for i, layer in enumerate(self.layers):
            x = layer(x, relu=(i < self.num_layers - 1) or final_relu)
        return x


def _build_tokenizer(tokenizer_vocab):
    import os
    path = tokenizer_vocab or os.environ.get('LDETR_BERT_VOCAB')
    if not path:
        return None
    from .tokenizer import BertWordPieceTokenizer
    return BertWordPieceTokenizer(path)


def _coerce_text(module, bbox_text, device):
    if isinstance(bbox_text, (list, tuple)) and len(bbox_text) and isinstance(bbox_text[0], (list, tuple)):
        if module.tokenizer is None:
            raise NotImplementedError('bbox_text strings need the BERT vocabulary: construct the module with tokenizer_vocab=<vocab.txt> '
                                      '(or set LDETR_BERT_VOCAB), or pass TextTokens / TextFeatures')
        if module.text_mode == 'features':
            raise NotImplementedError("bbox_text strings need the text encoder: construct the module with text_mode='encoder' (or 'encoder+lm')")
        from .tokenizer import texts_to_tokens
        return texts_to_tokens(module.tokenizer, bbox_text, module.max_text_length, device)
    return bbox_text


def _text_inputs(module, bbox_text, B, N, device):
    if isinstance(bbox_text, TextFeatures):
        return bbox_text.text_feat.to(device=device, dtype=torch.float32), bbox_text.text_len.to(device=device, dtype=torch.int64)
    if isinstance(bbox_text, TextTokens):
        T = bbox_text.input_ids.shape[-1]
        out = module.text_encoder(bbox_text.input_ids.reshape(B * N, T).to(device), attention_mask=bbox_text.attention_mask.reshape(B * N, T).to(device),
                                  return_dict=True, mode='text')
        return out.last_hidden_state[:, 0, :].reshape(B, N, -1), bbox_text.text_len.to(device=device, dtype=torch.int64)
    raise NotImplementedError('pass TextFeatures (precomputed CLS features) or TextTokens (tokenizer output); strings need the host tokenizer')


def _check_background_size(background_size):
    if ((background_size + 31) // 32) ** 2 > 16384:
        raise NotImplementedError(f'background_size={background_size}: at most 4096 (16384 image tokens)')


def _masked_ce_static(logits, target, valid):
    from .med import softmax_cross_entropy
    return softmax_cross_entropy(logits.flatten(0, 1), target.flatten().masked_fill(~valid.flatten(), -100))


def _zero_like_loss(ref):
    return ref.new_full((), 0.0)


class Generator(nn.Module):
    def __init__(self, z_dim, num_bbox_labels, img_channels, img_height, img_width, c_dim,
                 f_dim=256, num_heads=4, num_layers=8, hidden_dim=256,
                 med_config='configs/med_config.json', bert_f_dim=768, bert_num_encoder_layers=12, bert_num_decoder_layers=12,
                 bert_num_heads=12, background_size=1024, im_f_dim=512, max_text_length=256, text_mode=None, tokenizer_vocab=None):
        super().__init__()
        self.z_dim = z_dim
        self.tokenizer = _build_tokenizer(tokenizer_vocab)
        self.num_bbox_labels = num_bbox_labels
        self.c_dim = c_dim
        self.max_text_length = max_text_length
        self.text_mode = text_mode = _resolve_text_mode(text_mode, self.tokenizer)
        self.static_shapes = False
        _check_background_size(background_size)

        self.backbone = build_backbone()
        self.input_proj = Conv1x1(self.backbone.num_channels, hidden_dim, kernel_size=1)
        self.fc_z = Linear(z_dim * 9, bert_f_dim)
        self.emb_label = Embedding(num_bbox_labels, bert_f_dim)
        self.text_encoder = _build_text_encoder(text_mode, med_config, bert_num_encoder_layers, bert_num_heads)
        self.text_decoder = _build_text_decoder(text_mode, med_config, bert_num_decoder_layers, bert_num_heads, im_f_dim)
        self.enc_text_len = Embedding(max_text_length, bert_f_dim)
        self.fc_in = MLP(input_dim=4 * bert_f_dim, hidden_dim=bert_f_dim, output_dim=hidden_dim, num_layers=3)
        self.transformer = Transformer(d_model=hidden_dim, dropout=0.1, nhead=8, dim_feedforward=2048, num_encoder_layers=6,
                                       num_decoder_layers=6, normalize_before=False, return_intermediate_dec=False)
        self.bbox_embed = MLP(input_dim=hidden_dim, hidden_dim=hidden_dim, output_dim=4, num_layers=3)
        self.fc_z_rec = Linear(hidden_dim, z_dim * 9)
        self.fc_out_cls = Linear(hidden_dim, num_bbox_labels)
        self.fc_text_len_rec = Linear(hidden_dim, max_text_length)

    def trunk(self, background, body_out=None):
        if isinstance(background, (list, torch.Tensor)):
            background = nested_tensor_from_tensor_list(background)
        return self.backbone(background, body_out)

    def encode_condition(self, background, bbox_class, bbox_text, padding_mask):
        from . import shared_decode
        return shared_decode.encode_condition(self, background, bbox_class, bbox_text, padding_mask)

    def decode_candidates(self, cond, z):
        from . import shared_decode
        return shared_decode.decode_candidates(self, cond, z)

    def forward(self, z, bbox_class, bbox_real, bbox_text, bbox_patch, padding_mask, background, c, reconst=False, trunk_out=None):
        bg_feat, pos = self.trunk(background) if trunk_out is None else trunk_out
        bg_feat, mask = bg_feat[-1].decompose()
        assert mask is not None

        B, N = bbox_patch.shape[0], bbox_patch.shape[1]
        bbox_text = _coerce_text(self, bbox_text, bbox_class.device)
        z0 = normalize_2nd_moment(z.view(B, -1))
        zf = self.fc_z(z0).unsqueeze(1).expand(-1, N, -1)
        l = self.emb_label(bbox_class)
        text_feat, text_len = _text_inputs(self, bbox_text, B, N, bbox_class.device)
        text_len_feat = self.enc_text_len(text_len)
        x = torch.cat([zf, l, text_feat, text_len_feat], dim=-1)
        x = self.fc_in(x, final_relu=True).permute(1, 0, 2)

        x = self.transformer(src=self.input_proj(bg_feat), mask=mask, pos_embed=pos[-1], tgt=x, tgt_key_padding_mask=padding_mask)[0]
        bbox_fake = self.bbox_embed(x).sigmoid()
        if not reconst:
            return bbox_fake

        valid = ~padding_mask
        if self.static_shapes:
            z_rec = self.fc_z_rec(x)
            if z_rec.is_cuda and not z0.requires_grad:
                from ..hip.losses import masked_mse
                loss_z = masked_mse(z_rec, z0, valid.contiguous().view(torch.uint8), bdiv=N)
            else:
                vf = valid.to(torch.float32)
                cnt = vf.sum().clamp_min(1.0)
                loss_z = ((z_rec - z0.unsqueeze(1)).square().sum(-1) * vf).sum() / (cnt * z_rec.shape[-1])
            logit_cls = self.fc_out_cls(x)
            loss_text_len = _masked_ce_static(self.fc_text_len_rec(x), text_len, valid)
            loss_lm = _lm_loss(self, bbox_text, padding_mask, B, N, True)
            return bbox_fake, loss_z, logit_cls, (loss_lm if loss_lm is not None else _zero_like_loss(loss_z)), loss_text_len
        xv = x[valid]
        z_rec = self.fc_z_rec(xv)
        loss_z = F.mse_loss(z_rec, z0.unsqueeze(1).expand(-1, N, -1)[valid])
        logit_cls = self.fc_out_cls(xv)
        loss_lm = _lm_loss(self, bbox_text, padding_mask, B, N, False)
        loss_lm = loss_lm if loss_lm is not None else _zero_like_loss(loss_z)
        text_len_rec = self.fc_text_len_rec(xv)
        loss_text_len = F.cross_entropy(text_len_rec, text_len[valid])
        return bbox_fake, loss_z, logit_cls, loss_lm, loss_text_len


class Discriminator(nn.Module):
    def __init__(self, num_bbox_labels, img_channels, img_height, img_width, c_dim,
                 f_dim=256, num_heads=4, num_layers=8, max_bbox=50, hidden_dim=256,
                 med_config='configs/med_config.json', bert_f_dim=768, bert_num_encoder_layers=12, bert_num_decoder_layers=12,
                 bert_num_heads=12, background_size=1024, im_f_dim=512, max_text_length=256, text_mode=None, tokenizer_vocab=None):
        super().__init__()
        self.tokenizer = _build_tokenizer(tokenizer_vocab)
        self.num_bbox_labels = num_bbox_labels
        self.c_dim = c_dim
        self.max_text_length = max_text_length
        self.text_mode = text_mode = _resolve_text_mode(text_mode, self.tokenizer)
        self.static_shapes = False
        _check_background_size(background_size)

        self.backbone = build_backbone()
        self.input_proj = Conv1x1(self.backbone.num_channels, hidden_dim, kernel_size=1)
        self.fc_bbox = Linear(4, bert_f_dim)
        self.emb_label = Embedding(num_bbox_labels, bert_f_dim)
        self.text_encoder = _build_text_encoder(text_mode, med_config, bert_num_encoder_layers, bert_num_heads)
        self.text_decoder = _build_text_decoder(text_mode, med_config, bert_num_decoder_layers, bert_num_heads, im_f_dim)
        self.enc_text_len = Embedding(max_text_length, bert_f_dim)
        self.enc_fc_in = MLP(input_dim=4 * bert_f_dim, hidden_dim=bert_f_dim, output_dim=hidden_dim, num_layers=3)
        self.enc_transformer = TransformerWithToken(d_model=hidden_dim, dropout=0.1, nhead=8, dim_feedforward=2048,
                                                    num_encoder_layers=6, num_decoder_layers=6, normalize_before=False,
                                                    return_intermediate_dec=False)
        self.fc_out_disc = Linear(hidden_dim, 1)

        self.pos_token = nn.Parameter(torch.rand(max_bbox, 1, hidden_dim))
        self.dec_fc_in = Linear(hidden_dim + hidden_dim, hidden_dim)
        self.dec_transformer = TransformerEncoder(TransformerEncoderLayer(d_model=hidden_dim, nhead=8, dim_feedforward=2048), num_layers=6)
        self.bbox_embed = Linear(hidden_dim, 4)
        self.fc_out_cls = Linear(hidden_dim, num_bbox_labels)
        self.fc_text_len_rec = Linear(hidden_dim, max_text_length)
        self.bg_decoder = Decoder(z_dim=hidden_dim, w_dim=im_f_dim, channel_max=im_f_dim, channel_base=8192, img_channels=img_channels,
                                  img_resolution=background_size, use_noise=False, num_fp16_res=0, conv_clamp=None,
                                  fused_modconv_default=False)

        self.fc_bbox_uncond = Linear(4, bert_f_dim)
        self.emb_label_uncond = Embedding(num_bbox_labels, bert_f_dim)
        self.enc_fc_in_uncond = MLP(input_dim=2 * bert_f_dim, hidden_dim=bert_f_dim, output_dim=hidden_dim, num_layers=3)
        self.enc_transformer_uncond = TransformerWithToken_layoutganpp(d_model=hidden_dim, dim_feedforward=2048, nhead=8, num_layers=6)
        self.fc_out_disc_uncond = Linear(hidden_dim, 1)
        self.pos_token_uncond = nn.Parameter(torch.rand(max_bbox, 1, hidden_dim))
        self.dec_fc_in_uncond = Linear(hidden_dim + hidden_dim, hidden_dim)
        self.dec_transformer_uncond = TransformerEncoder(TransformerEncoderLayer(d_model=hidden_dim, nhead=8, dim_feedforward=2048), num_layers=6)
        self.bbox_embed_uncond = Linear(hidden_dim, 4)
        self.fc_out_cls_uncond = Linear(hidden_dim, num_bbox_labels)

    def trunk(self, background, body_out=None):
        if isinstance(background, (list, torch.Tensor)):
            background = nested_tensor_from_tensor_list(background)
        return self.backbone(background, body_out)

    def _logits(self, bbox, l, text_feat, text_len_feat, l_uncond, padding_mask, src, mask, pos):
        b = self.fc_bbox(bbox)
        x = torch.cat([b, l, text_feat, text_len_feat], dim=-1)
        x = self.enc_fc_in(x, final_relu=True).permute(1, 0, 2)
        x_uncond = torch.cat([self.fc_bbox_uncond(bbox), l_uncond], dim=-1)
        x_uncond = self.enc_fc_in_uncond(x_uncond, final_relu=True).permute(1, 0, 2)
        partner = None if composite.active() else self.enc_transformer_uncond.as_prog(x_uncond, padding_mask)
        if partner is not None:
            x, _, y_uncond = self.enc_transformer(src=src, mask=mask, pos_embed=pos, tgt=x, tgt_key_padding_mask=padding_mask, partner=partner[0])
            x_uncond = partner[1](y_uncond)
        else:
            x = self.enc_transformer(src=src, mask=mask, pos_embed=pos, tgt=x, tgt_key_padding_mask=padding_mask)[0]
            x_uncond = self.enc_transformer_uncond(x_uncond, src_key_padding_mask=padding_mask)
        x0 = x.transpose(0, 1)[0]
        logit_disc = self.fc_out_disc(x0).squeeze(-1)
        x0_uncond = x_uncond[0]
        return x0, logit_disc, x0_uncond, self.fc_out_disc_uncond(x0_uncond).squeeze(-1)

    def _reconstruct(self, x0, x0_uncond, bbox_text, text_len, padding_mask, B, N):
        valid = ~padding_mask
        x = x0.unsqueeze(0).expand(N, -1, -1)
        t = self.pos_token[:N].expand(-1, B, -1)
        x = self.dec_fc_in(torch.cat([x, t], dim=-1), relu=True)
        x_uncond = x0_uncond.unsqueeze(0).expand(N, -1, -1)
        t_uncond = self.pos_token_uncond[:N].expand(-1, B, -1)
        x_uncond = self.dec_fc_in_uncond(torch.cat([x_uncond, t_uncond], dim=-1), relu=True)
        x, x_uncond = encode_seq_first_pair(self.dec_transformer, x, self.dec_transformer_uncond, x_uncond, padding_mask)
        static = self.static_shapes
        x = x.permute(1, 0, 2) if static else x.permute(1, 0, 2)[valid]
        bbox_pred = self.bbox_embed(x).sigmoid()
        logit_cls = self.fc_out_cls(x)
        text_len_rec = self.fc_text_len_rec(x)
        if static:
            loss_text_len = _masked_ce_static(text_len_rec, text_len, valid)
        else:
            loss_text_len = F.cross_entropy(text_len_rec, text_len[valid])
        loss_lm = _lm_loss(self, bbox_text, padding_mask, B, N, static)
        loss_lm = loss_lm if loss_lm is not None else _zero_like_loss(loss_text_len)
        bg_rec = self.bg_decoder(x0)

        x_uncond = x_uncond.permute(1, 0, 2) if static else x_uncond.permute(1, 0, 2)[valid]
        bbox_pred_uncond = self.bbox_embed_uncond(x_uncond).sigmoid()
        logit_cls_uncond = self.fc_out_cls_uncond(x_uncond)
        return bbox_pred, logit_cls, loss_lm, loss_text_len, bg_rec, bbox_pred_uncond, logit_cls_uncond

    def forward(self, bbox, bbox_class, bbox_text, bbox_patch, padding_mask, background, c, reconst=False, trunk_out=None):
        bg_feat, pos = self.trunk(background) if trunk_out is None else trunk_out
        bg_feat, mask = bg_feat[-1].decompose()
        assert mask is not None

        B, N = bbox_patch.shape[0], bbox_patch.shape[1]
        bbox_text = _coerce_text(self, bbox_text, bbox_class.device)
        l = self.emb_label(bbox_class)
        text_feat, text_len = _text_inputs(self, bbox_text, B, N, bbox_class.device)
        text_len_feat = self.enc_text_len(text_len)
        x0, logit_disc, x0_uncond, logit_disc_uncond = self._logits(bbox, l, text_feat, text_len_feat, self.emb_label_uncond(bbox_class), padding_mask,
                                                                    self.input_proj(bg_feat), mask, pos[-1])
        if not reconst:
            return logit_disc, logit_disc_uncond
        return (logit_disc, logit_disc_uncond) + self._reconstruct(x0, x0_uncond, bbox_text, text_len, padding_mask, B, N)

    def forward_pair(self, bbox_fake, bbox_real, bbox_class, bbox_text, bbox_patch, padding_mask, background, c, trunk_out=None):
        bg_feat, pos = self.trunk(background) if trunk_out is None else trunk_out
        bg_feat, mask = bg_feat[-1].decompose()
        B, N = bbox_patch.shape[0], bbox_patch.shape[1]
        bbox_text = _coerce_text(self, bbox_text, bbox_class.device)
        l = self.emb_label(bbox_class)
        text_feat, text_len = _text_inputs(self, bbox_text, B, N, bbox_class.device)
        text_len_feat = self.enc_text_len(text_len)
        l_uncond = self.emb_label_uncond(bbox_class)
        two = lambda t: torch.cat([t, t], dim=0)
        x0, logit, x0_uncond, logit_uncond = self._logits(torch.cat([bbox_fake, bbox_real], dim=0), two(l), two(text_feat), two(text_len_feat), two(l_uncond),
                                                            two(padding_mask), two(self.input_proj(bg_feat)), two(mask), two(pos[-1]))
        rec = self._reconstruct(x0[B:], x0_uncond[B:], bbox_text, text_len, padding_mask, B, N)
        return (logit[:B], logit_uncond[:B]), (logit[B:], logit_uncond[B:]) + rec
```

Measured before the change: 504.4.

## Batch sibling small linears into one grouped small-GEMM launch

Adds a grouped small-GEMM kernel that runs up to four independent small GEMMs of mixed transpose modes in a single launch, with blocks ordered by per-split K. A new autograd function batches the forward and backward GEMMs of sibling linear layers through it. The generator and discriminator heads, the conditional/unconditional input MLPs and the QK/V attention projections are routed through it. The aim is to cut kernel-launch and host overhead for many tiny GEMMs, at the cost of more complex argument marshalling, extra Python descriptor building, and zero-filled full-size gradient buffers when a layer uses only a slice of its weight rows.

```diff
diff --git a/include/ldetr_hip.h b/include/ldetr_hip.h
--- a/include/ldetr_hip.h
+++ b/include/ldetr_hip.h
@@ -69,6 +69,9 @@
 int ldetr_gemm_pair_f32(const ldetr_gemm_desc* g0, const ldetr_gemm_desc* g1, void* stream);
 int ldetr_gemm_pair_is_single_launch(const ldetr_gemm_desc* g0, const ldetr_gemm_desc* g1);
 
+int ldetr_gemm_group_f32(const ldetr_gemm_desc* g, int n, void* stream);
+int ldetr_gemm_group_is_single_launch(const ldetr_gemm_desc* g, int n);
+
 int ldetr_conv2d_fwd_f32(const float* x, const ldetr_tensor4* xt, const float* w, int Cout, int KH, int KW, int stride,
                          int pad, float* y, int64_t ldy, int OH, int OW, const float* in_scale, int64_t in_scale_ld,
                          const ldetr_epilogue* ep, void* stream);
diff --git a/layoutdetr_amd/_lib.py b/layoutdetr_amd/_lib.py
--- a/layoutdetr_amd/_lib.py
+++ b/layoutdetr_amd/_lib.py
@@ -164,6 +164,8 @@
     'ldetr_sg2_handoff_f32': [_P, _P, _P, _P, _P, _P, _P, _P, _P, _P, _P, _P, _P, _P, _I, _L, _I, _F, _F, _P],
     'ldetr_gemm_pair_f32': [_P, _P, _P],
     'ldetr_gemm_pair_is_single_launch': [_P, _P],
+    'ldetr_gemm_group_f32': [_P, _I, _P],
+    'ldetr_gemm_group_is_single_launch': [_P, _I],
     'ldetr_demod_fwd_f32': [_P, _L, _L, _L, _L, _P, _P, _P, _I, _I, _I, _I, _I, _F, _P],
     'ldetr_demod_bwd_f32': [_P, _L, _L, _L, _L, _P, _P, _P, _P, _P, _I, _P, _I, _I, _I, _I, _I, _P],
     'ldetr_layout_losses_f32': [_P, _P, _P, _I, _I, _P, _P, _P],
diff --git a/layoutdetr_amd/build.py b/layoutdetr_amd/build.py
--- a/layoutdetr_amd/build.py
+++ b/layoutdetr_amd/build.py
@@ -18,7 +18,7 @@
 
 FLAGS = ([] if os.environ.get('LDETR_TILE_TRACE') else ['-DLDETR_TILE_TRACE=0']) + (['-DP3_TRACE'] if os.environ.get('LDETR_P3_TRACE') else []) + ['-O3', '-std=c++17', '-fPIC', f'--offload-arch={ARCH}', '-munsafe-fp-atomics', '-fno-gpu-rdc',
          '-Wno-unused-result', '-Rpass-analysis=kernel-resource-usage']
-NO_SCRATCH = ('wgrad_c32_3x3_kernel', 'gemm_f32_kernel', 'gemm_small_kernel', 'attn_fwd_kernel', 'attn_fwd_wide_kernel', 'attn_bwd_kernel', 'ffn_fwd_kernel', 'ffn_bwd_kernel', 'conv3x3_c32_kernel', 'mha_small_fwd_kernel', 'mha_cross_fwd_kernel', 'mha_small_bwd_kernel', 'mha_cross_bwd_kernel', 'wgrad_multi_kernel', 'ln_fwd_kernel', 'ln_bwd_kernel', 'p3_nt_kernel', 'p3_tn_kernel', 'p3_c3_kernel', 'p3_bwd_pair', 'layoutnet_features_kernel', 'layoutnet_forward_kernel', 'feature_stats_f64_kernel', 'layout_finish_kernel', 'layout_raster_kernel', 'page_blur_kernel', 'page_edge_kernel', 'patch_resize_kernel', 'sg2_handoff_kernel', 'png_gather_kernel', 'png_unfilter_kernel', 'png_enc_filter_kernel', 'png_enc_deflate_kernel', 'png_enc_assemble_kernel')
+NO_SCRATCH = ('wgrad_c32_3x3_kernel', 'gemm_f32_kernel', 'gemm_small_kernel', 'gemm_small_group_kernel', 'attn_fwd_kernel', 'attn_fwd_wide_kernel', 'attn_bwd_kernel', 'ffn_fwd_kernel', 'ffn_bwd_kernel', 'conv3x3_c32_kernel', 'mha_small_fwd_kernel', 'mha_cross_fwd_kernel', 'mha_small_bwd_kernel', 'mha_cross_bwd_kernel', 'wgrad_multi_kernel', 'ln_fwd_kernel', 'ln_bwd_kernel', 'p3_nt_kernel', 'p3_tn_kernel', 'p3_c3_kernel', 'p3_bwd_pair', 'layoutnet_features_kernel', 'layoutnet_forward_kernel', 'feature_stats_f64_kernel', 'layout_finish_kernel', 'layout_raster_kernel', 'page_blur_kernel', 'page_edge_kernel', 'patch_resize_kernel', 'sg2_handoff_kernel', 'png_gather_kernel', 'png_unfilter_kernel', 'png_enc_filter_kernel', 'png_enc_deflate_kernel', 'png_enc_assemble_kernel')
 
 
 def _hipcc():
diff --git a/layoutdetr_amd/csrc/gemm_conv.hip b/layoutdetr_amd/csrc/gemm_conv.hip
--- a/layoutdetr_amd/csrc/gemm_conv.hip
+++ b/layoutdetr_amd/csrc/gemm_conv.hip
@@ -1068,10 +1068,14 @@
     }
 }
 
+template <int NW> struct SmallLds { float red[NW][32][33]; float rsum[NW][32]; int last; };
+template <int NW> __device__ __forceinline__ SmallLds<NW>& small_lds() { __shared__ SmallLds<NW> s; return s; }
+
 template <int TA, int TB, int NW, bool FAST = false>
 __device__ __forceinline__ void gemm_small_body(const GemmParams& p, const int bx, const int by, const int bz, const int sk, const int gx) {
     using f32x16 = __attribute__((__vector_size__(16 * sizeof(float)))) float;
-    __shared__ float red[NW][32][33];
+    SmallLds<NW>& lds = small_lds<NW>();
+    float (&red)[NW][32][33] = lds.red;
     const int tid = threadIdx.x, lane = tid & 63, wave = tid >> 6;
     const int cl = lane & 31, kl = lane >> 5;
     const int m0 = by * 32, n0 = bx * 32;
@@ -1135,7 +1139,7 @@
             for (int t = 0; t < 16; t++) rs += a1[t];
         }
     }
-    __shared__ float rsum[NW][32];
+    float (&rsum)[NW][32] = lds.rsum;
     if (want_rs) {
         rs += __shfl_xor(rs, 32);
         if (kl == 0) rsum[wave][cl] = rs;
@@ -1168,7 +1172,7 @@
             }
         }
         asm volatile("s_waitcnt vmcnt(0)" ::: "memory");
-        __shared__ int s_last_small;
+        int& s_last_small = lds.last;
         __syncthreads();
         if (tid == 0) {
             const int old = atomicAdd(p.ws_count + tile, 1);
@@ -1236,6 +1240,27 @@
     else { const int c = b - nt0 * sk0, t = c % nt1; gemm_small_body<TA1, TB1, NW, FAST>(p1, t % gx1, t / gx1, c / nt1, sk1, gx1); }
 }
 
+constexpr int GROUP_MAX = 4;
+struct GroupArgs {
+    GemmParams p[GROUP_MAX];
+    int end[GROUP_MAX], gx[GROUP_MAX], nt[GROUP_MAX], sk[GROUP_MAX], mode[GROUP_MAX];
+};
+static_assert(sizeof(GroupArgs) <= 4096, "gemm_small_group_kernel: the argument block must fit the 4 KiB kernel-argument segment");
+
+template <int NW, bool FAST = false>
+__global__ __launch_bounds__(NW * 64) void gemm_small_group_kernel(GroupArgs a) {
+    const int b = blockIdx.x;
+    const int i = (b >= a.end[0]) + (b >= a.end[1]) + (b >= a.end[2]);
+    const int c = b - (i ? a.end[i - 1] : 0);
+    const int nt = a.nt[i], gx = a.gx[i], sk = a.sk[i], t = c % nt, bz = c / nt;
+    const GemmParams& p = a.p[i];
+    switch (a.mode[i]) {
+        case 0: gemm_small_body<0, 0, NW, FAST>(p, t % gx, t / gx, bz, sk, gx); break;
+        case 1: gemm_small_body<0, 1, NW, FAST>(p, t % gx, t / gx, bz, sk, gx); break;
+        default: gemm_small_body<1, 1, NW, FAST>(p, t % gx, t / gx, bz, sk, gx); break;
+    }
+}
+
 static inline bool al16(const void* p) { return (((uintptr_t)p) & 15) == 0; }
 
 
@@ -1249,11 +1274,17 @@
     return g_workspace[dev];
 }
 
+static bool ring_fits(long tiles, size_t bytes) {
+    const Workspace& w = workspace_for_current_device();
+    const size_t need = (bytes + 255) & ~(size_t)255;
+    const size_t pbytes = w.bytes > WS_COUNTERS * sizeof(int) ? w.bytes - WS_COUNTERS * sizeof(int) : 0;
+    return w.ptr && need <= pbytes && tiles <= WS_COUNTERS;
+}
 static bool ring_alloc(long tiles, size_t bytes, int** counters, float** partials) {
     Workspace& w = workspace_for_current_device();
     const size_t need = (bytes + 255) & ~(size_t)255;
     const size_t pbytes = w.bytes > WS_COUNTERS * sizeof(int) ? w.bytes - WS_COUNTERS * sizeof(int) : 0;
-    if (!w.ptr || need > pbytes || tiles > WS_COUNTERS) return false;
+    if (!ring_fits(tiles, bytes)) return false;
     if (w.counter_cursor + tiles > (size_t)WS_COUNTERS) w.counter_cursor = 0;
     if (w.partial_cursor + need > pbytes) w.partial_cursor = 0;
     *counters = reinterpret_cast<int*>(w.ptr) + w.counter_cursor;
@@ -1269,13 +1300,18 @@
     return ring_alloc(0, bytes, &counters, &r) ? r : nullptr;
 }
 
+static int small_split_factor(int K, long blocks) {
+    int sk = 1;
+    if (blocks <= 128 && K >= 1024) {
+        sk = K / 256; if (sk > 8) sk = 8;
+        while (sk > 1 && blocks * sk > 640) sk--;
+        if (sk > 1 && !ring_fits(blocks, (size_t)blocks * sk * 1024 * sizeof(float))) sk = 1;
+    }
+    return sk;
+}
 static int plan_small_split(GemmParams& p, long blocks) {
-    int sk = 1;
-    if (blocks <= 128 && p.K >= 1024) {
-        sk = p.K / 256; if (sk > 8) sk = 8;
-        while (sk > 1 && blocks * sk > 640) sk--;
-        if (sk > 1 && !ring_alloc(blocks, (size_t)blocks * sk * 1024 * sizeof(float), &p.ws_count, &p.ws)) sk = 1;
-    }
+    int sk = small_split_factor(p.K, blocks);
+    if (sk > 1 && !ring_alloc(blocks, (size_t)blocks * sk * 1024 * sizeof(float), &p.ws_count, &p.ws)) sk = 1;
     return sk;
 }
 
@@ -1292,6 +1328,8 @@
 static auto small_kernel() { return gemm_small_kernel<TA, TB, NW, FAST>; }
 template <int NW, bool FAST, int TA0, int TB0, int TA1, int TB1>
 static auto small_kernel() { return gemm_small_pair_kernel<TA0, TB0, TA1, TB1, NW, FAST>; }
+template <int NW, bool FAST>
+static auto small_kernel() { return gemm_small_group_kernel<NW, FAST>; }
 
 template <int... MODES, typename... Args>
 static void launch_small_kernel(bool fast, bool w8, dim3 grid, hipStream_t st, const Args&... args) {
@@ -1328,6 +1366,31 @@
     launch_small_kernel<TA0, 1, 1, 1>(fast, w8, grid, st, p0, p1, gx0, nt0, sk0, gx1, nt1, sk1);
     note_engine_launch(3, 32, 32, 0, w8 ? 8 : 4, fast ? 1 : 0, 0, sk0 * 256 + sk1, (long)grid.x, (TA0 * 2 + 1) * 4 + 3);
     return check_launch("gemm_small_pair");
+}
+
+static int launch_small_group(GemmParams* p, const int* mode, int n, hipStream_t st) {
+    int order[GROUP_MAX], gx[GROUP_MAX], nt[GROUP_MAX], sk[GROUP_MAX];
+    bool fast = true, w8 = true;
+    for (int i = 0; i < n; i++) {
+        gx[i] = cdiv(p[i].N, 32); nt[i] = gx[i] * cdiv(p[i].M, 32);
+        sk[i] = plan_small_split(p[i], nt[i]);
+        fast = fast && small_fast_ok(p[i], mode[i] >> 1, mode[i] & 1);
+        w8 = w8 && small_wants8(nt[i], sk[i], p[i].K);
+        order[i] = i;
+    }
+    for (int i = 1; i < n; i++)
+        for (int j = i; j > 0 && cdiv(p[order[j]].K, sk[order[j]]) > cdiv(p[order[j - 1]].K, sk[order[j - 1]]); j--) { const int o = order[j]; order[j] = order[j - 1]; order[j - 1] = o; }
+    GroupArgs a;
+    int total = 0, sks = 0, modes = 0;
+    for (int s = 0; s < GROUP_MAX; s++) {
+        const int i = order[s < n ? s : n - 1];
+        a.p[s] = p[i]; a.gx[s] = gx[i]; a.nt[s] = nt[i]; a.sk[s] = sk[i]; a.mode[s] = mode[i];
+        if (s < n) { total += nt[i] * sk[i]; sks |= sk[i] << (8 * s); modes |= (8 | mode[i]) << (4 * s); }
+        a.end[s] = total;
+    }
+    launch_small_kernel<>(fast, w8, dim3((unsigned)total), st, a);
+    note_engine_launch(7, 32, 32, 0, w8 ? 8 : 4, fast ? 1 : 0, 0, sks, (long)total, modes);
+    return check_launch("gemm_small_group");
 }
 
 struct EpiParams { GemmEpilogue ep; float* C; long ldc; long rows; int N; int pix_per_sample; };
@@ -1755,6 +1818,42 @@
     int rc = gemm_dense(*g0, stream);
     if (rc) return rc;
     return gemm_dense(*g1, stream);
+}
+
+static bool group_member_ok(const ldetr_gemm_desc& g) {
+    const bool ta = g.ta != 0, tb = g.tb != 0;
+    return g.A && g.B && g.C && small_class(g) && (!ta || tb) && (!(g.ep && g.ep->a_rowsum) || (ta && tb && g.lda == g.M));
+}
+static bool group_single_launch(const ldetr_gemm_desc* g, int n) {
+    if (!g || n < 1 || n > GROUP_MAX) return false;
+    bool w8 = false;
+    for (int i = 0; i < n; i++) {
+        if (!group_member_ok(g[i])) return false;
+        const long blocks = (long)cdiv(g[i].N, 32) * cdiv(g[i].M, 32);
+        const bool w = small_wants8(blocks, small_split_factor(g[i].K, blocks), g[i].K);
+        if (i && w != w8) return false;
+        w8 = w;
+    }
+    return true;
+}
+
+extern "C" int ldetr_gemm_group_is_single_launch(const ldetr_gemm_desc* g, int n) { return group_single_launch(g, n) ? 1 : 0; }
+
+extern "C" int ldetr_gemm_group_f32(const ldetr_gemm_desc* g, int n, void* stream) {
+    LDETR_CHECK(g, "gemm_group: null descriptor");
+    LDETR_CHECK(n >= 1 && n <= 16, "gemm_group: 1 <= n <= 16 problems");
+    for (int i0 = 0; i0 < n; i0 += GROUP_MAX) {
+        const int m = n - i0 < GROUP_MAX ? n - i0 : GROUP_MAX;
+        if (m > 1 && group_single_launch(g + i0, m)) {
+            GemmParams p[GROUP_MAX]; int mode[GROUP_MAX];
+            for (int i = 0; i < m; i++) { p[i] = fill_dense(g[i0 + i]); mode[i] = (g[i0 + i].ta ? 2 : 0) + (g[i0 + i].tb ? 1 : 0); }
+            const int rc = launch_small_group(p, mode, m, (hipStream_t)stream);
+            if (rc) return rc;
+        } else {
+            for (int i = 0; i < m; i++) { const int rc = gemm_dense(g[i0 + i], stream); if (rc) return rc; }
+        }
+    }
+    return LDETR_OK;
 }
 
 extern "C" int ldetr_conv2d_fwd_f32(const float* x, const ldetr_tensor4* xt, const float* w, int Cout, int KH, int KW,
diff --git a/layoutdetr_amd/hip/attention.py b/layoutdetr_amd/hip/attention.py
--- a/layoutdetr_amd/hip/attention.py
+++ b/layoutdetr_amd/hip/attention.py
@@ -3,7 +3,7 @@
 import torch
 
 from . import core
-from .linear import linear
+from .linear import linear, linear_group
 
 
 class _AttnFn(torch.autograd.Function):
@@ -206,6 +206,10 @@
         r = linear(query, W, bvec, passthru=passthru)
         qkv, alias = r if passthru else (r, query)
         o = _AttnPackedFn.apply(qkv, None, kpm_u8(key_padding_mask), B, nhead, Lq, p_drop)
+    elif same_qk and qk_in is not None and core.knob('GEMM_GROUP', 3) & 1:
+        r = linear_group([(qk_in, W, bvec, (0, 2 * d), core.ACT_NONE, False), (query, W, bvec, (2 * d, 3 * d), core.ACT_NONE, passthru)])
+        qk, v, alias = r[0], r[1], (r[2] if passthru else query)
+        o = _AttnPackedFn.apply(qk, v, kpm_u8(key_padding_mask), B, nhead, Lq, p_drop)
     elif same_qk and qk_in is not None:
         qk = linear(qk_in, W, bvec, rows=(0, 2 * d))
         r = linear(query, W, bvec, rows=(2 * d, 3 * d), passthru=passthru)
diff --git a/layoutdetr_amd/hip/core.py b/layoutdetr_amd/hip/core.py
--- a/layoutdetr_amd/hip/core.py
+++ b/layoutdetr_amd/hip/core.py
@@ -76,7 +76,7 @@
 
 
 _P3_KINDS = {1: 'p3_nt_kernel', 2: 'p3_c3_kernel', 3: 'p3_tn_kernel', 4: 'p3_bwd_pair_nt_kernel', 5: 'p3_bwd_pair_c3_kernel'}
-_ENGINE_KINDS = {1: 'gemm_f32_kernel', 2: 'gemm_small_kernel', 3: 'gemm_small_pair_kernel', 4: 'conv3x3_c32_kernel', 5: 'wgrad_c32_3x3_kernel', 6: 'stem_conv7x7_kernel'}
+_ENGINE_KINDS = {1: 'gemm_f32_kernel', 2: 'gemm_small_kernel', 3: 'gemm_small_pair_kernel', 4: 'conv3x3_c32_kernel', 5: 'wgrad_c32_3x3_kernel', 6: 'stem_conv7x7_kernel', 7: 'gemm_small_group_kernel'}
 
 
 def launched_kernel(tag):
@@ -95,7 +95,7 @@
     name = _ENGINE_KINDS.get(kind, 'engine_?')
     if kind == 1:
         return f'{name}<{bm},{bn},{bk},{nw}w' + (',FAST' if fast else '') + (',SPLIT' if split else '') + '>' + (f' splitK={sk}' if sk > 1 else '')
-    if kind in (2, 3):
+    if kind in (2, 3, 7):
         return f'{name}<{nw}w' + (',FAST' if fast else '') + '>'
     if kind == 4:
         return 'conv3x3_c32_split_kernel' if split else name
@@ -244,10 +244,10 @@
     return out
 
 
-def _pair_descs(g0, g1):
+def _pair_descs(*gs):
     descs = []
     flops = 0.0
-    for g in (g0, g1):
+    for g in gs:
         require_gpu(g['A'], g['B'], g['out'])
         d = _lib.GemmDesc()
         d.A = g['A'].data_ptr(); d.lda = g['A'].stride(0); d.ta = int(g['ta'])
@@ -269,6 +269,22 @@
 def gemm_pair(g0, g1):
     descs, flops = _pair_descs(g0, g1)
     engine_call('gemm', flops, lambda: check(lib().ldetr_gemm_pair_f32(ctypes.byref(descs[0]), ctypes.byref(descs[1]), stream()), 'gemm_pair'),
+                nbytes=4.0 * sum(d.M * d.K + d.N * d.K + d.M * d.N for d in descs))
+
+
+def _group_array(gs):
+    descs, flops = _pair_descs(*gs)
+    return (_lib.GemmDesc * len(descs))(*descs), flops, descs
+
+
+def gemm_group_is_single_launch(gs):
+    arr, _, _ = _group_array(gs)
+    return lib().ldetr_gemm_group_is_single_launch(arr, len(gs)) == 1
+
+
+def gemm_group(gs):
+    arr, flops, descs = _group_array(gs)
+    engine_call('gemm_group', flops, lambda: check(lib().ldetr_gemm_group_f32(arr, len(gs), stream()), 'gemm_group'),
                 nbytes=4.0 * sum(d.M * d.K + d.N * d.K + d.M * d.N for d in descs))
 
 
diff --git a/layoutdetr_amd/hip/linear.py b/layoutdetr_amd/hip/linear.py
--- a/layoutdetr_amd/hip/linear.py
+++ b/layoutdetr_amd/hip/linear.py
@@ -117,6 +117,137 @@
         return dx, dw, db, None, None, None, None, None, None, None, None
 
 
+def _rows2d(x, K):
+    x2 = x.reshape(-1, K)
+    if not (x2.dtype == torch.float32 and x2.stride(1) == 1 and x2.stride(0) >= K and x2.stride(0) % 4 == 0 and x2.data_ptr() % 16 == 0):
+        x2 = core.f32c(x2)
+    return x2
+
+
+def _issue_members(members):
+    chunks, cur = [], []
+    for probs in members:
+        if cur and sum(len(m) for m in cur) + len(probs) > 4:
+            chunks.append(cur); cur = []
+        if probs:
+            cur.append(probs)
+    if cur:
+        chunks.append(cur)
+    for chunk in chunks:
+        flat = [g for m in chunk for g in m]
+        if len(flat) > 1 and len(chunk) > 1 and core.gemm_group_is_single_launch(flat):
+            core.gemm_group(flat)
+            continue
+        for m in chunk:
+            if len(m) == 2 and m[1]['ep'].accumulate:
+                core.gemm_pair(m[0], m[1])
+                continue
+            for g in m:
+                core.gemm(g['A'], g['B'], g['ta'], g['tb'], g['M'], g['N'], g['K'], out=g['out'], ep=g['ep'])
+
+
+class _LinearGroupFn(torch.autograd.Function):
+
+    @staticmethod
+    def forward(ctx, meta, *tensors):
+        ctx.set_materialize_grads(False)
+        n = len(meta)
+        ys, probs, saved, cfg, params, x2s = [], [], [], [], [], {}
+        for i, (rows, act, passthru) in enumerate(meta):
+            x, weight, bias = tensors[3 * i:3 * i + 3]
+            core.require_gpu(x, weight, bias)
+            r0, r1 = rows if rows is not None else (0, weight.shape[0])
+            N, K = r1 - r0, weight.shape[1]
+            if id(x) not in x2s:
+                x2s[id(x)] = _rows2d(x, K)
+            x2 = x2s[id(x)]
+            w = core.f32c(weight.detach()[r0:r1])
+            b = core.f32c(bias.detach()[r0:r1]) if bias is not None else None
+            M = x2.shape[0]
+            y = torch.empty((M, N), device=x2.device, dtype=torch.float32)
+            probs.append(dict(A=x2, B=w, ta=0, tb=0, M=M, N=N, K=K, out=y, ep=core.epilogue(col_bias=b, act=act)))
+            saved += [x2, w, y if act != ACT_NONE else None]
+            cfg.append((act, bias is not None, x.shape, bool(passthru)))
+            params.append((weight, bias, r0, r1))
+            ys.append(y.reshape(*x.shape[:-1], N))
+        core.gemm_group(probs)
+        ctx.save_for_backward(*saved)
+        ctx.cfg, ctx.params = cfg, params
+        return tuple(ys) + tuple(tensors[3 * i] for i in range(n) if meta[i][2])
+
+    @staticmethod
+    def backward(ctx, *grads):
+        saved, cfg, n = ctx.saved_tensors, ctx.cfg, len(ctx.cfg)
+        passes = iter(grads[n:])
+        out, members = [None], []
+        for i in range(n):
+            x2, w, y = saved[3 * i:3 * i + 3]
+            act, has_bias, xshape, passthru = cfg[i]
+            dy, dx_pass = grads[i], (next(passes) if passthru else None)
+            if dy is None:
+                out += [dx_pass, None, None]
+                continue
+            N, K = w.shape
+            M = x2.shape[0]
+            dy2 = core.f32c(dy.reshape(-1, N))
+            need_x, need_w, need_b = ctx.needs_input_grad[1 + 3 * i], ctx.needs_input_grad[2 + 3 * i], has_bias and ctx.needs_input_grad[3 + 3 * i]
+            wparam, bparam, r0, r1 = ctx.params[i]
+            gw = core.flat_grad(wparam) if need_w else None
+            gb = core.flat_grad(bparam) if need_b else None
+            if gw is not None:
+                gw = gw[r0:r1]
+            if gb is not None:
+                gb = gb[r0:r1] if (N % 4 == 0 and r0 % 4 == 0) else None
+            flat_w = gw is not None and gw.is_contiguous()
+            dx = dw = db = rsum = None
+            if act != ACT_NONE:
+                dpre, db, _ = act_backward(dy2, y, act, 0.0, 1.0, need_b, dbias_out=gb)
+            else:
+                dpre = dy2
+                if need_b and gb is not None and need_w and flat_w:
+                    rsum = gb
+                elif need_b and gb is not None:
+                    core.check(core.lib().ldetr_colsum_f32(core.ptr(dpre), core.ptr(gb), 1, M, N, core.stream()), 'colsum')
+                elif need_b:
+                    db = core.colsum(dpre).reshape(-1)
+            probs = []
+            members.append(probs)
+            if need_x:
+                res = core.f32c(dx_pass.reshape(-1, K)) if dx_pass is not None else None
+                dx2 = torch.empty((M, K), device=dpre.device, dtype=torch.float32)
+                probs.append(dict(A=dpre, B=w, ta=0, tb=1, M=M, N=K, K=N, out=dx2, ep=core.epilogue(residual=res)))
+                dx = dx2.reshape(xshape)
+            elif dx_pass is not None:
+                dx = dx_pass
+            if need_w and flat_w:
+                probs.append(dict(A=dpre, B=x2, ta=1, tb=1, M=N, N=K, K=M, out=gw, ep=core.epilogue(accumulate=True, a_rowsum=rsum)))
+            elif need_w:
+                dw = torch.empty((N, K), device=dpre.device, dtype=torch.float32)
+                probs.append(dict(A=dpre, B=x2, ta=1, tb=1, M=N, N=K, K=M, out=dw, ep=core.epilogue()))
+            full = wparam.shape[0]
+            if dw is not None and (r1 - r0) != full:
+                dwf = torch.zeros((full, K), device=dw.device, dtype=torch.float32); dw = (dwf, dw, r0, r1)
+            if db is not None and (r1 - r0) != full:
+                dbf = torch.zeros(full, device=db.device, dtype=torch.float32); dbf[r0:r1] = db; db = dbf
+            out += [dx, dw, db]
+        _issue_members(members)
+        for k, v in enumerate(out):
+            if isinstance(v, tuple):
+                dwf, dw, r0, r1 = v
+                dwf[r0:r1] = dw
+                out[k] = dwf
+        return tuple(out)
+
+
+def linear_group(specs):
+    n = len(specs)
+    rev = specs[::-1]
+    r = _LinearGroupFn.apply(tuple((s[3], s[4], bool(s[5])) for s in rev), *[t for s in rev for t in s[:3]])
+    ys = list(r[:n])[::-1]
+    aliases = list(r[n:])[::-1]
+    return ys + aliases
+
+
 def linear(x, weight, bias=None, act=ACT_NONE, act_alpha=0.0, act_gain=1.0, p_drop=0.0, wscale=1.0, rows=None, add_input=None,
            passthru=False):
     return _LinearFn.apply(x, weight, bias, act, act_alpha, act_gain, p_drop, wscale, rows, add_input, passthru)
diff --git a/layoutdetr_amd/training/networks_detr.py b/layoutdetr_amd/training/networks_detr.py
--- a/layoutdetr_amd/training/networks_detr.py
+++ b/layoutdetr_amd/training/networks_detr.py
@@ -7,7 +7,7 @@
 from ..hip import composite
 from ..hip import conv as hconv
 from ..hip import core
-from ..hip.linear import linear
+from ..hip.linear import linear, linear_group
 from .detr_backbone import Backbone, Joiner
 from .detr_position_encoding import PositionEmbeddingSine
 from .detr_transformer import Transformer, TransformerEncoder, TransformerEncoderLayer, TransformerWithToken
@@ -169,6 +169,12 @@
         return linear(x, self.weight, self.bias, act=core.ACT_RELU if relu else core.ACT_NONE)
 
 
+def linear_siblings(members):
+    if len(members) < 2 or composite.active() or not (core.knob('GEMM_GROUP', 3) & 2) or not all(x.is_cuda for _, x, _ in members):
+        return [m(x, relu=relu) for m, x, relu in members]
+    return linear_group([(x, m.weight, m.bias, None, core.ACT_RELU if relu else core.ACT_NONE, False) for m, x, relu in members])
+
+
 class Conv1x1(nn.Conv2d):
 
     def forward(self, x_nchw_view):
@@ -185,9 +191,9 @@
         h = [hidden_dim] * (num_layers - 1)
         self.layers = nn.ModuleList(Linear(n, k) for n, k in zip([input_dim] + h, h + [output_dim]))
 
-    def forward(self, x, final_relu=False):
+    def forward(self, x, final_relu=False, first=None):
         for i, layer in enumerate(self.layers):
-            x = layer(x, relu=(i < self.num_layers - 1) or final_relu)
+            x = first if (i == 0 and first is not None) else layer(x, relu=(i < self.num_layers - 1) or final_relu)
         return x
 
 
@@ -296,13 +302,16 @@
         x = self.fc_in(x, final_relu=True).permute(1, 0, 2)
 
         x = self.transformer(src=self.input_proj(bg_feat), mask=mask, pos_embed=pos[-1], tgt=x, tgt_key_padding_mask=padding_mask)[0]
-        bbox_fake = self.bbox_embed(x).sigmoid()
+        if not (reconst and self.static_shapes):
+            bbox_fake = self.bbox_embed(x).sigmoid()
         if not reconst:
             return bbox_fake
 
         valid = ~padding_mask
         if self.static_shapes:
-            z_rec = self.fc_z_rec(x)
+            h0, z_rec, logit_cls, text_len_rec = linear_siblings([(self.bbox_embed.layers[0], x, True), (self.fc_z_rec, x, False), (self.fc_out_cls, x, False),
+                                                                  (self.fc_text_len_rec, x, False)])
+            bbox_fake = self.bbox_embed(x, first=h0).sigmoid()
             if z_rec.is_cuda and not z0.requires_grad:
                 from ..hip.losses import masked_mse
                 loss_z = masked_mse(z_rec, z0, valid.contiguous().view(torch.uint8), bdiv=N)
@@ -310,8 +319,7 @@
                 vf = valid.to(torch.float32)
                 cnt = vf.sum().clamp_min(1.0)
                 loss_z = ((z_rec - z0.unsqueeze(1)).square().sum(-1) * vf).sum() / (cnt * z_rec.shape[-1])
-            logit_cls = self.fc_out_cls(x)
-            loss_text_len = _masked_ce_static(self.fc_text_len_rec(x), text_len, valid)
+            loss_text_len = _masked_ce_static(text_len_rec, text_len, valid)
             loss_lm = _lm_loss(self, bbox_text, padding_mask, B, N, True)
             return bbox_fake, loss_z, logit_cls, (loss_lm if loss_lm is not None else _zero_like_loss(loss_z)), loss_text_len
         xv = x[valid]
@@ -381,9 +389,10 @@
     def _logits(self, bbox, l, text_feat, text_len_feat, l_uncond, padding_mask, src, mask, pos):
         b = self.fc_bbox(bbox)
         x = torch.cat([b, l, text_feat, text_len_feat], dim=-1)
-        x = self.enc_fc_in(x, final_relu=True).permute(1, 0, 2)
         x_uncond = torch.cat([self.fc_bbox_uncond(bbox), l_uncond], dim=-1)
-        x_uncond = self.enc_fc_in_uncond(x_uncond, final_relu=True).permute(1, 0, 2)
+        for lc, lu in zip(self.enc_fc_in.layers, self.enc_fc_in_uncond.layers):
+            x, x_uncond = linear_siblings([(lc, x, True), (lu, x_uncond, True)])
+        x, x_uncond = x.permute(1, 0, 2), x_uncond.permute(1, 0, 2)
         partner = None if composite.active() else self.enc_transformer_uncond.as_prog(x_uncond, padding_mask)
         if partner is not None:
             x, _, y_uncond = self.enc_transformer(src=src, mask=mask, pos_embed=pos, tgt=x, tgt_key_padding_mask=padding_mask, partner=partner[0])
@@ -392,24 +401,25 @@
             x = self.enc_transformer(src=src, mask=mask, pos_embed=pos, tgt=x, tgt_key_padding_mask=padding_mask)[0]
             x_uncond = self.enc_transformer_uncond(x_uncond, src_key_padding_mask=padding_mask)
         x0 = x.transpose(0, 1)[0]
-        logit_disc = self.fc_out_disc(x0).squeeze(-1)
         x0_uncond = x_uncond[0]
-        return x0, logit_disc, x0_uncond, self.fc_out_disc_uncond(x0_uncond).squeeze(-1)
+        logit_disc, logit_uncond = linear_siblings([(self.fc_out_disc, x0, False), (self.fc_out_disc_uncond, x0_uncond, False)])
+        return x0, logit_disc.squeeze(-1), x0_uncond, logit_uncond.squeeze(-1)
 
     def _reconstruct(self, x0, x0_uncond, bbox_text, text_len, padding_mask, B, N):
         valid = ~padding_mask
         x = x0.unsqueeze(0).expand(N, -1, -1)
         t = self.pos_token[:N].expand(-1, B, -1)
-        x = self.dec_fc_in(torch.cat([x, t], dim=-1), relu=True)
         x_uncond = x0_uncond.unsqueeze(0).expand(N, -1, -1)
         t_uncond = self.pos_token_uncond[:N].expand(-1, B, -1)
-        x_uncond = self.dec_fc_in_uncond(torch.cat([x_uncond, t_uncond], dim=-1), relu=True)
+        x, x_uncond = linear_siblings([(self.dec_fc_in, torch.cat([x, t], dim=-1), True), (self.dec_fc_in_uncond, torch.cat([x_uncond, t_uncond], dim=-1), True)])
         x, x_uncond = encode_seq_first_pair(self.dec_transformer, x, self.dec_transformer_uncond, x_uncond, padding_mask)
         static = self.static_shapes
         x = x.permute(1, 0, 2) if static else x.permute(1, 0, 2)[valid]
-        bbox_pred = self.bbox_embed(x).sigmoid()
-        logit_cls = self.fc_out_cls(x)
-        text_len_rec = self.fc_text_len_rec(x)
+        x_uncond = x_uncond.permute(1, 0, 2) if static else x_uncond.permute(1, 0, 2)[valid]
+        bbox_pred, logit_cls, text_len_rec, bbox_pred_uncond, logit_cls_uncond = linear_siblings(
+            [(self.bbox_embed, x, False), (self.fc_out_cls, x, False), (self.fc_text_len_rec, x, False),
+             (self.bbox_embed_uncond, x_uncond, False), (self.fc_out_cls_uncond, x_uncond, False)])
+        bbox_pred, bbox_pred_uncond = bbox_pred.sigmoid(), bbox_pred_uncond.sigmoid()
         if static:
             loss_text_len = _masked_ce_static(text_len_rec, text_len, valid)
         else:
@@ -418,9 +428,6 @@
         loss_lm = loss_lm if loss_lm is not None else _zero_like_loss(loss_text_len)
         bg_rec = self.bg_decoder(x0)
 
-        x_uncond = x_uncond.permute(1, 0, 2) if static else x_uncond.permute(1, 0, 2)[valid]
-        bbox_pred_uncond = self.bbox_embed_uncond(x_uncond).sigmoid()
-        logit_cls_uncond = self.fc_out_cls_uncond(x_uncond)
         return bbox_pred, logit_cls, loss_lm, loss_text_len, bg_rec, bbox_pred_uncond, logit_cls_uncond
 
     def forward(self, bbox, bbox_class, bbox_text, bbox_patch, padding_mask, background, c, reconst=False, trunk_out=None):
```

After: 506.7 (median of 6 runs). No clear change (+0.5%).
